# QZ1-boy/CDFO

Measured on AMD Instinct MI355X. Metric: x4 SR frames/sec, 7-frame 270x480->1080p, higher is better.
Workload: dtype fp16 MFMA, fp32 accumulate (1 pass inside Block_, 2 passes = fp16 hi+lo activations elsewhere, split-bf16 for the returned feature cache; 2-4e-4 max-abs vs the fp32 reference, bound 1e-3); 1 GPU; JCT-VC ClassB-shape synthetic clips: 8 clips/GPU x 7x1x270x480 luma (padded to 272x480) + MV/residual/partition/unfiltered priors -> 1080x1920, fresh path (pre_L1_fea=None), precision=fp16x2, Gumbel noise drawn per forward inside the mask kernel (the reference's default behaviour); clips_per_gpu=8, parallelism=batch-shard x1, weights=random init (seed 0), launch=eager

## Files before the change

### cdfo_amd/csrc/conv1x1_stream.hip

```cpp
#include "plane_chunk.h"

namespace {

struct st_item { const float* base; int ld; int ch0; };

struct st_args {
  st_item act[CDFO_MAXSRC * 4];
  int nkb;
  st_item res[2];
  const float* res_scale;
  const float* w; long long w_bstride; const float* bias;
  int Cin, Cout, CoutP, act_fn;
  float* out; int ldo;
  int B; long long P;
  int tiles_per_image; long long tiles;
  int ns;
  _Float16* ln_hl; const float* ln_g; const float* ln_b;
  const float* w_last;
  int W;
  float* csum; int csum_slots;
  pc_plane plane;
};

__host__ __device__ inline long long st_owner(long long t, long long tiles, int grid) { return ((t + 1) * grid + tiles - 1) / tiles - 1; }
// ... 42 lines not shown
    d_part[k] = (s & 15) ^ (p & 15);
  }
  auto part_off = [&](int q) { return r * 256 + ((q ^ (r & 15)) << 4); };

  f16x8_t twh[TAPS ? 4 : 1], twl[TAPS ? 4 : 1];
  if (TAPS) {
#pragma unroll
    for (int s4 = 0; s4 < 4; ++s4)
#pragma unroll
      for (int j = 0; j < 8; ++j) {
        const float wv = r < 9 ? a.w_last[(16 * s4 + 8 * h + j) * 9 + r] : 0.f;
        twh[s4][j] = (_Float16)wv;
        twl[s4][j] = (_Float16)(wv - (float)twh[s4][j]);
      }
  }

  for (long long img_t0 = t_lo; img_t0 < t_hi;) {
    const int b = (int)(img_t0 / a.tiles_per_image);
    const long long img_end = (long long)(b + 1) * a.tiles_per_image;
    const long long seg_hi = img_end < t_hi ? img_end : t_hi;
    __syncthreads();
    {
      const float* wb = a.w + (long long)b * a.w_bstride;
      const int ngrp = (a.Cin >> 2) * NCB * 64;
      for (int i = tid; i < ngrp; i += ST_THREADS) {
        const int rowpos = i % (NCB * 64), kg = i / (NCB * 64);
        const int n = mfma_row_channel(rowpos);
        f32x4 wv = {0.f, 0.f, 0.f, 0.f};
        if (n < a.CoutP) wv = *reinterpret_cast<const f32x4*>(wb + ((long long)kg * a.CoutP + n) * 4);
        const int c = kg >> 2, hh = (kg >> 1) & 1, j0 = (kg & 1) * 4;
        u32x2 hi, lo;
        split4_bf16(wv, hi, lo);
        const int off = ((c * 2 + hh) * (NCB * 64) + rowpos) * 16 + j0 * 2;
        *reinterpret_cast<u32x2*>(sWh + off) = hi;
        *reinterpret_cast<u32x2*>(sWl + off) = lo;
      }
      for (int i = tid; i < NCB * 64; i += ST_THREADS) sBias[i] = (a.bias && i < a.Cout) ? a.bias[i] : 0.f;
      if (PLANE) pc_load_weights<NCB>(a.plane.w + (long long)b * a.plane.w_bstride, a.CoutP, sPh, sPl, tid);
    }
    __syncthreads();

    const long long n_items = (seg_hi - img_t0) * items_per_tile;
    long long issued = 0;
    auto issue = [&](long long it) {
      const long long tile = img_t0 + it / items_per_tile;
      const int k = (int)(it % items_per_tile);
      const long long p0 = (tile - (long long)b * a.tiles_per_image) * 128 + wave * 32;
      if (a.res_scale && k == 0) {
        const long long rows = a.P - p0;
        const i32x4 rs = lds_dma_rsrc_uniform(a.res_scale + (long long)b * a.P + (rows > 0 ? p0 : 0),
                                              (unsigned)(rows > 0 ? (rows < 32 ? rows : 32) * 4 : 0));
        lds_dma0_dword((unsigned)r * 4, rs, __builtin_amdgcn_readfirstlane(scale_lds + (unsigned)(tile & 1) * 256));
      }
      if (PLANE && k == 0)
        pc_issue(pc_image(a.plane, b), (int)a.P, a.plane.W, (int)p0, lane, tap_lds + (unsigned)((it / items_per_tile) % NS) * PC_SLOT);
      st_item src;
      int chan0;
      if (k < nkb) { src = a.act[k]; chan0 = src.ch0; }
      else {
        const int j = k - nkb;
        src = a.res[j / NCB];
        chan0 = (j % NCB) * 64;
      }
      const long long rows_left = a.P - p0;
      const float* base = src.base + ((long long)b * a.P + (rows_left > 0 ? p0 : 0)) * src.ld + chan0;
      i32x4 rsrc = lds_dma_rsrc_uniform(base, 0u);
      const long long bytes = rows_left > 0 ? (rows_left < 32 ? rows_left : 32) * (long long)src.ld * 4 : 0;
      lds_dma_rsrc_resize_uniform(rsrc, (unsigned)bytes);
      unsigned voff[8];
#pragma unroll
      for (int q = 0; q < 8; ++q) voff[q] = (unsigned)(d_px[q] * src.ld * 4 + d_part[q] * 16);
      lds_dma0(voff, rsrc, __builtin_amdgcn_readfirstlane(ring_lds + (unsigned)(it % NS) * ST_STAGE));
    };
    for (; issued < NS - 1 && issued < n_items; ++issued) issue(issued);

    f32x16 acc[NCB][2];
    float cs[CSUM ? 32 : 1];
#pragma unroll
    for (int e = 0; e < (CSUM ? 32 : 1); ++e) cs[e] = 0.f;
    for (long long it = 0; it < n_items; ++it) {
      const int k = (int)(it % items_per_tile);
      st_wait_landed(TAPS ? 0 : issued - it - 1);
      const unsigned char* st = ring + (it % NS) * ST_STAGE;
      if (TAPS) {
        if (issued < n_items) { wait_lgkm<0>(); issue(issued); ++issued; }
      }
      if (k == 0) {
#pragma unroll
        for (int cb = 0; cb < NCB; ++cb)
#pragma unroll
          for (int ni = 0; ni < 2; ++ni)
#pragma unroll
            for (int e = 0; e < 16; ++e) acc[cb][ni][e] = 0.f;
        if (PLANE) {
          const int p = (int)((img_t0 + it / items_per_tile - (long long)b * a.tiles_per_image) * 128) + wave * 32 + r;
          unsigned thi[4], tlo[4];
          pc_operand(tap_slots + ((it / items_per_tile) % NS) * PC_SLOT, r, h, p, (int)a.P, a.plane.W, thi, tlo);
          pc_mfma<NCB>(sPh, sPl, r, h, thi, tlo, acc);
        }
      }
      if (k < nkb) {
#pragma unroll
        for (int c = 0; c < 4; ++c) {
          const f32x4 v0 = *reinterpret_cast<const f32x4*>(st + part_off(c * 4 + h * 2));
          const f32x4 v1 = *reinterpret_cast<const f32x4*>(st + part_off(c * 4 + h * 2 + 1));
          union { unsigned u[4]; bf16x8_t v; } ph, pl;
          split8_bf16(v0, v1, ph.u, pl.u);
          const int wrow = ((k * 4 + c) * 2 + h) * (NCB * 64) + r;
#pragma unroll
          for (int cb = 0; cb < NCB; ++cb)
#pragma unroll
            for (int ni = 0; ni < 2; ++ni) {
              const bf16x8_t wh = *reinterpret_cast<const bf16x8_t*>(sWh + (wrow + cb * 64 + ni * 32) * 16);
              const bf16x8_t wl = *reinterpret_cast<const bf16x8_t*>(sWl + (wrow + cb * 64 + ni * 32) * 16);
              acc[cb][ni] = __builtin_amdgcn_mfma_f32_32x32x16_bf16(wh, pl.v, acc[cb][ni], 0, 0, 0);
              acc[cb][ni] = __builtin_amdgcn_mfma_f32_32x32x16_bf16(wl, ph.v, acc[cb][ni], 0, 0, 0);
              acc[cb][ni] = __builtin_amdgcn_mfma_f32_32x32x16_bf16(wh, ph.v, acc[cb][ni], 0, 0, 0);
            }
        }
        if (k == nkb - 1) {
#pragma unroll
          for (int cb = 0; cb < NCB; ++cb)
#pragma unroll
            for (int ni = 0; ni < 2; ++ni)
#pragma unroll
              for (int e = 0; e < 16; ++e) {
                const float t = acc[cb][ni][e] + sBias[cb * 64 + ni * 32 + (e >> 3) * 16 + h * 8 + (e & 7)];
                acc[cb][ni][e] = fmaxf(t, 0.f) + slope * fminf(t, 0.f);
              }
        }
      } else {
        const int cb = (k - nkb) % NCB;
        float sc = 1.f;
        if (a.res_scale && (k - nkb) / NCB == nres - 1)
          sc = *reinterpret_cast<const float*>(scale_slots + ((img_t0 + it / items_per_tile) & 1) * 256 + lane * 4);
#pragma unroll
        for (int cc = 0; cc < NCB; ++cc) {
          if (cc != cb) continue;
#pragma unroll
          for (int ni = 0; ni < 2; ++ni)
#pragma unroll
            for (int jj = 0; jj < 2; ++jj) {
              const int q = (ni * 32 + jj * 16 + h * 8) >> 2;
              const f32x4 r0 = *reinterpret_cast<const f32x4*>(st + part_off(q));
              const f32x4 r1 = *reinterpret_cast<const f32x4*>(st + part_off(q + 1));
#pragma unroll
              for (int e = 0; e < 4; ++e) { acc[cc][ni][8 * jj + e] = fmaf(sc, r0[e], acc[cc][ni][8 * jj + e]); acc[cc][ni][8 * jj + 4 + e] = fmaf(sc, r1[e], acc[cc][ni][8 * jj + 4 + e]); }
            }
        }
      }
      if (!TAPS && issued < n_items) { wait_lgkm<0>(); issue(issued); ++issued; }
      if (k == items_per_tile - 1) {
        const long long tile = img_t0 + it / items_per_tile;
        const long long pin = (tile - (long long)b * a.tiles_per_image) * 128 + wave * 32 + r;
        if (NCB == 1 && a.ln_hl && !a.ln_g) {
          typedef _Float16 st_f16x8 __attribute__((ext_vector_type(8)));
          if (pin < a.P) {
#pragma unroll
            for (int ni = 0; ni < 2; ++ni)
#pragma unroll
              for (int jj = 0; jj < 2; ++jj) {
                const int n = ni * 32 + jj * 16 + h * 8;
                st_f16x8 hv;
#pragma unroll
                for (int e = 0; e < 8; ++e) hv[e] = (_Float16)acc[0][ni][8 * jj + e];
                *reinterpret_cast<st_f16x8*>(a.ln_hl + (((long long)b * 4 + (n >> 4)) * a.P + pin) * 16 + h * 8) = hv;
              }
          }
        } else if (NCB == 1 && a.ln_hl) {
          typedef _Float16 st_f16x8 __attribute__((ext_vector_type(8)));
          float sm = 0.f;
#pragma unroll
          for (int ni = 0; ni < 2; ++ni)
#pragma unroll
            for (int e = 0; e < 16; ++e) sm += acc[0][ni][e];
          sm += __shfl_xor(sm, 32, 64);
          const float mu = sm * (1.f / 64.f);
          float sq = 0.f;
#pragma unroll
          for (int ni = 0; ni < 2; ++ni)
#pragma unroll
            for (int e = 0; e < 16; ++e) { const float d = acc[0][ni][e] - mu; sq = fmaf(d, d, sq); }
          sq += __shfl_xor(sq, 32, 64);
          const float rstd = 1.f / sqrtf(sq * (1.f / 64.f) + 1e-5f);
          if (pin < a.P) {
#pragma unroll
            for (int ni = 0; ni < 2; ++ni)
#pragma unroll
              for (int jj = 0; jj < 2; ++jj) {
                const int n = ni * 32 + jj * 16 + h * 8;
                const f32x4 g0 = *reinterpret_cast<const f32x4*>(a.ln_g + n), g1 = *reinterpret_cast<const f32x4*>(a.ln_g + n + 4);
                const f32x4 b0 = *reinterpret_cast<const f32x4*>(a.ln_b + n), b1 = *reinterpret_cast<const f32x4*>(a.ln_b + n + 4);
                st_f16x8 hi, lo;
#pragma unroll
                for (int e = 0; e < 8; ++e) {
                  const float y = (acc[0][ni][8 * jj + e] - mu) * rstd * (e < 4 ? g0[e & 3] : g1[e & 3]) + (e < 4 ? b0[e & 3] : b1[e & 3]);
                  hi[e] = (_Float16)y;
                  lo[e] = (_Float16)(y - (float)hi[e]);
                }
                _Float16* o16 = a.ln_hl + (((long long)b * 8 + (n >> 4)) * a.P + pin) * 16 + h * 8;
                *reinterpret_cast<st_f16x8*>(o16) = hi;
                *reinterpret_cast<st_f16x8*>(o16 + 4 * a.P * 16) = lo;
              }
          }
        }
        if (TAPS) {
          const int oy = (int)(pin / a.W), ox = (int)(pin - (long long)oy * a.W);
#pragma unroll
          for (int cb = 0; cb < NCB; ++cb) {
            float amax = 0.f;
#pragma unroll
            for (int ni = 0; ni < 2; ++ni)
#pragma unroll
              for (int e = 0; e < 16; ++e) amax = fmaxf(amax, fabsf(acc[cb][ni][e]));
            amax = fmaxf(amax, __shfl_xor(amax, 32, 64));
            int ex = 0;
            if (amax > 0.f && amax < INFINITY) frexpf(amax, &ex);
            ex = ex < -100 ? -100 : (ex > 100 ? 100 : ex);
            const float sc = ldexpf(1.f, 14 - ex), inv = ldexpf(1.f, ex - 14);
            f32x16 tacc;
#pragma unroll
            for (int e = 0; e < 16; ++e) tacc[e] = 0.f;
#pragma unroll
            for (int s4 = 0; s4 < 4; ++s4) {
              unsigned hh[4], ll[4];
#pragma unroll
              for (int j = 0; j < 4; ++j)
                split_pair_f16(acc[cb][s4 >> 1][8 * (s4 & 1) + 2 * j] * sc, acc[cb][s4 >> 1][8 * (s4 & 1) + 2 * j + 1] * sc, hh[j], ll[j]);
              const u32x4 hu = {hh[0], hh[1], hh[2], hh[3]}, lu = {ll[0], ll[1], ll[2], ll[3]};
              const f16x8_t yh = __builtin_bit_cast(f16x8_t, hu), yl = __builtin_bit_cast(f16x8_t, lu);
              tacc = __builtin_amdgcn_mfma_f32_32x32x16_f16(twl[s4], yh, tacc, 0, 0, 0);
              tacc = __builtin_amdgcn_mfma_f32_32x32x16_f16(twh[s4], yl, tacc, 0, 0, 0);
              tacc = __builtin_amdgcn_mfma_f32_32x32x16_f16(twh[s4], yh, tacc, 0, 0, 0);
            }
            if (pin < a.P) {
              const long long opix = ((long long)b * 2 * (a.P / a.W) + 2 * oy + (cb >> 1)) * (2 * a.W) + 2 * ox + (cb & 1);
              float* op = a.out + opix * a.ldo;
              const f32x4 t4 = {tacc[0] * inv, tacc[1] * inv, tacc[2] * inv, tacc[3] * inv};
              *reinterpret_cast<f32x4*>(op + 4 * h) = t4;
              if (h == 0) op[8] = tacc[4] * inv;
            }
          }
        } else if (pin < a.P) {
          if (CSUM) {
#pragma unroll
            for (int ni = 0; ni < 2; ++ni)
#pragma unroll
              for (int e = 0; e < 16; ++e) cs[ni * 16 + e] += acc[0][ni][e];
          }
          float* op = a.out + ((long long)b * a.P + pin) * a.ldo;
#pragma unroll
          for (int cb = 0; cb < NCB; ++cb)
#pragma unroll
            for (int ni = 0; ni < 2; ++ni)
#pragma unroll
              for (int jj = 0; jj < 2; ++jj) {
                const int n = cb * 64 + ni * 32 + jj * 16 + h * 8;
                if (n < a.Cout) {
                  f32x4 v0, v1;
#pragma unroll
                  for (int e = 0; e < 4; ++e) { v0[e] = acc[cb][ni][8 * jj + e]; v1[e] = acc[cb][ni][8 * jj + 4 + e]; }
                  *reinterpret_cast<f32x4*>(op + n) = v0;
                  *reinterpret_cast<f32x4*>(op + n + 4) = v1;
                }
              }
        }
      }
    }
    if (CSUM) {
      float* red = reinterpret_cast<float*>(ring);
#pragma unroll
      for (int ni = 0; ni < 2; ++ni)
#pragma unroll
        for (int jj = 0; jj < 2; ++jj) {
          const int n = ni * 32 + jj * 16 + h * 8;
          const f32x4 v0 = {cs[ni * 16 + 8 * jj], cs[ni * 16 + 8 * jj + 1], cs[ni * 16 + 8 * jj + 2], cs[ni * 16 + 8 * jj + 3]};
          const f32x4 v1 = {cs[ni * 16 + 8 * jj + 4], cs[ni * 16 + 8 * jj + 5], cs[ni * 16 + 8 * jj + 6], cs[ni * 16 + 8 * jj + 7]};
          *reinterpret_cast<f32x4*>(red + r * 64 + n) = v0;
          *reinterpret_cast<f32x4*>(red + r * 64 + n + 4) = v1;
        }
      __syncthreads();
      const int slot = (int)(blockIdx.x - st_owner((long long)b * a.tiles_per_image, a.tiles, gridDim.x));
      if (tid < 64 && slot >= 0 && slot < a.csum_slots) {
        float sw[4];
#pragma unroll
        for (int wv = 0; wv < 4; ++wv) {
          const float* rw = reinterpret_cast<const float*>(smem + ring_off + wv * NS * ST_STAGE);
          float t = 0.f;
          for (int rr = 0; rr < 32; ++rr) t += rw[rr * 64 + tid];
          sw[wv] = t;
        }
        a.csum[((long long)b * a.csum_slots + slot) * 64 + tid] = (sw[0] + sw[1]) + (sw[2] + sw[3]);
      }
    }
    img_t0 = seg_hi;
  }
}

struct sg_args {
  st_item src[3];
  const float* w; const float* bias; int act_fn;
  long long P; int tiles_per_image; long long tiles;
  float* gram; float* sum0; float* sum1; int slots;
};

constexpr int SG_NS = 3;

template <int CH>
__global__ __launch_bounds__(ST_THREADS) void align_gram_partial_kernel(sg_args a) {
  extern __shared__ __attribute__((aligned(16))) unsigned char smem[];
  constexpr int NS = SG_NS, NKB = 2, IPT = 3, GS = CH + 2;
  const int tid = threadIdx.x, lane = tid & 63, h = lane >> 5, r = lane & 31;
  const int wave = __builtin_amdgcn_readfirstlane(tid >> 6);
  constexpr int w_half = NKB * 4 * 2 * 64 * 16;
  constexpr int ring_off = 2 * w_half + 64 * 4;
  unsigned char* sWh = smem;
  unsigned char* sWl = smem + w_half;
  float* sBias = reinterpret_cast<float*>(smem + 2 * w_half);
  unsigned char* ring = smem + ring_off + wave * NS * ST_STAGE;
  const unsigned ring_lds = (unsigned)(unsigned long long)(smem) + ring_off + wave * NS * ST_STAGE;

  const long long t_lo = a.tiles * blockIdx.x / gridDim.x, t_hi = a.tiles * (blockIdx.x + 1) / gridDim.x;
  if (t_lo >= t_hi) return;
  const float slope = a.act_fn == CDFO_ACT_NONE ? 1.f : (a.act_fn == CDFO_ACT_LRELU ? 0.1f : 0.f);

  int d_px[8], d_part[8];
#pragma unroll
  for (int k = 0; k < 8; ++k) {
    const int s = 64 * k + lane, p = s >> 4;
    d_px[k] = p;
    d_part[k] = (s & 15) ^ (p & 15);
  }
  auto part_off = [&](int q) { return r * 256 + ((q ^ (r & 15)) << 4); };

  for (int i = tid; i < (128 >> 2) * 64; i += ST_THREADS) {
    const int rowpos = i % 64, kg = i / 64;
    const int n = mfma_row_channel(rowpos);
    const f32x4 wv = *reinterpret_cast<const f32x4*>(a.w + ((long long)kg * 64 + n) * 4);
    const int c = kg >> 2, hh = (kg >> 1) & 1, j0 = (kg & 1) * 4;
    u32x2 hi, lo;
    split4_bf16(wv, hi, lo);
    const int off = ((c * 2 + hh) * 64 + rowpos) * 16 + j0 * 2;
    *reinterpret_cast<u32x2*>(sWh + off) = hi;
    *reinterpret_cast<u32x2*>(sWl + off) = lo;
  }
  for (int i = tid; i < 64; i += ST_THREADS) sBias[i] = a.bias ? a.bias[i] : 0.f;

  const int c_part = lane >> 2, c_sub = (lane & 3) * 4, h_part = (lane / CH) * CH / 4;

  for (long long img_t0 = t_lo; img_t0 < t_hi;) {
    const int b = (int)(img_t0 / a.tiles_per_image);
    const long long img_end = (long long)(b + 1) * a.tiles_per_image;
    const long long seg_hi = img_end < t_hi ? img_end : t_hi;
    __syncthreads();

    const long long n_items = (seg_hi - img_t0) * IPT;
    long long issued = 0;
    auto issue = [&](long long it) {
      const long long tile = img_t0 + it / IPT;
      const st_item src = a.src[(int)(it % IPT)];
      const long long p0 = (tile - (long long)b * a.tiles_per_image) * 128 + wave * 32;
      const long long rows_left = a.P - p0;
      const float* base = src.base + ((long long)b * a.P + (rows_left > 0 ? p0 : 0)) * src.ld + src.ch0;
      i32x4 rsrc = lds_dma_rsrc_uniform(base, 0u);
      const long long bytes = rows_left > 0 ? (rows_left < 32 ? rows_left : 32) * (long long)src.ld * 4 : 0;
      lds_dma_rsrc_resize_uniform(rsrc, (unsigned)bytes);
      unsigned voff[8];
#pragma unroll
      for (int q = 0; q < 8; ++q) voff[q] = (unsigned)(d_px[q] * src.ld * 4 + d_part[q] * 16);
      lds_dma0(voff, rsrc, __builtin_amdgcn_readfirstlane(ring_lds + (unsigned)(it % NS) * ST_STAGE));
    };
    for (; issued < NS - 1 && issued < n_items; ++issued) issue(issued);

    f32x16 acc[2];
    float g[CH], sq = 0.f, sk = 0.f, sx[2] = {0.f, 0.f};
#pragma unroll
    for (int j = 0; j < CH; ++j) g[j] = 0.f;
    for (long long it = 0; it < n_items; ++it) {
      const int k = (int)(it % IPT);
      st_wait_landed(issued - it - 1);
      const unsigned char* st = ring + (it % NS) * ST_STAGE;
      if (k == 0) {
#pragma unroll
        for (int ni = 0; ni < 2; ++ni)
#pragma unroll
          for (int e = 0; e < 16; ++e) acc[ni][e] = 0.f;
      }
      if (k < NKB) {
#pragma unroll
        for (int c = 0; c < 4; ++c) {
          const f32x4 v0 = *reinterpret_cast<const f32x4*>(st + part_off(c * 4 + h * 2));
          const f32x4 v1 = *reinterpret_cast<const f32x4*>(st + part_off(c * 4 + h * 2 + 1));
          union { unsigned u[4]; bf16x8_t v; } ph, pl;
          split8_bf16(v0, v1, ph.u, pl.u);
          const int wrow = ((k * 4 + c) * 2 + h) * 64 + r;
#pragma unroll
          for (int ni = 0; ni < 2; ++ni) {
            const bf16x8_t wh = *reinterpret_cast<const bf16x8_t*>(sWh + (wrow + ni * 32) * 16);
            const bf16x8_t wl = *reinterpret_cast<const bf16x8_t*>(sWl + (wrow + ni * 32) * 16);
            acc[ni] = __builtin_amdgcn_mfma_f32_32x32x16_bf16(wh, pl.v, acc[ni], 0, 0, 0);
            acc[ni] = __builtin_amdgcn_mfma_f32_32x32x16_bf16(wl, ph.v, acc[ni], 0, 0, 0);
            acc[ni] = __builtin_amdgcn_mfma_f32_32x32x16_bf16(wh, ph.v, acc[ni], 0, 0, 0);
          }
        }
        float t4[4] = {0.f, 0.f, 0.f, 0.f};
#pragma unroll
        for (int p = 0; p < 32; ++p)
          t4[p & 3] += *reinterpret_cast<const float*>(st + p * 256 + ((c_part ^ (p & 15)) << 4) + c_sub);
        sx[k] += (t4[0] + t4[1]) + (t4[2] + t4[3]);
        if (k == NKB - 1) {
          const long long pin = (img_t0 + it / IPT - (long long)b * a.tiles_per_image) * 128 + wave * 32 + r;
          const bool inside = pin < a.P;
#pragma unroll
          for (int ni = 0; ni < 2; ++ni)
#pragma unroll
            for (int e = 0; e < 16; ++e) {
              const float t = acc[ni][e] + sBias[ni * 32 + (e >> 3) * 16 + h * 8 + (e & 7)];
              acc[ni][e] = inside ? fmaxf(t, 0.f) + slope * fminf(t, 0.f) : 0.f;
            }
        }
      } else {
        unsigned char* kst = ring + ((it - 1) % NS) * ST_STAGE;
#pragma unroll
        for (int ni = 0; ni < 2; ++ni)
#pragma unroll
          for (int jj = 0; jj < 2; ++jj) {
            const int q0 = (ni * 32 + jj * 16 + h * 8) >> 2;
            const f32x4 v0 = {acc[ni][8 * jj], acc[ni][8 * jj + 1], acc[ni][8 * jj + 2], acc[ni][8 * jj + 3]};
            const f32x4 v1 = {acc[ni][8 * jj + 4], acc[ni][8 * jj + 5], acc[ni][8 * jj + 6], acc[ni][8 * jj + 7]};
            *reinterpret_cast<f32x4*>(kst + part_off(q0)) = v0;
            *reinterpret_cast<f32x4*>(kst + part_off(q0 + 1)) = v1;
          }
        float gt[CH], tq = 0.f, tk = 0.f;
#pragma unroll
        for (int j = 0; j < CH; ++j) gt[j] = 0.f;
#pragma unroll
        for (int p = 0; p < 32; ++p) {
          const int own = p * 256 + ((c_part ^ (p & 15)) << 4) + c_sub;
          const float qv = *reinterpret_cast<const float*>(st + own);
          const float kc = *reinterpret_cast<const float*>(kst + own);
          tq = fmaf(qv, qv, tq);
          tk = fmaf(kc, kc, tk);
#pragma unroll
          for (int j4 = 0; j4 < CH / 4; ++j4) {
            const f32x4 kv = *reinterpret_cast<const f32x4*>(kst + p * 256 + (((h_part + j4) ^ (p & 15)) << 4));
#pragma unroll
            for (int e = 0; e < 4; ++e) gt[j4 * 4 + e] = fmaf(qv, kv[e], gt[j4 * 4 + e]);
          }
        }
#pragma unroll
        for (int j = 0; j < CH; ++j) g[j] += gt[j];
        sq += tq;
        sk += tk;
      }
      if (issued < n_items) { wait_lgkm<0>(); issue(issued); ++issued; }
    }

    {
      float* red = reinterpret_cast<float*>(ring);
#pragma unroll
      for (int j = 0; j < CH; ++j) red[lane * GS + j] = g[j];
      red[lane * GS + CH] = sq;
      red[lane * GS + CH + 1] = sk;
      red[64 * GS + lane] = sx[0];
      red[64 * GS + 64 + lane] = sx[1];
      __syncthreads();
      const int slot = (int)(blockIdx.x - st_owner((long long)b * a.tiles_per_image, a.tiles, gridDim.x));
      if (slot >= 0 && slot < a.slots) {
        const float* r0 = reinterpret_cast<const float*>(smem + ring_off);
        const float* r1 = reinterpret_cast<const float*>(smem + ring_off + 1 * NS * ST_STAGE);
        const float* r2 = reinterpret_cast<const float*>(smem + ring_off + 2 * NS * ST_STAGE);
        const float* r3 = reinterpret_cast<const float*>(smem + ring_off + 3 * NS * ST_STAGE);
        const long long bs = (long long)b * a.slots + slot;
        for (int i = tid; i < 64 * GS + 128; i += ST_THREADS) {
          const float v = (r0[i] + r1[i]) + (r2[i] + r3[i]);
          if (i < 64 * GS) a.gram[bs * (64 * GS) + i] = v;
          else if (i < 64 * GS + 64) a.sum0[bs * 64 + (i - 64 * GS)] = v;
          else a.sum1[bs * 64 + (i - 64 * GS - 64)] = v;
        }
      }
    }
    img_t0 = seg_hi;
  }
}

}

extern "C" int cdfo_stream_slots_for_grid(int B, long long P, int grid) {
  if (B <= 0 || P <= 0 || grid <= 0 || (P + 127) / 128 > 0x7fffffff / 2) return CDFO_EINVAL;
  const int tpi = (int)((P + 127) / 128);
  const long long tiles = (long long)B * tpi;
  return st_slots(B, tpi, (int)(tiles < grid ? tiles : grid));
}
extern "C" int cdfo_stream_slot_of(int B, long long P, int grid, int wg, int b) {
  if (B <= 0 || P <= 0 || grid <= 0 || wg < 0 || b < 0 || b >= B) return CDFO_EINVAL;
  const int tpi = (int)((P + 127) / 128);
  const long long tiles = (long long)B * tpi;
  const int g = (int)(tiles < grid ? tiles : grid);
  if (wg >= g) return -1;
  const long long t_lo = tiles * wg / g, t_hi = tiles * (wg + 1) / g;
  const long long lo = t_lo > (long long)b * tpi ? t_lo : (long long)b * tpi, hi = t_hi < (long long)(b + 1) * tpi ? t_hi : (long long)(b + 1) * tpi;
  if (lo >= hi) return -1;
  return (int)(wg - st_owner((long long)b * tpi, tiles, g));
}
extern "C" int cdfo_align_stats_slots(int B, long long P) {
  const int cus = cdfo_num_cus();
  if (cus <= 0) return CDFO_EINVAL;
  return cdfo_stream_slots_for_grid(B, P, cus);
}

extern "C" int cdfo_align_stats(const float* x0, int ld0, const float* x1, int ld1, const float* q, int ldq, const float* w_packed,
                                const float* bias, int act, int ch_per_head, int B, long long P, int nslots, float* gram_partial,
                                float* sum0_partial, float* sum1_partial, void* stream) {
  if (B <= 0 || P <= 0 || nslots <= 0 || !x0 || !x1 || !q || !w_packed || !gram_partial || !sum0_partial || !sum1_partial) return CDFO_EINVAL;
  if (act != CDFO_ACT_NONE && act != CDFO_ACT_LRELU && act != CDFO_ACT_RELU) return CDFO_EINVAL;
  if (ch_per_head != 8 && ch_per_head != 16) return CDFO_EINVAL;
  const int lds_[3] = {ld0, ld1, ldq};
  for (int i = 0; i < 3; ++i)
    if (lds_[i] < 64 || lds_[i] % 4 || (long long)lds_[i] * 4 * 32 >= (1ll << 31)) return CDFO_EINVAL;
  if (!aligned16(x0) || !aligned16(x1) || !aligned16(q) || !aligned16(w_packed) || !aligned16(gram_partial) || !aligned16(sum0_partial) ||
      !aligned16(sum1_partial))
    return CDFO_EALIGN;
  if ((P + 127) / 128 > 0x7fffffff / 2) return CDFO_EINVAL;
  hipStream_t st = static_cast<hipStream_t>(stream);
  sg_args s{};
  s.src[0] = {x0, ld0, 0}; s.src[1] = {x1, ld1, 0}; s.src[2] = {q, ldq, 0};
  s.w = w_packed; s.bias = bias; s.act_fn = act;
  s.P = P;
  s.gram = gram_partial; s.sum0 = sum0_partial; s.sum1 = sum1_partial; s.slots = nslots;
  int grid;
  if (!st_tiling(B, P, s.tiles_per_image, s.tiles, grid)) return CDFO_EINVAL;
  if (nslots < st_slots(B, s.tiles_per_image, grid)) return CDFO_EINVAL;
  const int lds = st_lds_bytes(2, 1, SG_NS);
  const double px = (double)B * P;
  CdfoProfScope prof(st, KID_GRAM, px * (2.0 * 128 * 64 + 2.0 * 64 * 18), 4.0 * 192 * px);
  static CdfoAttrOnce once8, once16;
  return ch_per_head == 16 ? st_launch(align_gram_partial_kernel<16>, once16, grid, lds, st, s)
                           : st_launch(align_gram_partial_kernel<8>, once8, grid, lds, st, s);
}

int cdfo_conv1x1_stream_try(const cdfo_conv_args& a, hipStream_t st, const pc_plane* pl) {
  const bool ln_out = a.out2_cp16 != nullptr;
  const bool taps = a.store_mode == CDFO_STORE_TAPS9;
  if (taps && pl) return 0;
  if (taps) {
    if (a.Cin != 64 || a.nsrc != 1 || a.ldo % 4 || a.ldo < 12 || a.ln_gamma || ln_out || (long long)a.ld[0] * 4 * 32 >= (1ll << 31)) return 0;
    st_args s{};
    s.act[0].base = a.src[0]; s.act[0].ld = a.ld[0]; s.act[0].ch0 = 0;
    s.nkb = 1;
    s.w = a.w; s.w_bstride = a.w_bstride; s.bias = a.bias;
    s.Cin = 64; s.Cout = 256; s.CoutP = 256; s.act_fn = a.act;
    s.out = a.out; s.ldo = a.ldo; s.B = a.B; s.P = (long long)a.H * a.W;
    s.w_last = a.res2; s.W = a.W;
    s.ns = 2;
    int grid;
    if (!st_tiling(a.B, s.P, s.tiles_per_image, s.tiles, grid)) return CDFO_EINVAL;
    const double px = (double)a.B * s.P;
    CdfoProfScope prof(st, KID_CONV1, 2.0 * px * 256 * 64 + 2.0 * px * 4 * 9 * 64, 4.0 * (px * 64 + px * 4 * a.ldo + 64.0 * 256));
    static CdfoAttrOnce once;
    const int e = st_launch(conv1x1_stream_kernel<4, true>, once, grid, st_lds_bytes(1, 4, s.ns), st, s);
    return e == 0 ? 1 : e;
  }
  if (a.store_mode != CDFO_STORE_PLAIN || (a.ln_gamma && !ln_out) || a.CoutP % 64 || a.CoutP > 128 || a.Cout % 8) return 0;
  const bool plane = pl != nullptr;
  if (plane && (a.CoutP != 64 || ln_out || a.res2_pixscale || !pc_shape_ok((long long)a.H * a.W, a.W))) return 0;
  if (ln_out && (a.CoutP != 64 || a.Cout != 64)) return 0;
  if (a.chan_sum_out && (a.CoutP != 64 || a.Cout != 64 || ln_out || a.chan_sum_slots <= 0)) return 0;
  const int ncb = a.CoutP / 64, nkb = a.Cin / 64;
  if (nkb < 1 || nkb > CDFO_MAXSRC * 4) return 0;
  const int w_bytes = st_weight_bytes(nkb, ncb);
  const int scale_bytes = (a.res2 && a.res2_pixscale) ? 4 * 512 : 0;
  int ns = plane ? (ST_MAX_LDS - w_bytes - pc_weight_bytes(ncb)) / (4 * (ST_STAGE + PC_SLOT)) : (ST_MAX_LDS - scale_bytes - w_bytes) / (4 * ST_STAGE);
  if (ns > ST_MAXNS) ns = ST_MAXNS;
  if (scale_bytes) {
    const int items_per_tile = nkb + ((a.res1 ? 1 : 0) + 1) * ncb;
    if (ns > items_per_tile + 2) ns = items_per_tile + 2;
  }
  if (ns < 3) return 0;
  const long long P = (long long)a.H * a.W;
  st_args s{};
  int k = 0;
  for (int i = 0; i < a.nsrc; ++i) {
    if ((long long)a.ld[i] * 4 * 32 >= (1ll << 31)) return 0;
    for (int c = 0; c < a.cs[i]; c += 64) { s.act[k].base = a.src[i]; s.act[k].ld = a.ld[i]; s.act[k].ch0 = c; ++k; }
  }
  if (k != nkb) return 0;
  s.nkb = nkb;
  int nr = 0;
  if (a.res1) { if (a.ldr1 < a.CoutP) return 0; s.res[nr].base = a.res1; s.res[nr].ld = a.ldr1; ++nr; }
  if (a.res2) { if (a.ldr2 < a.CoutP) return 0; s.res[nr].base = a.res2; s.res[nr].ld = a.ldr2; ++nr; }
  s.res_scale = a.res2 ? a.res2_pixscale : nullptr;
  s.w = a.w; s.w_bstride = a.w_bstride; s.bias = a.bias;
  s.Cin = a.Cin; s.Cout = a.Cout; s.CoutP = a.CoutP; s.act_fn = a.act;
  s.out = a.out; s.ldo = a.ldo; s.B = a.B; s.P = P;
  s.ln_hl = ln_out ? static_cast<_Float16*>(a.out2_cp16) : nullptr; s.ln_g = a.ln_gamma; s.ln_b = a.ln_beta;
  s.ns = ns;
  int grid;
  if (!st_tiling(a.B, P, s.tiles_per_image, s.tiles, grid)) return CDFO_EINVAL;
  const int lds = st_lds_bytes(nkb, ncb, ns) + scale_bytes + (plane ? pc_lds_bytes(ncb, ns) : 0);
  const double px = (double)a.B * P;
  if (plane) { s.plane = *pl; s.plane.W = a.W; }
  CdfoProfScope prof(st, KID_CONV1, 2.0 * px * a.Cout * (a.Cin + (plane ? 16 : 0)),
                     4.0 * (px * a.Cout * (1 + nr) + px * a.Cin + (plane ? px : 0.0) + (double)a.Cin * a.Cout));
  if (a.chan_sum_out) {
    if (a.chan_sum_slots < st_slots(a.B, s.tiles_per_image, grid)) return 0;
    s.csum = a.chan_sum_out; s.csum_slots = a.chan_sum_slots;
  }
  static CdfoAttrOnce once_csum, once1, once2, once_pl, once_pl_csum;
  if (plane) {
    const int e = a.chan_sum_out ? st_launch(conv1x1_stream_kernel<1, false, true, true>, once_pl_csum, grid, lds, st, s)
                                 : st_launch(conv1x1_stream_kernel<1, false, false, true>, once_pl, grid, lds, st, s);
    return e == 0 ? 1 : e;
  }
  const int e = a.chan_sum_out ? st_launch(conv1x1_stream_kernel<1, false, true>, once_csum, grid, lds, st, s)
                : ncb == 1     ? st_launch(conv1x1_stream_kernel<1>, once1, grid, lds, st, s)
                               : st_launch(conv1x1_stream_kernel<2>, once2, grid, lds, st, s);
  return e == 0 ? 1 : e;
}
```

### cdfo_amd/csrc/plane_chunk.h

```cpp
#pragma once
#include "stream_ring.h"

struct pc_plane {
  const float* base; int Bi; long long s_b, s_g;
  int W;
  const float* w; long long w_bstride;
};

namespace {

constexpr int PC_SLOT = 3 * 256;
constexpr unsigned PC_OUTSIDE = 0x80000000u;

__host__ __device__ constexpr int pc_weight_bytes(int ncb) { return 2 * (2 * ncb * 64 * 16); }
__host__ __device__ constexpr int pc_lds_bytes(int ncb, int ns) { return pc_weight_bytes(ncb) + 4 * ns * PC_SLOT; }
inline bool pc_shape_ok(long long P, int W) { return W > 0 && P > 0 && P % W == 0 && P + 2ll * W + 64 < (1ll << 29); }

__device__ __forceinline__ const float* pc_image(const pc_plane& pl, int m) {
  return pl.base + (long long)(m % pl.Bi) * pl.s_b + (long long)(m / pl.Bi) * pl.s_g;
}

template <int NCB>
__device__ __forceinline__ void pc_load_weights(const float* w16, int CoutP, unsigned char* sPh, unsigned char* sPl, int tid) {
  for (int i = tid; i < 2 * NCB * 64; i += ST_THREADS) {
    const int rowpos = i % (NCB * 64), hh = i / (NCB * 64);
    const int n = mfma_row_channel(rowpos);
    f32x4 v0 = {0.f, 0.f, 0.f, 0.f}, v1 = {0.f, 0.f, 0.f, 0.f};
    if (n < CoutP) {
      v0 = *reinterpret_cast<const f32x4*>(w16 + n * 16 + hh * 8);
      v1 = *reinterpret_cast<const f32x4*>(w16 + n * 16 + hh * 8 + 4);
    }
    unsigned hi[4], lo[4];
    split8_bf16(v0, v1, hi, lo);
    const u32x4 h4 = {hi[0], hi[1], hi[2], hi[3]}, l4 = {lo[0], lo[1], lo[2], lo[3]};
    *reinterpret_cast<u32x4*>(sPh + (hh * (NCB * 64) + rowpos) * 16) = h4;
    *reinterpret_cast<u32x4*>(sPl + (hh * (NCB * 64) + rowpos) * 16) = l4;
  }
}

__device__ __forceinline__ void pc_issue(const float* img, int P, int W, int p0, int lane, unsigned slot_lds) {
  const i32x4 rs = lds_dma_rsrc_uniform(img, (unsigned)P * 4u);
#pragma unroll
  for (int dy = 0; dy < 3; ++dy) {
    const int idx = p0 + (dy - 1) * W - 1 + lane;
    const unsigned voff = (lane < 34 && idx >= 0 && idx < P) ? (unsigned)idx * 4u : PC_OUTSIDE;
    lds_dma0_dword(voff, rs, __builtin_amdgcn_readfirstlane(slot_lds + (unsigned)dy * 256u));
  }
}

__device__ __forceinline__ void pc_operand(const unsigned char* slot, int r, int h, int p, int P, int W, unsigned (&hi)[4],
                                           unsigned (&lo)[4]) {
  const int x = p % W;
  const bool inside = p < P, lok = inside && x > 0, rok = inside && x + 1 < W;
  float t[9];
#pragma unroll
  for (int dy = 0; dy < 3; ++dy) {
    const float* row = reinterpret_cast<const float*>(slot + dy * 256) + r;
    t[3 * dy] = lok ? row[0] : 0.f;
    t[3 * dy + 1] = inside ? row[1] : 0.f;
    t[3 * dy + 2] = rok ? row[2] : 0.f;
  }
  f32x4 v0, v1;
#pragma unroll
  for (int j = 0; j < 4; ++j) {
    v0[j] = h ? (j == 0 ? t[8] : (j == 1 && inside ? 1.f : 0.f)) : t[j];
    v1[j] = h ? 0.f : t[4 + j];
  }
  split8_bf16(v0, v1, hi, lo);
}

template <int NCB>
__device__ __forceinline__ void pc_mfma(const unsigned char* sPh, const unsigned char* sPl, int r, int h, const unsigned (&hi)[4],
                                        const unsigned (&lo)[4], f32x16 (&acc)[NCB][2]) {
  union { unsigned u[4]; bf16x8_t v; } ph, pl;
#pragma unroll
  for (int i = 0; i < 4; ++i) { ph.u[i] = hi[i]; pl.u[i] = lo[i]; }
  const int wrow = h * (NCB * 64) + r;
#pragma unroll
  for (int cb = 0; cb < NCB; ++cb)
#pragma unroll
    for (int ni = 0; ni < 2; ++ni) {
      const bf16x8_t wh = *reinterpret_cast<const bf16x8_t*>(sPh + (wrow + cb * 64 + ni * 32) * 16);
      const bf16x8_t wl = *reinterpret_cast<const bf16x8_t*>(sPl + (wrow + cb * 64 + ni * 32) * 16);
      acc[cb][ni] = __builtin_amdgcn_mfma_f32_32x32x16_bf16(wh, pl.v, acc[cb][ni], 0, 0, 0);
      acc[cb][ni] = __builtin_amdgcn_mfma_f32_32x32x16_bf16(wl, ph.v, acc[cb][ni], 0, 0, 0);
      acc[cb][ni] = __builtin_amdgcn_mfma_f32_32x32x16_bf16(wh, ph.v, acc[cb][ni], 0, 0, 0);
    }
}

}
```

### cdfo_amd/csrc/stats.hip

```cpp
#include "common.h"

namespace {

__global__ __launch_bounds__(256) void chan_sum_partial_kernel(const float* __restrict__ in, int ldi, long long P,
                                                               int nchunk, float* __restrict__ partial) {
  __shared__ f32x4 red[16][16];
  const int b = blockIdx.y, chunk = blockIdx.x;
  const int c4 = threadIdx.x & 15, sub = threadIdx.x >> 4;
  const long long per = (P + nchunk - 1) / nchunk;
  const long long p0 = chunk * per, p1 = (p0 + per < P) ? p0 + per : P;
  const float* base = in + (long long)b * P * ldi + c4 * 4;
  f32x4 s0 = {0.f, 0.f, 0.f, 0.f}, s1 = s0;
  long long p = p0 + sub;
  for (; p + 16 < p1; p += 32) {
    s0 += *reinterpret_cast<const f32x4*>(base + p * ldi);
    s1 += *reinterpret_cast<const f32x4*>(base + (p + 16) * ldi);
  }
  if (p < p1) s0 += *reinterpret_cast<const f32x4*>(base + p * ldi);
  red[sub][c4] = s0 + s1;
  __syncthreads();
  if (sub == 0) {
    f32x4 t = red[0][c4];
#pragma unroll
    for (int k = 1; k < 16; ++k) t += red[k][c4];
    *reinterpret_cast<f32x4*>(partial + ((long long)b * nchunk + chunk) * 64 + c4 * 4) = t;
  }
}

template <int CH>
__global__ __launch_bounds__(256) void gram_partial_kernel(const float* __restrict__ q, int ldq,
                                                           const float* __restrict__ k, int ldk, long long P,
                                                           int nchunk, float* __restrict__ partial) {
  __shared__ float red[4][64 * (CH + 2)];
  const int b = blockIdx.y, chunk = blockIdx.x;
  const int c = threadIdx.x & 63, sub = threadIdx.x >> 6;
  const int hbase = (c / CH) * CH;
  const long long per = (P + nchunk - 1) / nchunk;
  const long long p0 = chunk * per, p1 = (p0 + per < P) ? p0 + per : P;
  const float* qb = q + (long long)b * P * ldq;
  const float* kb = k + (long long)b * P * ldk;
  float g[CH], sq = 0.f, sk = 0.f;
#pragma unroll
  for (int j = 0; j < CH; ++j) g[j] = 0.f;
  for (long long p = p0 + sub; p < p1; p += 4) {
    const float qv = qb[p * ldq + c];
    const float kc = kb[p * ldk + c];
    sq += qv * qv;
    sk += kc * kc;
#pragma unroll
    for (int j4 = 0; j4 < CH / 4; ++j4) {
      const f32x4 kv = *reinterpret_cast<const f32x4*>(kb + p * ldk + hbase + j4 * 4);
#pragma unroll
      for (int e = 0; e < 4; ++e) g[j4 * 4 + e] += qv * kv[e];
    }
  }
#pragma unroll
  for (int j = 0; j < CH; ++j) red[sub][c * (CH + 2) + j] = g[j];
  red[sub][c * (CH + 2) + CH] = sq;
  red[sub][c * (CH + 2) + CH + 1] = sk;
  __syncthreads();
  float* out = partial + ((long long)b * nchunk + chunk) * 64 * (CH + 2);
  for (int i = threadIdx.x; i < 64 * (CH + 2); i += 256) out[i] = (red[0][i] + red[1][i]) + (red[2][i] + red[3][i]);
}

template <int CH>
__device__ void reduce_and_softmax(const float* __restrict__ partial, int nchunk, const float* __restrict__ temperature,
                                   float* stats, float* attn) {
  constexpr int N = 64 * (CH + 2);
  for (int i = threadIdx.x; i < N; i += blockDim.x) {
    float s = 0.f;
#pragma unroll 8
    for (int ch = 0; ch < nchunk; ++ch) s += partial[(long long)ch * N + i];
    stats[i] = s;
  }
  __syncthreads();
  if (threadIdx.x < 64) {
    const int c = threadIdx.x, head = c / CH;
    const float nq = fmaxf(sqrtf(stats[c * (CH + 2) + CH]), 1e-12f);
    const float t = temperature[head];
    float l[CH], mx = -INFINITY;
#pragma unroll
    for (int j = 0; j < CH; ++j) {
      const float nk = fmaxf(sqrtf(stats[(head * CH + j) * (CH + 2) + CH + 1]), 1e-12f);
      l[j] = stats[c * (CH + 2) + j] / (nq * nk) * t;
      mx = fmaxf(mx, l[j]);
    }
    float sum = 0.f;
#pragma unroll
    for (int j = 0; j < CH; ++j) { l[j] = expf(l[j] - mx); sum += l[j]; }
#pragma unroll
    for (int j = 0; j < CH; ++j) attn[c * CH + j] = l[j] / sum;
  }
  __syncthreads();
}

__global__ __launch_bounds__(256) void mdta_fold_kernel(const float* __restrict__ partial, int nchunk,
                                                        const float* __restrict__ temperature,
                                                        const float* __restrict__ proj, float* __restrict__ wout) {
  constexpr int CH = 8;
  __shared__ float stats[64 * (CH + 2)];
  __shared__ float attn[64 * CH];
  const int b = blockIdx.x;
  reduce_and_softmax<CH>(partial + (long long)b * nchunk * 64 * (CH + 2), nchunk, temperature, stats, attn);
  float* wo = wout + (long long)b * 4096;
  for (int idx = threadIdx.x; idx < 4096; idx += blockDim.x) {
    const int o = idx >> 6, i = idx & 63, hb = (i / CH) * CH, j = i - hb;
    float s = 0.f;
#pragma unroll
    for (int cc = 0; cc < CH; ++cc) s += proj[o * 64 + hb + cc] * attn[(hb + cc) * CH + j];
    wo[((i >> 2) * 64 + o) * 4 + (i & 3)] = s;
  }
}

__global__ __launch_bounds__(256) void align_fold_kernel(const float* __restrict__ gram_partial, int nchunk_g,
                                                         const float* __restrict__ sum_warp,
                                                         const float* __restrict__ sum_pred, int nchunk_s, float inv_P,
                                                         const float* __restrict__ temperature,
                                                         const float* __restrict__ du0_w, const float* __restrict__ du0_b,
                                                         const float* __restrict__ du2_w, const float* __restrict__ du2_b,
                                                         const float* __restrict__ proj, const float* __restrict__ wf,
                                                         float* __restrict__ wout) {
  constexpr int CH = 16;
  __shared__ float stats[64 * (CH + 2)];
  __shared__ float attn[64 * CH];
  __shared__ float Q[64 * 64];
  __shared__ float mean[2][64];
  __shared__ float hid[2][4];
  __shared__ float gate[2][64];
  const int b = blockIdx.x;
  reduce_and_softmax<CH>(gram_partial + (long long)b * nchunk_g * 64 * (CH + 2), nchunk_g, temperature, stats, attn);
  if (threadIdx.x < 128) {
    const int which = threadIdx.x >> 6, c = threadIdx.x & 63;
    const float* sp = (which ? sum_pred : sum_warp) + (long long)b * nchunk_s * 64;
    float s = 0.f;
#pragma unroll 8
    for (int ch = 0; ch < nchunk_s; ++ch) s += sp[ch * 64 + c];
    mean[which][c] = s * inv_P;
  }
  __syncthreads();
  if (threadIdx.x < 8) {
    const int which = threadIdx.x >> 2, m = threadIdx.x & 3;
    float s = du0_b[m];
    for (int c = 0; c < 64; ++c) s += du0_w[m * 64 + c] * mean[which][c];
    hid[which][m] = fmaxf(s, 0.f);
  }
  __syncthreads();
  if (threadIdx.x < 128) {
    const int which = threadIdx.x >> 6, c = threadIdx.x & 63;
    float s = du2_b[c];
    for (int m = 0; m < 4; ++m) s += du2_w[c * 4 + m] * hid[which][m];
    gate[which][c] = 1.f / (1.f + expf(-s));
  }
  for (int idx = threadIdx.x; idx < 4096; idx += blockDim.x) {
    const int o = idx >> 6, c = idx & 63;
    float s = 0.f;
    for (int m = 0; m < 64; ++m) s += wf[o * 128 + m] * proj[m * 64 + c];
    Q[idx] = s;
  }
  __syncthreads();
  float* wo = wout + (long long)b * (192 * 64);
  for (int idx = threadIdx.x; idx < 4096; idx += blockDim.x) {
    const int o = idx >> 6, i = idx & 63, hb = (i / CH) * CH, j = i - hb;
    float r = 0.f;
#pragma unroll
    for (int cc = 0; cc < CH; ++cc) r += Q[o * 64 + hb + cc] * attn[(hb + cc) * CH + j];
    wo[((i >> 2) * 64 + o) * 4 + (i & 3)] = r * gate[0][i];
    wo[(((64 + i) >> 2) * 64 + o) * 4 + (i & 3)] = r * gate[1][i];
    wo[(((128 + i) >> 2) * 64 + o) * 4 + (i & 3)] = wf[o * 128 + 64 + i];
  }
}

__global__ __launch_bounds__(64) void vec_mlp_kernel(const float* __restrict__ sum_partial, int nchunk, float inv_P,
                                                     const float* __restrict__ w1, const float* __restrict__ b1, int c1,
                                                     int act1, const float* __restrict__ w2,
                                                     const float* __restrict__ b2, int c2, int act2,
                                                     float* __restrict__ out) {
  __shared__ float mean[64], hid[64];
  const int b = blockIdx.x, t = threadIdx.x;
  float s = 0.f;
#pragma unroll 8
  for (int ch = 0; ch < nchunk; ++ch) s += sum_partial[((long long)b * nchunk + ch) * 64 + t];
  mean[t] = s * inv_P;
  __syncthreads();
  if (t < c1) {
    float a = b1 ? b1[t] : 0.f;
    for (int c = 0; c < 64; ++c) a += w1[t * 64 + c] * mean[c];
    hid[t] = act_apply(a, act1);
  }
  __syncthreads();
  if (!w2) {
    if (t < c1) out[(long long)b * c1 + t] = hid[t];
    return;
  }
  if (t < c2) {
    float a = b2 ? b2[t] : 0.f;
    for (int c = 0; c < c1; ++c) a += w2[t * c1 + c] * hid[c];
    out[(long long)b * c2 + t] = act_apply(a, act2);
  }
}

}

extern "C" int cdfo_chan_sum_partial(const float* in, int ldi, int B, long long P, int nchunk, float* partial,
                                     void* stream) {
  if (B <= 0 || P <= 0 || nchunk <= 0 || ldi % 4) return CDFO_EINVAL;
  if (!aligned16(in) || !aligned16(partial)) return CDFO_EALIGN;
  CdfoProfScope prof(static_cast<hipStream_t>(stream), KID_CHAN_SUM, 0, 4.0*64*(double)B*P);
  hipLaunchKernelGGL(chan_sum_partial_kernel, dim3(nchunk, B), dim3(256), 0, static_cast<hipStream_t>(stream), in, ldi,
                     P, nchunk, partial);
  CDFO_LAUNCH_CHECK();
  return 0;
}

extern "C" int cdfo_gram_partial(const float* q, int ldq, const float* k, int ldk, int B, long long P, int ch_per_head,
                                 int nchunk, float* partial, void* stream) {
  if (B <= 0 || P <= 0 || nchunk <= 0 || ldk % 4) return CDFO_EINVAL;
  if (!aligned16(k)) return CDFO_EALIGN;
  hipStream_t st = static_cast<hipStream_t>(stream);
  CdfoProfScope prof(static_cast<hipStream_t>(stream), KID_GRAM, 2.0*64*(ch_per_head+2)*(double)B*P, 4.0*128*(double)B*P);
  if (ch_per_head == 8)
    hipLaunchKernelGGL(gram_partial_kernel<8>, dim3(nchunk, B), dim3(256), 0, st, q, ldq, k, ldk, P, nchunk, partial);
  else if (ch_per_head == 16)
    hipLaunchKernelGGL(gram_partial_kernel<16>, dim3(nchunk, B), dim3(256), 0, st, q, ldq, k, ldk, P, nchunk, partial);
  else
    return CDFO_EINVAL;
  CDFO_LAUNCH_CHECK();
  return 0;
}

extern "C" int cdfo_mdta_fold(const float* partial, int nchunk, const float* temperature, const float* proj_w, int B,
                              float* wout, void* stream) {
  if (B <= 0 || nchunk <= 0) return CDFO_EINVAL;
  CdfoProfScope prof(static_cast<hipStream_t>(stream), KID_FOLD, 0, 0);
  hipLaunchKernelGGL(mdta_fold_kernel, dim3(B), dim3(256), 0, static_cast<hipStream_t>(stream), partial, nchunk,
                     temperature, proj_w, wout);
  CDFO_LAUNCH_CHECK();
  return 0;
}

extern "C" int cdfo_align_fold(const float* gram_partial, int nchunk_g, const float* sum_warp, const float* sum_pred,
                               int nchunk_s, long long P, const float* temperature, const float* du0_w,
                               const float* du0_b, const float* du2_w, const float* du2_b, const float* proj_w,
                               const float* fusion_w, int B, float* wout, void* stream) {
  if (B <= 0 || nchunk_g <= 0 || nchunk_s <= 0 || P <= 0) return CDFO_EINVAL;
  CdfoProfScope prof(static_cast<hipStream_t>(stream), KID_FOLD, 0, 0);
  hipLaunchKernelGGL(align_fold_kernel, dim3(B), dim3(256), 0, static_cast<hipStream_t>(stream), gram_partial, nchunk_g,
                     sum_warp, sum_pred, nchunk_s, 1.0f / (float)P, temperature, du0_w, du0_b, du2_w, du2_b, proj_w,
                     fusion_w, wout);
  CDFO_LAUNCH_CHECK();
  return 0;
}

extern "C" int cdfo_vec_mlp(const float* sum_partial, int nchunk, long long P, const float* w1, const float* b1, int c1,
                            int act1, const float* w2, const float* b2, int c2, int act2, int B, float* out,
                            void* stream) {
  if (B <= 0 || nchunk <= 0 || c1 <= 0 || c1 > 64 || (w2 && (c2 <= 0 || c2 > 64))) return CDFO_EINVAL;
  CdfoProfScope prof(static_cast<hipStream_t>(stream), KID_FOLD, 0, 0);
  hipLaunchKernelGGL(vec_mlp_kernel, dim3(B), dim3(64), 0, static_cast<hipStream_t>(stream), sum_partial, nchunk,
                     1.0f / (float)P, w1, b1, c1, act1, w2, b2, c2, act2, out);
  CDFO_LAUNCH_CHECK();
  return 0;
}
```

### cdfo_amd/csrc/stream_ring.h

```cpp
#pragma once
#include "lds_dma.h"
#include "numeric.h"

namespace {

constexpr int ST_THREADS = 256;
constexpr int ST_STAGE = 8192;
constexpr int ST_MAXNS = 4;
constexpr int ST_MAX_LDS = 160 * 1024 - 256;

__device__ __forceinline__ void st_wait_landed(long long younger) {
  if (younger >= 2) wait_vm<16>();
  else if (younger == 1) wait_vm<8>();
  else wait_vm<0>();
}

inline bool st_tiling(int B, long long P, int& tiles_per_image, long long& tiles, int& grid) {
  tiles_per_image = (int)((P + 127) / 128);
  tiles = (long long)B * tiles_per_image;
  const int cus = cdfo_num_cus();
  grid = (int)(tiles < cus ? tiles : cus);
  return cus > 0;
}
inline int st_weight_bytes(int nkb, int ncb) { return 2 * (nkb * 4 * 2 * ncb * 64 * 16) + ncb * 64 * 4; }
inline int st_lds_bytes(int nkb, int ncb, int ns) { return st_weight_bytes(nkb, ncb) + 4 * ns * ST_STAGE; }

template <class KernelPtr, class Args>
int st_launch(KernelPtr kernel, CdfoAttrOnce& once, int grid, int lds, hipStream_t st, const Args& s) {
  const hipError_t e = cdfo_set_max_lds(once, reinterpret_cast<const void*>(kernel), ST_MAX_LDS);
  if (e != hipSuccess) return (int)e;
  hipLaunchKernelGGL(kernel, dim3(grid), dim3(ST_THREADS), lds, st, s);
  return (int)hipGetLastError();
}

}
```

### cdfo_amd/cvsr_v8.py

```python
from __future__ import annotations

import threading

import contextlib
import math
from typing import Dict, List, Optional, Sequence

import torch
import torch.nn as nn

from . import kernels as K
from . import switches

NF, NFRAMES = 64, 7


def _param_spec():
    sp = []

    def conv(key, co, ci, kh, kw=None, bias=True, init="default"):
        kw = kw or kh
        sp.append((key + ".weight", (co, ci, kh, kw), ci * kh * kw, init))
        if bias:
            sp.append((key + ".bias", (co,), ci * kh * kw, "zero" if init == "kaiming0.1" else "bias"))

    conv("conv_first", 64, 1, 3)
    conv("conv_second", 64, 1, 3)
    p = "transformer_feature_extraction.path1."
    for n in ("norm1", "norm2"):
        sp.append((p + n + ".body.weight", (64,), None, "ones"))
        sp.append((p + n + ".body.bias", (64,), None, "zero"))
    sp.append((p + "attn.temperature", (8, 1, 1), None, "ones"))
    conv(p + "attn.qkv", 192, 64, 1, bias=False)
    conv(p + "attn.qkv_dwconv", 192, 1, 3, bias=False)
    conv(p + "attn.project_out", 64, 64, 1, bias=False)
    conv(p + "conv", 64, 64, 3)
    u = p + "side_to_feaoneUDSA.body."
    conv(u + "0", 16, 64, 3)
    conv(u + "2", 16, 16, 3)
    conv(u + "4", 16, 16, 3)
    conv(u + "6.spatial", 1, 2, 7)
    conv(u + "7", 16, 16, 3)
    conv(u + "9", 16, 16, 3)
    conv(u + "11", 64, 16, 3)
    conv("conv_expand_fea_r", 64, 128, 3)
    conv("conv_expand_ufs", 64, 1, 3)
    conv("conv_expand_rms", 64, 1, 3)
    conv("tsa_fusion", 64, 448, 1)
    for g in range(7):
        gp = f"recon_trunk.body.{g}."
        conv(gp + "conv", 64, 64, 3)
        for b in range(3):
            bp = gp + f"body.{b}."
            conv(bp + "body.0", 256, 64, 3, init="kaiming0.1")
            conv(bp + "body.2", 64, 256, 3, init="kaiming0.1")
            conv(bp + "down.0", 64, 64, 1, init="kaiming0.1")
            conv(bp + "up.0", 64, 64, 1, init="kaiming0.1")
    conv("upconv1", 256, 64, 1)
    conv("upconv2", 256, 64, 1)
    conv("conv_last", 1, 64, 3)
    a = "MV_deform_align."
    sp.append((a + "temperature", (4, 1, 1), None, "ones"))
    conv(a + "conv_du.0", 4, 64, 1)
    conv(a + "conv_du.2", 64, 4, 1)
    conv(a + "project_out", 64, 64, 1, bias=False)
    conv(a + "fusion_in.0", 64, 128, 1)
    conv(a + "fusion_in.2", 64, 64, 1)
    conv(a + "fusion_out.0", 64, 128, 1, bias=False)
    conv(a + "CALayer.conv_du.0", 64, 64, 1)
    conv(a + "CALayer.conv_du.2", 64, 64, 1)
    for rb in ("ResidualBlock.", "ResidualBlock1."):
        conv(a + rb + "conv1", 64, 64, 3, init="kaiming0.1")
        conv(a + rb + "conv2", 64, 64, 3, init="kaiming0.1")
    r = "RDAB."
    conv(r + "input_conv", 128, 64, 1)
    conv(r + "conv_du_re.0", 64, 64, 1)
    conv(r + "conv_du_re.2", 64, 64, 3)
    conv(r + "conv_du_re2.0", 64, 64, 1)
    conv(r + "fuse", 64, 128, 1)
    conv(r + "directW1_conv", 1, 1, 1, 9)
    conv(r + "directH1_conv", 1, 1, 9, 1)
    return sp


class _Holder(nn.Module):
    """Parameter container: reproduces the reference's module tree names without its Python forward code."""


def _register(root: nn.Module, key: str, param: nn.Parameter):
    parts = key.split(".")
    m = root
    for name in parts[:-1]:
        if name not in m._modules:
            m.add_module(name, _Holder())
        m = m._modules[name]
    m.register_parameter(parts[-1], param)


class CVSR_V8(nn.Module):
    def __init__(self, nf=64, nframes=7, fea_ext_RBs=7, SCGs=4, istraining=False):
        super().__init__()
        if nf != 64 or nframes != 7:
            raise ValueError("the HIP path is specialised for nf=64, nframes=7 (the only configuration the reference runs)")
        self.nf, self.center, self.istraining, self.stride = nf, nframes // 2, istraining, 4
        self.gumbel_uniform: Optional[Sequence[torch.Tensor]] = None
        self._precision = "fp16x2"
        self.neighbour_streams = 0
        self.udsa_n16 = switches.get("CDFO_UDSA_N16")
        self.udsa_side_stream = switches.get("CDFO_UDSA_STREAM")
        self.attn_pv_single = not switches.get("CDFO_ATTN_PV3")
        self.rdab_fused = switches.get("CDFO_RDAB_FUSED")
        self.prior_stems = switches.get("CDFO_PRIOR_STEMS")
        self.inline_rms = switches.get("CDFO_INLINE_RMS")
        self.neighbour_group = 0
        self.overlap_new_frame = switches.get("CDFO_OVERLAP_NEW")
        self.new_frame_alone = switches.get("CDFO_NEW_ALONE")
        self.trunk_side_stream = switches.get("CDFO_TRUNK_SIDE")
        self.wino_halfsplit = switches.get("CDFO_WINO_HS")
        self.align_stats = switches.get("CDFO_ALIGN_STATS")
        self.fe_weight_lo = True
        self.fea_r_single_pass = switches.get("CDFO_FEA_R_1PASS")
        for key, shape, fan_in, init in _param_spec():
            t = torch.empty(shape)
            if init == "default":
                nn.init.kaiming_uniform_(t, a=math.sqrt(5))
            elif init == "kaiming0.1":
                nn.init.kaiming_normal_(t, a=0, mode="fan_in")
                t.mul_(0.1)
            elif init == "bias":
                bound = 1.0 / math.sqrt(fan_in)
                nn.init.uniform_(t, -bound, bound)
            elif init == "ones":
                t.fill_(1.0)
            else:
                t.zero_()
            _register(self, key, nn.Parameter(t))
        self.debug_taps: Optional[dict] = None
        self.capture_noise: Optional[list] = None
        self._noise_seed = 0
        self._noise_key: Optional[torch.Tensor] = None
        self.range_guard = True
        self.last_range: Optional[dict] = None
        self._probe = None
        self._warned_range = False
        self.frames_extracted = 0
        self.frames_compensated = 0
        self._packed: Optional[dict] = None
        self._packed_sig = None

    def _signature(self):
        return tuple((p.data_ptr(), p._version) for p in self.parameters())

    def _weights(self) -> dict:
        sig = self._signature()
        if self._packed is not None and sig == self._packed_sig:
            return self._packed
        sd = {k: v.detach() for k, v in self.named_parameters()}
        for k, v in sd.items():
            if not v.is_cuda:
                raise NotImplementedError("CVSR_V8 (HIP): parameters must live on the GPU; call .cuda() / .to(device)")
            if v.dtype != torch.float32:
                raise NotImplementedError("CVSR_V8 (HIP): fp32 parameters expected")
        w: Dict[str, object] = {}

        def pc(key, **kw):
            w[key] = K.pack_conv(sd[key + ".weight"], sd.get(key + ".bias"), **kw)

        p = "transformer_feature_extraction.path1."
        for key in (p + "attn.qkv", p + "conv", p + "side_to_feaoneUDSA.body.0", p + "side_to_feaoneUDSA.body.11",
                    "conv_expand_fea_r", "tsa_fusion", "MV_deform_align.fusion_out.0",
                    "MV_deform_align.ResidualBlock.conv1", "MV_deform_align.ResidualBlock.conv2",
                    "MV_deform_align.ResidualBlock1.conv1", "MV_deform_align.ResidualBlock1.conv2",
                    "RDAB.input_conv", "RDAB.conv_du_re.0", "RDAB.conv_du_re.2", "RDAB.fuse"):
            pc(key)
        for g in range(7):
            pc(f"recon_trunk.body.{g}.conv")
            w[f"recon_trunk.body.{g}.conv_hl2"] = K.pack_conv_hilo(sd[f"recon_trunk.body.{g}.conv.weight"],
                                                                   sd[f"recon_trunk.body.{g}.conv.bias"], weight_lo=False)
            for b in range(3):
                for leaf in ("body.0", "body.2", "down.0", "up.0"):
                    pc(f"recon_trunk.body.{g}.body.{b}.{leaf}")
        masks = []
        for ph in range(4):
            pa, pb = ph >> 1, ph & 1
            m = 0
            for dy in range(3):
                for dx in range(3):
                    if 0 <= 2 * dy + pa - 1 <= 3 and 0 <= 2 * dx + pb - 1 <= 3:
                        m |= 1 << (dy * 3 + dx)
            masks += [m] * 16
        tap_mask = torch.tensor(masks, dtype=torch.int32, device=sd["conv_first.weight"].device)
        for g in range(7):
            for b in range(3):
                bp = f"recon_trunk.body.{g}.body.{b}."
                w3, b2 = sd[bp + "body.2.weight"], sd[bp + "body.2.bias"]
                wdn, bdn = sd[bp + "down.0.weight"][:, :, 0, 0], sd[bp + "down.0.bias"]
                w4 = w3.new_zeros(64, 256, 4, 4)
                for pa in range(2):
                    for pb in range(2):
                        w4[:, :, pa:pa + 3, pb:pb + 3] += 0.25 * w3
                wp = w3.new_zeros(64, 4, 256, 3, 3)
                for ph in range(4):
                    pa, pb = ph >> 1, ph & 1
                    for dy in range(3):
                        for dx in range(3):
                            u, v = 2 * dy + pa - 1, 2 * dx + pb - 1
                            if 0 <= u <= 3 and 0 <= v <= 3:
                                wp[:, ph, :, dy, dx] = w4[:, :, u, v]
                wf = torch.einsum("po,ocyx->pcyx", wdn, wp.view(64, 1024, 3, 3)).contiguous()
                fused = K.pack_conv(wf, wdn @ b2 + bdn)
                fused.tap_mask = tap_mask
                w[bp + "down_fused"] = fused
                wup, bup = sd[bp + "up.0.weight"][:, :, 0, 0], sd[bp + "up.0.bias"]
                w[bp + "body.2_up"] = K.pack_conv(torch.einsum("po,ocyx->pcyx", wup, w3).contiguous(), wup @ b2 + bup)
                w[bp + "pro"] = K.pack_block_prologue(sd[bp + "up.0.weight"], sd[bp + "up.0.bias"],
                                                      sd[bp + "down.0.weight"], sd[bp + "down.0.bias"])
        fe = "transformer_feature_extraction.path1."
        wlo = bool(getattr(self, "fe_weight_lo", True))
        w[fe + "conv_hl"] = K.pack_conv_hilo(sd[fe + "conv.weight"], sd[fe + "conv.bias"], wlo)
        w[fe + "side_to_feaoneUDSA.body.11_hl"] = K.pack_conv_hilo(sd[fe + "side_to_feaoneUDSA.body.11.weight"],
                                                                   sd[fe + "side_to_feaoneUDSA.body.11.bias"], wlo)
        w[fe + "qkv_dw"] = K.pack_qkv_dw(sd[fe + "attn.qkv.weight"], sd[fe + "norm1.body.weight"], sd[fe + "norm1.body.bias"])
        w["rms_du0"] = K.compose_stem_1x1(sd["conv_expand_rms.weight"], sd["conv_expand_rms.bias"], sd["RDAB.conv_du_re.0.weight"],
                                          sd["RDAB.conv_du_re.0.bias"])
        w["RDAB.conv_du_re.2_s2d"] = K.pack_conv_s2p2_s2d(sd["RDAB.conv_du_re.2.weight"], sd["RDAB.conv_du_re.2.bias"])
        w["RDAB.conv_du_re.2_stats"] = K.pack_rdab_stats(sd["RDAB.conv_du_re.2.weight"])
        w["rms_chunk"] = K.pack_plane_chunk(sd["conv_expand_rms.weight"], sd["conv_expand_rms.bias"])
        w["rms_chunk_input_conv"] = K.pack_plane_chunk(*K.compose_stem_1x1(
            sd["conv_expand_rms.weight"], sd["conv_expand_rms.bias"], sd["RDAB.input_conv.weight"],
            torch.zeros_like(sd["RDAB.input_conv.bias"])))
        w[fe + "side_to_feaoneUDSA.body.0_n16"] = K.pack_conv_n16(sd[fe + "side_to_feaoneUDSA.body.0.weight"])
        w["udsa_head"] = K.pack_udsa_head(sd[fe + "side_to_feaoneUDSA.body.0.weight"], sd[fe + "side_to_feaoneUDSA.body.0.bias"],
                                          sd["conv_second.weight"], sd["conv_second.bias"])
        pc("upconv1", shuffle2=True)
        pc("upconv2", shuffle2=True)
        w["raw"] = {k: v.contiguous() for k, v in sd.items()}
        self._packed, self._packed_sig = w, sig
        return w

    PRECISIONS = {"f32": K.PREC_F32, "bf16x3": K.PREC_BF16X3, "bf16": K.PREC_BF16, "fp16x2": K.PREC_FP16X2}

    def _conv(self, *args, exact=False, inner=False, **kw):
        prec = self.PRECISIONS[self.precision]
        if exact and prec == K.PREC_FP16X2:
            prec = K.PREC_BF16X3
        elif inner and prec == K.PREC_FP16X2:
            prec = K.PREC_FP16X1
        return K.conv(*args, prec=prec, **kw)

    def _udsa(self, w, x2, res, head=None):
        raw = w["raw"]
        u = "transformer_feature_extraction.path1.side_to_feaoneUDSA.body."
        if head is not None:
            t = head
        elif self.precision != "f32" and self.udsa_n16:
            t = K.conv3x3_n16(x2, w[u + "0_n16"], raw[u + "0.bias"], K.ACT_LRELU)
        else:
            t = self._conv(x2, w[u + "0"], pad=1, act=K.ACT_LRELU, exact=True)
        t = K.small_conv16(t, raw[u + "2.weight"], raw[u + "2.bias"], 2, 2, act=K.ACT_LRELU)
        t = K.small_conv16(t, raw[u + "4.weight"], raw[u + "4.bias"], 2, 2, act=K.ACT_LRELU)
        t = K.spatial_gate16(t, raw[u + "6.spatial.weight"], raw[u + "6.spatial.bias"])
        t = K.small_conv16(t, raw[u + "7.weight"], raw[u + "7.bias"], 2, 2, 0, True, K.ACT_LRELU)
        if self.precision == "fp16x2":
            t = K.small_conv16(t, raw[u + "9.weight"], raw[u + "9.bias"], 2, 2, 1, True, K.ACT_LRELU, out_hl=True)
            return K.conv_ring(t, w[u + "11_hl"], act=K.ACT_LRELU, res1=res, plane_wrap=2)
        t = K.small_conv16(t, raw[u + "9.weight"], raw[u + "9.bias"], 2, 2, 1, True, K.ACT_LRELU)
        return self._conv(t, w[u + "11"], pad=1, act=K.ACT_LRELU, res1=res, exact=True)

    def _feature_extraction(self, w, x1, prior, P, Bn):
        raw = w["raw"]
        p = "transformer_feature_extraction.path1."
        x2 = None
        main = torch.cuda.current_stream(x1.device)
        side = self._trunk_side(x1.device) if self.udsa_side_stream else None
        for rnd in range(3):
            with (torch.cuda.stream(side) if side is not None else contextlib.nullcontext()):
                if side is not None and rnd == 0:
                    side.wait_stream(main)
                if rnd == 0:
                    x2 = self._udsa(w, None, x1, head=K.udsa_head(prior, P, Bn, self.H, self.W, w["udsa_head"]))
                else:
                    x2 = self._udsa(w, x2, x2)
                if side is not None:
                    x2.record_stream(main)
            if self.precision == "f32":
                qkv = self._conv(x1, w[p + "attn.qkv"], ln=(raw[p + "norm1.body.weight"], raw[p + "norm1.body.bias"]))
                qkv = K.dwconv3x3(qkv, raw[p + "attn.qkv_dwconv.weight"])
            else:
                v, part, n = K.qkv_dw(x1, w[p + "qkv_dw"], raw[p + "attn.qkv_dwconv.weight"], gram=True)
                fold = K.mdta_fold(part, n, raw[p + "attn.temperature"], raw[p + "attn.project_out.weight"])
                if self.precision == "fp16x2":
                    x1, ln = self._conv(v, fold, res1=x1, ln_out=(raw[p + "norm2.body.weight"], raw[p + "norm2.body.bias"]))
                else:
                    x1 = self._conv(v, fold, res1=x1)
            if self.precision == "f32":
                part, n = K.gram_partial(qkv[..., 0:64], qkv[..., 64:128], 8)
                fold = K.mdta_fold(part, n, raw[p + "attn.temperature"], raw[p + "attn.project_out.weight"])
                x1 = self._conv(qkv[..., 128:192], fold, res1=x1)
            if side is not None:
                main.wait_stream(side)
            if self.precision == "fp16x2":
                x1 = K.conv_ring(ln, w[p + "conv_hl"], res1=x1, res2=x2, plane_wrap=8)
            else:
                ln = K.layernorm64(x1, raw[p + "norm2.body.weight"], raw[p + "norm2.body.bias"])
                x1 = self._conv(ln, w[p + "conv"], pad=1, res1=x1, res2=x2, exact=True)
        return x1

    def _rdab(self, w, du0, x, noises, stats=None, rms_planes=None):
        raw = w["raw"]
        GB, H, W, _ = x.shape
        G = len(noises)
        B = GB // G
        if stats is not None:
            part, n, count = stats
        else:
            t = self._conv(du0, w["RDAB.conv_du_re.2_s2d"], pad=1, act=K.ACT_RELU, exact=True)
            part, n = K.chan_sum_partial(t)
            count = t.shape[1] * t.shape[2]
        vmax = K.vec_mlp(part, n, count, raw["RDAB.conv_du_re2.0.weight"],
                         raw["RDAB.conv_du_re2.0.bias"], 64, K.ACT_RELU)
        am = 20 if self.precision == "fp16x2" and self.attn_pv_single else 0
        wW, bW = raw["RDAB.directW1_conv.weight"], raw["RDAB.directW1_conv.bias"]
        fused_prep = self.rdab_fused and self.precision != "f32" and K.rdab_prep_fused_ok(x, w["RDAB.input_conv"])
        if rms_planes is not None and not (fused_prep and rms_planes[1] % B == 0):
            raise ValueError("_rdab: rms_planes needs the fused mask kernel and each noise's images inside one block of planes")
        if fused_prep:
            vdt = torch.float16 if am == 20 else torch.float32
            sq, vrow, qwin = (K.empty_act(GB, H, W, 64, x.device) for _ in range(3))
            vwin = torch.empty((GB, H, W, 64), dtype=vdt, device=x.device)
            for g, noise in enumerate(noises):
                sl = slice(g * B, (g + 1) * B)
                plane = None
                if rms_planes is not None:
                    view, Bi, s_b, s_g = rms_planes
                    off = (g * B % Bi) * s_b + (g * B // Bi) * s_g
                    first = view.as_strided((1,), (1,), view.storage_offset() + off)
                    plane = (first, B, s_b, 0, w["rms_chunk_input_conv"])
                K.rdab_prep_fused(x[sl], w["RDAB.input_conv"], vmax[sl], noise, wW, bW, v_f16=(False, am == 20),
                                  outs=(sq[sl], vrow[sl], qwin[sl], vwin[sl]), plane=plane)
        else:
            vdt = torch.float32
            xq = self._conv(x, w["RDAB.input_conv"])
            vwin = xq[..., 64:128]
            sq, vrow, qwin = (K.empty_act(GB, H, W, 64, x.device) for _ in range(3))
            for g, noise in enumerate(noises):
                sl = slice(g * B, (g + 1) * B)
                outs = (sq[sl], vrow[sl], qwin[sl])
                if isinstance(noise, tuple):
                    _, seed, draw, capture = noise
                    K.rdab_prep_rng(xq[sl], vmax[sl], seed, draw, wW, bW, noise_out=capture, outs=outs)
                else:
                    K.rdab_prep(xq[sl], vmax[sl], noise, wW, bW, outs=outs)
        cat = K.empty_act(GB, H, W, 128, x.device)
        rowo = K.seq_attn(sq, vrow, am, out_dtype=vdt)
        qc = K.colconv9(sq, raw["RDAB.directH1_conv.weight"], raw["RDAB.directH1_conv.bias"])
        K.seq_attn(qc, rowo, am + 1, out=cat[..., 0:64])
        K.seq_attn(qwin, vwin, am + 2, out=cat[..., 64:128])
        if rms_planes is not None:
            return self._conv(cat, w["RDAB.fuse"], res1=x, plane=(*rms_planes, w["rms_chunk"]))
        return self._conv(cat, w["RDAB.fuse"], res1=x)

    def _align(self, w, xc, extra, pred, mvs, mv_bstride, out, frames=None):
        raw = w["raw"]
        a = "MV_deform_align."
        GB, H, W, _ = xc.shape
        B = GB // len(mvs)
        warped = K.empty_act(GB, H, W, NF, xc.device)
        if frames is not None:
            bank, idx, mvs1, slot0 = frames
            K.flow_warp_frames(bank, idx, mvs1, mv_bstride, slot0, len(mvs), B, out=warped)
        for g, mv in enumerate(mvs if frames is None else ()):
            K.flow_warp(extra[g * B:(g + 1) * B], mv, mv_bstride, out=warped[g * B:(g + 1) * B])
        fused = self.precision != "f32" and self.align_stats
        if fused:
            gp, sw, sp, ng = K.align_stats(warped, pred, xc, w[a + "fusion_out.0"], K.ACT_RELU, 16)
            ns = ng
        else:
            kf = self._conv([warped, pred], w[a + "fusion_out.0"], act=K.ACT_RELU)
            gp, ng = K.gram_partial(xc, kf, 16)
            sw, ns = K.chan_sum_partial(warped)
            sp, _ = K.chan_sum_partial(pred)
        fold = K.align_fold(gp, ng, sw, sp, ns, H * W, raw[a + "temperature"], raw[a + "conv_du.0.weight"],
                            raw[a + "conv_du.0.bias"], raw[a + "conv_du.2.weight"], raw[a + "conv_du.2.bias"],
                            raw[a + "project_out.weight"], raw[a + "fusion_out.0.weight"])
        if fused:
            o, part, n = self._conv([warped, pred, xc], fold, act=K.ACT_RELU, chan_sum_out=True)
        else:
            o = self._conv([warped, pred, xc], fold, act=K.ACT_RELU)
            part, n = K.chan_sum_partial(o)
        gate = K.vec_mlp(part, n, H * W, raw[a + "CALayer.conv_du.0.weight"], raw[a + "CALayer.conv_du.0.bias"], 64,
                         K.ACT_RELU, raw[a + "CALayer.conv_du.2.weight"], raw[a + "CALayer.conv_du.2.bias"], 64,
                         K.ACT_SIGMOID)
        rb = [w[a + n] for n in ("ResidualBlock.conv1", "ResidualBlock.conv2", "ResidualBlock1.conv1", "ResidualBlock1.conv2")]
        fast16 = self.precision == "fp16x2" and H % 2 == 0 and all(c.wh is not None for c in rb)
        if fast16:
            o, o16 = K.scale_channels(o, gate, want_cp16=True)
        else:
            o = K.scale_channels(o, gate)
        if fast16:
            n16 = torch.empty_like(o16)
            o = K.conv3x3_ws_res(K.conv3x3_ws(o16, rb[0], act=K.ACT_RELU), rb[1], res1=o, out2_cp16=n16)
            return K.conv3x3_ws_res(K.conv3x3_ws(n16, rb[2], act=K.ACT_RELU), rb[3], res1=o, res2=xc, out=out)
        r = self._conv(o, rb[0], pad=1, act=K.ACT_RELU)
        o = self._conv(r, rb[1], pad=1, res1=o)
        r = self._conv(o, rb[2], pad=1, act=K.ACT_RELU)
        return self._conv(r, rb[3], pad=1, res1=o, res2=xc, out=out)

    def _block(self, w, p, x, x16=None, want16=False, want_hl=False):
        b0, b2, dn, up = w[p + "body.0"], w[p + "body.2"], w[p + "down.0"], w[p + "up.0"]
        t16 = self.precision == "fp16x2"
        if t16 and x.shape[1] % 4 == 0 and b0.wh is not None:
            c1 = lambda src, **kw: K.conv3x3_body0(src, b0, act=K.ACT_LRELU, **kw)
            up2 = (b0.ww is not None and K.wino_up2_enabled() and x.shape[1] % 2 == 0 and x.shape[2] % 2 == 0
                   and x.shape[1] * x.shape[2] * 8 * b0.Cout < (1 << 31))
            if x16 is None:
                u16, d16, x16 = K.block_prologue(x, w[p + "pro"], want_x16=True, lowres_up=up2)
            else:
                u16, d16 = K.block_prologue(x, w[p + "pro"], lowres_up=up2)
            hs = up2 and self.wino_halfsplit
            c2 = (lambda src: K.conv3x3_wino_up2(src, b0, act=K.ACT_LRELU, halfsplit=hs)) if up2 else (lambda src: c1(src, s2d=True))
            side = self._trunk_side(x.device) if self.trunk_side_stream else None
            if side is not None:
                main = torch.cuda.current_stream(x.device)
                side.wait_stream(main)
                with torch.cuda.stream(side):
                    d = K.conv_ring(c1(d16), w[p + "body.2_up"])
                out = K.conv_ring(c1(x16), b2, res1=x)
                t = c2(u16)
                main.wait_stream(side)
                d.record_stream(main)
            else:
                out = K.conv_ring(c1(x16), b2, res1=x)
                d = K.conv_ring(c1(d16), w[p + "body.2_up"])
                t = c2(u16)
            y16 = torch.empty_like(x16) if want16 else None
            if want_hl:
                y16 = torch.empty((x16.shape[0], 8) + tuple(x16.shape[2:]), dtype=torch.float16, device=x16.device)
            y = K.conv_ring(t, w[p + "down_fused"], res1=out, res_up2=d, out2_cp16=y16, out2_hl=want_hl, src_halfsplit=hs)
            return (y, y16) if (want16 or want_hl) else y
        out = self._conv(self._conv(x, b0, pad=1, act=K.ACT_LRELU, out_f16=t16, inner=True), b2, pad=1, res1=x)
        d = self._conv(K.resample2(x, up=False), dn)
        d = self._conv(self._conv(d, b0, pad=1, act=K.ACT_LRELU, out_f16=t16, inner=True), b2, pad=1)
        K.resample2(self._conv(d, up), up=True, out=out, accumulate=True)
        u = K.resample2(self._conv(x, up), up=True, out_f16=t16)
        t = self._conv(u, b0, pad=1, act=K.ACT_LRELU, s2d=True, out_f16=t16, inner=True)
        y = self._conv(t, w[p + "down_fused"], pad=1, res1=out)
        return (y, None) if want16 else y

    def _side(self, device, count):
        cache = self.__dict__.setdefault("_side_streams", {})
        if (device, count) not in cache:
            cache[(device, count)] = [torch.cuda.Stream(device) for _ in range(count)]
        return cache[(device, count)]

    def _trunk_side(self, device):
        return self._side(device, 1)[0]

    def _trunk(self, w, fused):
        y = fused
        for g in range(7):
            r, r16 = y, None
            fast = self.precision == "fp16x2" and y.shape[1] % 4 == 0 and w[f"recon_trunk.body.{g}.body.0.body.0"].wh is not None
            for b in range(3):
                if b < 2:
                    r, r16 = self._block(w, f"recon_trunk.body.{g}.body.{b}.", r, r16, want16=True)
                elif fast:
                    r, r16 = self._block(w, f"recon_trunk.body.{g}.body.{b}.", r, r16, want_hl=True)
                else:
                    r, r16 = self._block(w, f"recon_trunk.body.{g}.body.{b}.", r, r16), None
            if fast:
                y = K.conv_ring(r16, w[f"recon_trunk.body.{g}.conv_hl2"], res1=y, res2=fused if g == 6 else None)
            else:
                y = self._conv(r, w[f"recon_trunk.body.{g}.conv"], pad=1, res1=y, res2=fused if g == 6 else None)
        return y

    _tls = threading.local()

    @property
    def precision(self) -> str:
        ov = getattr(CVSR_V8._tls, "override", None)
        if ov is not None and ov[0] is self:
            return ov[1]
        return self._precision

    @precision.setter
    def precision(self, value: str):
        if value not in self.PRECISIONS:
            raise ValueError(f"precision must be one of {sorted(self.PRECISIONS)}, got {value!r}")
        self._precision = value

    def _resolve_noise(self, x, gumbel_uniform):
        noise = gumbel_uniform if gumbel_uniform is not None else self.gumbel_uniform
        if noise is None:
            if torch.cuda.is_current_stream_capturing():
                if self._noise_key is None or self._noise_key.device != x.device:
                    raise RuntimeError("CVSR_V8 (HIP): call model.refresh_noise_key(device) before capturing a forward "
                                       "that draws its own Gumbel noise")
                self._noise_seed = self._noise_key
            else:
                self._noise_seed = K.next_noise_seed(x.device)
        return noise

    def forward(self, x, mvs0, mvs1, pms, rms, ufs, pre_L1_fea=None, gumbel_uniform=None):
        self._check("forward", x, grad_ok=True, capture_ok=True)
        with K.on_device(x):
            training = torch.is_grad_enabled() and any(p.requires_grad for p in self.parameters())
            if training and torch.cuda.is_current_stream_capturing():
                raise RuntimeError("CVSR_V8 (HIP): the autograd path cannot be captured into a HIP graph (its mask kernel takes the "
                                   "Philox key as a launch argument); capture inference forwards under torch.no_grad()")
            noise = self._resolve_noise(x, gumbel_uniform)
            if training:
                if pre_L1_fea is not None:
                    raise NotImplementedError("CVSR_V8 (HIP): the cached-feature path is an inference path; training uses fresh clips")
                for prm in self.parameters():
                    if not prm.is_cuda or prm.dtype != torch.float32:
                        raise NotImplementedError("CVSR_V8 (HIP): fp32 parameters on the GPU expected")
                from .cvsr_v8_train import forward_train
                return forward_train(self, x, mvs0, mvs1, pms, rms, ufs, noise)
            return self._guarded(x.device, lambda: self._forward(x, mvs0, mvs1, pms, rms, ufs, pre_L1_fea, noise))

    def _guarded(self, device, run, rerun=None):
        if not (self.precision == "fp16x2" and self.range_guard):
            return run()
        capturing = torch.cuda.is_current_stream_capturing()
        if capturing:
            probe = self.__dict__.get("_graph_probe")
            if probe is None:
                raise RuntimeError("CVSR_V8 (HIP): the fp16 range guard reads probes back and cannot be captured by hand; use "
                                   "model.capture(), whose graph carries the two probes and whose replay() reads them back")
            probe.zero_()
        else:
            probe = torch.zeros(4, dtype=torch.int32, device=device)
        self._probe = probe
        try:
            res = run()
        finally:
            self._probe = None
        if capturing or not self._settle_range(probe):
            return res
        return self._recompute_bf16x3(rerun or run, self._noise_seed)

    def _settle_range(self, probe) -> bool:
        pinned = self.__dict__.setdefault("_guard_pinned", {})
        if probe.device not in pinned:
            pinned[probe.device] = torch.zeros(4, dtype=torch.int32).pin_memory()
        host = pinned[probe.device]
        host.copy_(probe, non_blocking=True)
        ev = torch.cuda.Event()
        ev.record()
        ev.synchronize()
        self.last_range = self._range_verdict(host)
        return self.last_range["fallback"]

    FP16_WINDOW = (2.0 ** -6, 2.0 ** 11)

    def _range_verdict(self, host4) -> dict:
        amax = host4[0:1].view(torch.float32).item()
        nonfinite = bool(host4[1].item()) or bool(host4[3].item())
        lo, hi = self.FP16_WINDOW
        return {"trunk_input_amax": amax, "nonfinite": nonfinite, "fallback": nonfinite or not (amax == 0.0 or lo <= amax <= hi)}

    def _range_fallback(self, args, out_ref, l1_ref):
        x, mvs0, mvs1, pms, rms, ufs, pre, noise, seed = args
        res = self._recompute_bf16x3(lambda: self._forward(x, mvs0, mvs1, pms, rms, ufs, pre, noise), seed)
        if out_ref is not None:
            out_ref.copy_(res[0])
        if l1_ref is not None:
            l1_ref.copy_(res[1])
        return res

    def _recompute_bf16x3(self, run, seed):
        lr = self.last_range
        if not self._warned_range:
            import warnings
            warnings.warn(f"CVSR_V8 (HIP): activations leave the fp16 range (max |trunk input| = {lr['trunk_input_amax']:.3g}, non-finite "
                          f"result: {lr['nonfinite']}); this forward and others like it are recomputed with "
                          "precision='bf16x3'.  Set model.precision = 'bf16x3' to avoid the repeated work.")
            self._warned_range = True
        CVSR_V8._tls.override = (self, "bf16x3")
        keep_seed, self._noise_seed = self._noise_seed, seed
        try:
            with torch.no_grad():
                return run()
        finally:
            CVSR_V8._tls.override = None
            self._noise_seed = keep_seed

    def forward_front(self, x, mvs0, mvs1, pms, rms, ufs, pre_L1_fea=None, gumbel_uniform=None):
        self._check("forward_front", x, capture_ok=True)
        with K.on_device(x):
            noise = self._resolve_noise(x, gumbel_uniform)
            fused, L1, xf = self._front(x, mvs0, mvs1, pms, rms, ufs, pre_L1_fea, noise)
        return (fused, xf), L1.permute(0, 3, 1, 2)

    def forward_back(self, state):
        fused, xf = state
        with K.on_device(fused):
            return self._back(fused, xf)

    def _check(self, what: str, t: torch.Tensor, size=None, clip=False, grad_ok=False, capture_ok=False):
        if not t.is_cuda:
            raise NotImplementedError("CVSR_V8 (HIP): CPU tensors are not supported; there is no CPU fallback")
        if not grad_ok and torch.is_grad_enabled() and any(p.requires_grad for p in self.parameters()):
            raise NotImplementedError(f"CVSR_V8 (HIP): {what} is an inference call -- wrap it in torch.no_grad()")
        if not capture_ok and torch.cuda.is_current_stream_capturing():
            raise NotImplementedError(f"CVSR_V8 (HIP): {what} is not captured into HIP graphs")
        if clip:
            if t.dim() != 5 or t.shape[1] != NFRAMES or t.shape[2] != 1:
                raise ValueError(f"expected x of shape [B,7,1,H,W], got {tuple(t.shape)}")
            size = t.shape[3:]
        if size is not None:
            H, W = size
            if H % 8 or W % 8:
                raise ValueError(f"H and W must be multiples of 8 (window attention, arch.py:2147,2235); got {H}x{W}")

    def extract_features(self, frames, pms):
        self._check("extract_features", frames, size=frames.shape[2:])
        F, C, H, W = frames.shape
        if C != 1 or tuple(pms.shape) != (F, 1, H, W):
            raise ValueError(f"expected frames and pms of shape [F,1,H,W], got {tuple(frames.shape)} and {tuple(pms.shape)}")
        with K.on_device(frames):
            w = self._weights()
            raw = w["raw"]
            self.H, self.W = H, W
            self.frames_extracted += F
            f = K.stem_conv(frames.contiguous().float(), H * W, F, H, W, raw["conv_first.weight"], raw["conv_first.bias"], K.ACT_LRELU)
            return self._feature_extraction(w, f, pms.contiguous().float(), H * W, F)

    def forward_windows(self, Lf, x, mvs0, mvs1, rms, ufs, gumbel_uniform=None):
        self._check("forward_windows", x, clip=True)
        Kw, N, C, H, W = x.shape
        if tuple(Lf.shape) != (N, Kw, H, W, NF):
            raise ValueError(f"expected x [K,7,1,H,W] and Lf [7,K,H,W,64], got {tuple(x.shape)} and {tuple(Lf.shape)}")
        if Lf.dtype != torch.float32 or not Lf.is_contiguous():
            raise ValueError("Lf must be a dense fp32 tensor")
        with K.on_device(x):
            noise = self._resolve_noise(x, gumbel_uniform)
            x = x.contiguous().float()
            mvs1 = mvs1.contiguous().float()
            self.H, self.W = H, W

            def run():
                fused = self._fuse_windows(self._weights(), Lf, x, mvs1, rms, ufs, noise)
                return self._back(fused, x)

            return self._guarded(x.device, run)

    def resolve_noise_key(self, device, key: Optional[int] = None) -> int:
        self._noise_seed = K.next_noise_seed(torch.device(device)) if key is None else int(key)
        return self._noise_seed

    def compensate_features(self, fea, rms, gumbel_uniform=None, draws=None):
        self._check("compensate_features", fea, size=fea.shape[1:3])
        if fea.dim() != 4 or fea.shape[3] != NF or fea.dtype != torch.float32 or not fea.is_contiguous():
            raise ValueError(f"compensate_features: fea must be a dense fp32 [F,H,W,64] tensor, got {fea.dtype} {tuple(fea.shape)}")
        F, H, W, _ = fea.shape
        if tuple(rms.shape) != (F, 1, H, W):
            raise ValueError(f"compensate_features: rms must be [F,1,H,W] = {(F, 1, H, W)}, got {tuple(rms.shape)}")
        noise = gumbel_uniform if gumbel_uniform is not None else self.gumbel_uniform
        draws = list(range(F)) if draws is None else [int(d) for d in draws]
        if len(draws) != F or (noise is not None and len(noise) != F):
            raise ValueError(f"compensate_features: one noise tensor / one draw index per frame expected (F = {F})")
        for f, u in enumerate(noise or ()):
            if tuple(u.shape) != (1, NF, H, W):
                raise ValueError(f"compensate_features: noise of frame {f} must be [1,64,{H},{W}], got {tuple(u.shape)}")
        with K.on_device(fea):
            w = self._weights()
            self.H, self.W = H, W
            self.frames_compensated += F
            return self._compensate(w, fea, [(rms.contiguous().float(), H * W, slice(0, F))], draws, noise)[0]

    def forward_windows_shared(self, Lc, comp_bank, comp_idx, x, mvs1, ufs, recompensate=None):
        self._check("forward_windows_shared", x, clip=True)
        Kw, N, C, H, W = x.shape
        if tuple(Lc.shape) != (Kw, H, W, NF) or comp_bank.dim() != 4 or tuple(comp_bank.shape[1:]) != (H, W, NF):
            raise ValueError(f"expected x [K,7,1,H,W], Lc [K,H,W,64] and comp_bank [cap,H,W,64], got {tuple(x.shape)}, {tuple(Lc.shape)} "
                             f"and {tuple(comp_bank.shape)}")
        for name, t in (("Lc", Lc), ("comp_bank", comp_bank)):
            if t.dtype != torch.float32 or not t.is_contiguous():
                raise ValueError(f"{name} must be a dense fp32 tensor")
        if comp_idx.dtype != torch.int32 or comp_idx.device != x.device or comp_idx.numel() != (N - 1) * Kw or not comp_idx.is_contiguous():
            raise ValueError("comp_idx must be a dense int32 [6,K] tensor on the operands' device")
        if tuple(mvs1.shape) != (Kw, N, 2, H, W) or ufs.numel() != Kw * N * H * W:
            raise ValueError(f"expected mvs1 [K,7,2,H,W] and ufs [K,7,1,H,W], got {tuple(mvs1.shape)} and {tuple(ufs.shape)}")
        with K.on_device(x):
            x = x.contiguous().float()
            mvs1 = mvs1.contiguous().float()
            ufs = ufs.contiguous().float().view(Kw, 1, N, H, W)
            self.H, self.W = H, W
            state = [comp_bank, comp_idx.view(-1)]

            def run():
                fused = self._fuse_windows_shared(self._weights(), Lc, state[0], state[1], x, mvs1, ufs)
                return self._back(fused, x)

            def rerun():
                if recompensate is not None:
                    bank2, idx2 = recompensate()
                    state[0], state[1] = bank2, idx2.view(-1)
                return run()

            return self._guarded(x.device, run, rerun)

    def capture(self, x, mvs0, mvs1, pms, rms, ufs, pre_L1_fea=None, gumbel_uniform=None, check_range: bool = True):
        from .graph import CapturedForward
        return CapturedForward(self, x, mvs0, mvs1, pms, rms, ufs, pre_L1_fea, gumbel_uniform, check_range)

    def capture_pipelined(self, x, mvs0, mvs1, pms, rms, ufs, pre_L1_fea=None, gumbel_uniform=None, check_range: bool = True):
        from .graph import PipelinedForward
        return PipelinedForward(self, x, mvs0, mvs1, pms, rms, ufs, pre_L1_fea, gumbel_uniform, check_range)

    def refresh_noise_key(self, device=None) -> int:
        dev = torch.device(device) if device is not None else next(self.parameters()).device
        if dev.type == "cuda" and dev.index is None:
            dev = torch.device("cuda", torch.cuda.current_device())
        seed = K.next_noise_seed(dev)
        if self._noise_key is None or self._noise_key.device != dev:
            self._noise_key = torch.empty(1, dtype=torch.int64, device=dev)
        self._noise_key.fill_(seed)
        return seed

    def _forward(self, x, mvs0, mvs1, pms, rms, ufs, pre_L1_fea=None, gumbel_uniform=None):
        fused, L1, xf = self._front(x, mvs0, mvs1, pms, rms, ufs, pre_L1_fea, gumbel_uniform)
        return self._back(fused, xf, L1), L1.permute(0, 3, 1, 2)

    def _front(self, x, mvs0, mvs1, pms, rms, ufs, pre_L1_fea=None, gumbel_uniform=None):
        self._check("forward", x, clip=True, grad_ok=True, capture_ok=True)
        B, N, C, H, W = x.shape
        w = self._weights()
        raw = w["raw"]
        self.H, self.W = H, W
        ctr = self.center
        x = x.contiguous().float()
        pms = pms.contiguous().float()
        mvs1 = mvs1.contiguous().float()
        P = H * W

        nstr = int(getattr(self, "neighbour_streams", 0)) or 2
        gsz = int(getattr(self, "neighbour_group", 0)) or ctr
        deferred_new = None

        self.frames_extracted += B * N if pre_L1_fea is None else B
        if pre_L1_fea is None:
            f = K.stem_conv(x, P, B * N, H, W, raw["conv_first.weight"], raw["conv_first.bias"], K.ACT_LRELU)
            L1 = self._feature_extraction(w, f, pms, P, B * N)
        else:
            last_x, last_p = x[:, -1].contiguous(), pms[:, -1].contiguous()
            pre = self._as_pixel_major(pre_L1_fea, B * N, H, W)
            L1 = torch.empty_like(pre)
            L1v, prev = L1.view(B, N, H, W, NF), pre.view(B, N, H, W, NF)
            L1v[:, :-1].copy_(prev[:, 1:])

            def new_frame_features():
                f = K.stem_conv(last_x, P, B, H, W, raw["conv_first.weight"], raw["conv_first.bias"], K.ACT_LRELU)
                L1v[:, -1].copy_(self._feature_extraction(w, f, last_p, P, B))

            if B == 1 and nstr > 1 and gsz == ctr and self.overlap_new_frame:
                deferred_new = new_frame_features
            else:
                new_frame_features()
        Lf = (K.swap_outer(L1, B, N) if B > 1 else L1).view(N, B, H, W, NF)
        return self._fuse_windows(w, Lf, x, mvs1, rms, ufs, gumbel_uniform, deferred_new), L1, x

    def _fuse_windows(self, w, Lf, x, mvs1, rms, ufs, gumbel_uniform, deferred_new=None):
        N, ctr = NFRAMES, self.center
        nstr = int(getattr(self, "neighbour_streams", 0)) or 2
        gsz = int(getattr(self, "neighbour_group", 0)) or ctr
        if ufs.shape[1] != 1:
            ufs, rms = ufs.transpose(1, 2), rms.transpose(1, 2)
        ufs = ufs.contiguous().float()
        rms = rms.contiguous().float()
        groups = [list(range(s, min(s + gsz, e))) for (s0, e) in ((0, ctr), (ctr + 1, N)) for s in range(s0, e, gsz)]
        if deferred_new is not None and self.new_frame_alone:
            groups = [list(range(0, ctr)), list(range(ctr + 1, N - 1)), [N - 1]]
        xcG = Lf[ctr].repeat(gsz, 1, 1, 1) if gsz > 1 else Lf[ctr]
        keep = []
        aligned = self._fork_join(x.device, nstr, groups, deferred_new, lambda gi, idxs: self._neighbour_group(
            w, Lf, idxs, xcG, ufs, rms, mvs1, gumbel_uniform, keep))
        return self._fuse(w, Lf[ctr], aligned)

    def _fuse_windows_shared(self, w, Lc, comp_bank, comp_idx, x, mvs1, ufs):
        B, N, ctr = x.shape[0], NFRAMES, self.center
        xcG = Lc.repeat(ctr, 1, 1, 1)
        keep = []
        aligned = self._fork_join(x.device, 2, [list(range(0, ctr)), list(range(ctr + 1, N))], None, lambda gi, idxs: self._align_group(
            w, idxs, xcG, ufs, mvs1, keep, frames=(comp_bank, comp_idx[gi * ctr * B:(gi + 1) * ctr * B])))
        return self._fuse(w, Lc, aligned)

    def _fork_join(self, device, nstr, groups, deferred_new, body):
        main = torch.cuda.current_stream(device)
        side = self._side(device, nstr) if nstr > 1 else []
        for st in side:
            st.wait_stream(main)
        if deferred_new is not None:
            deferred_new()
        by_frame = {}
        for gi, idxs in enumerate(groups):
            on_side = bool(side) and not (deferred_new is not None and NFRAMES - 1 in idxs)
            with torch.cuda.stream(side[gi % len(side)]) if on_side else contextlib.nullcontext():
                al = body(gi, idxs)
            if on_side:
                al.record_stream(main)
            B = al.shape[0] // len(idxs)
            for n, i in enumerate(idxs):
                by_frame[i] = al[n * B:(n + 1) * B]
        for st in side:
            main.wait_stream(st)
        return by_frame

    def _fuse(self, w, centre, aligned):
        fused = self._conv([centre if i == self.center else aligned[i] for i in range(NFRAMES)], w["tsa_fusion"], act=K.ACT_LRELU)
        if self._probe is not None:
            K.range_probe(fused, self._probe[0:2])
        return fused

    def _back(self, fused, x, L1=None):
        B, N, C, H, W = x.shape
        w = self._weights()
        raw = w["raw"]
        ctr, P = self.center, H * W
        t = self._trunk(w, fused)
        if self._probe is not None:
            K.range_probe(t, self._probe[2:4])
        if self.debug_taps is not None:
            self.debug_taps.update(L1_fea=L1, fused=fused, trunk=t)
        t = self._conv(t, w["upconv1"], act=K.ACT_LRELU)
        if self.precision == "f32":
            t = self._conv(t, w["upconv2"], act=K.ACT_LRELU)
            out = K.conv_last(t, raw["conv_last.weight"], raw["conv_last.bias"], x[:, ctr], N * P)
        else:
            out = K.upconv_last(t, w["upconv2"], raw["conv_last.weight"], raw["conv_last.bias"], x[:, ctr], N * P)
        return out

    def _neighbour_group(self, w, Lf, idxs, xcG, ufs, rms, mvs1, noise, keep):
        N, B, H, W, _ = Lf.shape
        G = len(idxs)
        stems = [(rms[:, 0, i], N * H * W, slice(n * B, (n + 1) * B)) for n, i in enumerate(idxs)]
        draws = [i - (i > self.center) for i in idxs]
        fea_i, x_n = self._compensate(w, Lf[idxs[0]:idxs[0] + G].view(G * B, H, W, NF), stems, draws,
                                      None if noise is None else [noise[d] for d in draws], keep)
        if self.debug_taps is not None:
            for n, i in enumerate(idxs):
                self.debug_taps[f"rdab_{i}"] = x_n[n * B:(n + 1) * B]
        return self._align_group(w, idxs, xcG, ufs, mvs1, keep, extra=fea_i)

    def _compensate(self, w, fea, stems, draws, noise, keep=None):
        raw = w["raw"]
        M, H, W, _ = fea.shape
        dev = fea.device
        du0 = stats = planes = None
        if self.prior_stems and self.precision != "f32" and not self.istraining and K.rdab_stats_ok(H, W):
            stats = self._mask_stats(w, stems, M, H, W)
            planes = self._inline_rms_planes(w, fea, stems, len(draws))
        if planes is not None:
            fea_com = None
        elif stats is not None:
            fea_com = K.empty_act(M, H, W, NF, dev)
            for rms, bstride, sl in stems:
                K.stem_conv(rms, bstride, sl.stop - sl.start, H, W, raw["conv_expand_rms.weight"], raw["conv_expand_rms.bias"],
                            add=fea[sl], out2=fea_com[sl], write_out=False)
        else:
            fea_com = K.empty_act(M, H, W, NF, dev)
            du0 = K.empty_act(M, H // 2 + 1, W // 2 + 1, 4 * NF, dev)
            du0[:, H // 2].zero_()
            du0[:, :, W // 2].zero_()
            for rms, bstride, sl in stems:
                K.stem_conv2(rms, bstride, sl.stop - sl.start, H, W, raw["conv_expand_rms.weight"], raw["conv_expand_rms.bias"],
                             fea[sl], fea_com[sl], w["rms_du0"][0], w["rms_du0"][1], K.ACT_RELU, du0[sl], s2dB=True)
        noises = []
        for k, draw in enumerate(draws):
            if noise is None:
                cap = None
                if self.capture_noise is not None:
                    cap = torch.empty((M // len(draws), NF, H, W), device=dev, dtype=torch.float32)
                    self.capture_noise.append(cap)
                noises.append(("rng", self._noise_seed, draw, cap))
            else:
                noises.append(noise[k].to(device=dev, dtype=torch.float32).contiguous())
        if planes is not None:
            x_n = self._rdab(w, du0, fea, noises, stats, rms_planes=planes)
        else:
            x_n = self._rdab(w, du0, fea_com, noises, stats)
        fea_i = self._conv([fea, x_n], w["conv_expand_fea_r"], pad=1, inner=self.fea_r_single_pass)
        if keep is not None:
            keep.extend([du0, stats, fea_com, noises, x_n, fea_i])
        return fea_i, x_n

    @staticmethod
    def _affine_stems(stems):
        v0, s_b, sl0 = stems[0]
        Bi = sl0.stop - sl0.start
        step = (stems[1][0].data_ptr() - v0.data_ptr()) // 4 if len(stems) > 1 else 0
        if step >= 0 and all(v.untyped_storage().data_ptr() == v0.untyped_storage().data_ptr() and bs == s_b
                             and (sl.start, sl.stop) == (k * Bi, (k + 1) * Bi) and v.data_ptr() == v0.data_ptr() + 4 * k * step
                             for k, (v, bs, sl) in enumerate(stems)):
            return v0, Bi, s_b, step
        return None

    def _inline_rms_planes(self, w, fea, stems, nnoise):
        M, H, W, _ = fea.shape
        if not (self.inline_rms and "rms_chunk" in w and self.rdab_fused and K.plane_ok(H, W) and M % nnoise == 0
                and K.rdab_prep_fused_ok(fea, w["RDAB.input_conv"])):
            return None
        aff = self._affine_stems(stems)
        if aff is None or aff[1] % (M // nnoise) or any(v.dtype != torch.float32 for v, _, _ in stems):
            return None
        return aff

    @staticmethod
    def _mask_stats(w, stems, M, H, W):
        args = (*w["rms_du0"], w["RDAB.conv_du_re.2_stats"], w["raw"]["RDAB.conv_du_re.2.bias"])
        aff = CVSR_V8._affine_stems(stems)
        if aff is not None:
            v0, Bi, s_b, step = aff
            return K.rdab_stats(v0, Bi, s_b, step, M, H, W, *args)
        count = (H // 2 + 1) * (W // 2 + 1)
        n = K.nchunks_for(count)
        part = torch.empty((M, n, 64), dtype=torch.float32, device=stems[0][0].device)
        for v, bs, sl in stems:
            K.rdab_stats(v, sl.stop - sl.start, bs, 0, sl.stop - sl.start, H, W, *args, out=part[sl])
        return part, n, count

    def _align_group(self, w, idxs, xcG, ufs, mvs1, keep, extra=None, frames=None):
        raw = w["raw"]
        B, N, _, H, W = mvs1.shape
        GB, P = len(idxs) * B, H * W
        ufs_prior = K.empty_act(GB, H, W, NF, xcG.device)
        for n, i in enumerate(idxs):
            K.stem_conv(ufs[:, 0, i], N * P, B, H, W, raw["conv_expand_ufs.weight"], raw["conv_expand_ufs.bias"],
                        out=ufs_prior[n * B:(n + 1) * B])
        al = K.empty_act(GB, H, W, NF, xcG.device)
        xc = xcG if xcG.shape[0] == GB else xcG[:GB]
        self._align(w, xc, extra, ufs_prior, [mvs1[:, i] for i in idxs], N * 2 * P, al,
                    frames=None if frames is None else (*frames, mvs1, idxs[0]))
        if self.debug_taps is not None:
            for n, i in enumerate(idxs):
                self.debug_taps[f"align_{i}"] = al[n * B:(n + 1) * B]
        keep.extend([ufs_prior, xc])
        return al

    @staticmethod
    def _as_pixel_major(t: torch.Tensor, F: int, H: int, W: int) -> torch.Tensor:
        if tuple(t.shape) != (F, NF, H, W):
            raise ValueError(f"pre_L1_fea must be [{F},{NF},{H},{W}], got {tuple(t.shape)}")
        t = t.float()
        v = t.permute(0, 2, 3, 1)
        if v.is_contiguous():
            return v
        return K.nchw_to_nhwc(t.contiguous())
```

### cdfo_amd/kernels.py

```python
from __future__ import annotations

import contextlib
import ctypes as C
from dataclasses import dataclass
from typing import Optional, Sequence

import numpy as np
import torch

from . import _lib, switches
from ._lib import CdfoError, ConvArgs, _vp, check

ACT_NONE, ACT_LRELU, ACT_RELU, ACT_SIGMOID = 0, 1, 2, 3
PREC_F32, PREC_BF16X3, PREC_BF16, PREC_FP16X2, PREC_FP16, PREC_FP16X1 = 0, 1, 2, 3, 4, 5


def _stream() -> C.c_void_p:
    return C.c_void_p(torch.cuda.current_stream().cuda_stream)


def on_device(t: torch.Tensor):
    if not t.is_cuda:
        raise NotImplementedError("the HIP path needs device tensors (there is no CPU fallback)")
    return torch.cuda.device(t.device)
# ... 1057 lines not shown
    lo = (w - hi.float()).bfloat16()
    pack = lambda t: t.view(128, 4, 2, 8).permute(1, 2, 0, 3).contiguous().view(-1)
    return torch.cat([pack(hi), pack(lo)]).contiguous(), torch.cat([b_up.detach().float(), b_dn.detach().float()]).contiguous()


def block_prologue(x: torch.Tensor, packed, want_x16: bool = False, lowres_up: bool = False):
    B, H, W, Cc, ld = _chk_act(x)
    assert Cc == 64 and H % 2 == 0 and W % 2 == 0
    u16 = torch.empty((B, 4, H, W, 16) if lowres_up else (B, 4, 2 * H, 2 * W, 16), dtype=torch.float16, device=x.device)
    d16 = torch.empty((B, 4, H // 2, W // 2, 16), dtype=torch.float16, device=x.device)
    x16 = torch.empty((B, 4, H, W, 16), dtype=torch.float16, device=x.device) if want_x16 else None
    check(_lib.lib().cdfo_block_prologue2(_vp(x), ld, B, H, W, _vp(packed[0]), _vp(packed[1]), _vp(None if lowres_up else u16),
                                          _vp(u16 if lowres_up else None), _vp(d16), _vp(x16), _stream()), "cdfo_block_prologue2")
    return (u16, d16, x16) if want_x16 else (u16, d16)


def pack_qkv_dw(w_qkv: torch.Tensor, gamma: torch.Tensor, beta: torch.Tensor):
    w = w_qkv.detach().float().reshape(192, 64)
    wg = w * gamma.detach().float()[None, :]
    hi = wg.bfloat16()
    lo = (wg - hi.float()).bfloat16()
    pack = lambda t: t.view(192, 4, 2, 8).permute(1, 2, 0, 3).contiguous().view(-1)
    return torch.cat([pack(hi), pack(lo)]).contiguous(), (w @ beta.detach().float()).contiguous()


def qkv_dw(x: torch.Tensor, packed, dw_w: torch.Tensor, eps: float = 1e-5, gram: bool = False):
    B, H, W, Cc, ld = _chk_act(x)
    assert Cc == 64
    if gram:
        out = empty_act(B, H, W, 64, x.device)
        n = int(_lib.lib().cdfo_qkv_dw_gram_slots(B, H, W))
        if n < 1:
            raise CdfoError("cdfo_qkv_dw_gram_slots failed")
        part = torch.zeros((B, n, 640), dtype=torch.float32, device=x.device)
        check(_lib.lib().cdfo_qkv_dw(_vp(x), ld, B, H, W, _vp(packed[0]), _vp(packed[1]), _vp(dw_w), C.c_float(eps), _vp(out),
                                     64, _vp(part), n, _stream()), "cdfo_qkv_dw")
        return out, part, n
    out = empty_act(B, H, W, 192, x.device)
    check(_lib.lib().cdfo_qkv_dw(_vp(x), ld, B, H, W, _vp(packed[0]), _vp(packed[1]), _vp(dw_w), C.c_float(eps), _vp(out),
                                 192, None, 0, _stream()), "cdfo_qkv_dw")
    return out


def layernorm64_hl(x: torch.Tensor, gamma: torch.Tensor, beta: torch.Tensor) -> torch.Tensor:
    B, H, W, Cc, ld = _chk_act(x)
    assert Cc == 64
    out = torch.empty((B, 8, H, W, 16), dtype=torch.float16, device=x.device)
    check(_lib.lib().cdfo_layernorm64_cp16hl(_vp(x), ld, _vp(gamma), _vp(beta), B, C.c_longlong(H * W), _vp(out), _stream()),
          "cdfo_layernorm64_cp16hl")
    return out


def pack_conv_hilo(weight: torch.Tensor, bias: Optional[torch.Tensor], weight_lo: bool = True) -> PackedConv:
    w = weight.detach().float()
    wh = w.half().float()
    return pack_conv(torch.cat([wh, wh, w - wh] if weight_lo else [wh, wh], 1).contiguous(), bias)


def dwconv3x3(x: torch.Tensor, w: torch.Tensor) -> torch.Tensor:
    B, H, W, Cc, ld = _chk_act(x)
    out = empty_act(B, H, W, Cc, x.device)
    check(_lib.lib().cdfo_dwconv3x3(_vp(x), ld, _vp(w), B, H, W, Cc, _vp(out), Cc, _stream()), "cdfo_dwconv3x3")
    return out


def flow_warp(x: torch.Tensor, mv: torch.Tensor, mv_bstride: int, out: Optional[torch.Tensor] = None) -> torch.Tensor:
    B, H, W, Cc, ld = _chk_act(x)
    if out is None:
        out = empty_act(B, H, W, Cc, x.device)
    elif tuple(out.shape) != (B, H, W, Cc) or not out.is_contiguous():
        raise ValueError("flow_warp: out must be a dense tensor of the input's shape")
    check(_lib.lib().cdfo_flow_warp(_vp(x), ld, _vp(mv), C.c_longlong(mv_bstride), B, H, W, Cc, _vp(out), Cc,
                                    _stream()), "cdfo_flow_warp")
    return out


def flow_warp_frames(bank: torch.Tensor, idx: torch.Tensor, mv: torch.Tensor, mv_kstride: int, slot0: int, G: int, K: int,
                     out: Optional[torch.Tensor] = None) -> torch.Tensor:
    n_bank, H, W, Cc, ld = _chk_act(bank, "bank")
    if idx.dtype != torch.int32 or idx.device != bank.device or idx.dim() != 1 or not idx.is_contiguous() or idx.numel() != G * K:
        raise ValueError("flow_warp_frames: idx must be a dense int32 vector of G*K entries on the bank's device")
    if mv.dtype != torch.float32 or mv.device != bank.device:
        raise ValueError("flow_warp_frames: mv must be an fp32 tensor on the bank's device")
    if out is None:
        out = empty_act(G * K, H, W, Cc, bank.device)
    _, _, _, _, ldo = _chk_act(out, "out")
    if tuple(out.shape) != (G * K, H, W, Cc):
        raise ValueError("flow_warp_frames: out must hold G*K frames of the bank's shape")
    check(_lib.lib().cdfo_flow_warp_frames(_vp(bank), ld, n_bank, _vp(idx), _vp(mv), C.c_longlong(mv_kstride), slot0, G, K, H, W, Cc,
                                           _vp(out), ldo, _stream()), "cdfo_flow_warp_frames")
    return out


def resample2(x: torch.Tensor, up: bool, out: Optional[torch.Tensor] = None, accumulate: bool = False,
              out_f16: bool = False, cp16: bool = False) -> torch.Tensor:
    B, H, W, Cc, ld = _chk_act(x)
    Ho, Wo = (2 * H, 2 * W) if up else (H // 2, W // 2)
    if cp16:
        assert up and out is None and not accumulate
        out = torch.empty((B, Cc // 16, Ho, Wo, 16), dtype=torch.float16, device=x.device)
        check(_lib.lib().cdfo_resample2(_vp(x), ld, B, H, W, Cc, _vp(out), 16, 1, 0, 2, _stream()), "cdfo_resample2")
        return out
    odt = torch.float16 if out_f16 else torch.float32
    if out is None:
        assert not accumulate
        out = torch.empty((B, Ho, Wo, Cc), dtype=odt, device=x.device)
    ob, oh, ow, oc, ldo = _chk_act(out, "out", odt)
    assert (ob, oh, ow, oc) == (B, Ho, Wo, Cc)
    check(_lib.lib().cdfo_resample2(_vp(x), ld, B, H, W, Cc, _vp(out), ldo, int(up), int(accumulate), int(out_f16),
                                    _stream()), "cdfo_resample2")
    return out


def scale_channels(x: torch.Tensor, gate: torch.Tensor, want_cp16: bool = False):
    B, H, W, Cc, ld = _chk_act(x)
    out = empty_act(B, H, W, Cc, x.device)
    o16 = torch.empty((B, Cc // 16, H, W, 16), dtype=torch.float16, device=x.device) if want_cp16 else None
    check(_lib.lib().cdfo_scale_channels(_vp(x), ld, _vp(gate), B, C.c_longlong(H * W), Cc, _vp(out), Cc, _vp(o16),
                                         _stream()), "cdfo_scale_channels")
    return (out, o16) if want_cp16 else out


def upconv_last(x: torch.Tensor, pc: PackedConv, w_last: torch.Tensor, b_last: torch.Tensor, xc: torch.Tensor,
                xc_bstride: int) -> torch.Tensor:
    if not pc.shuffle2 or pc.Cout != 256 or pc.ks != 1:
        raise ValueError("upconv_last: needs the pixel-shuffle packing of a 1x1 conv with 256 outputs")
    a, taps = _conv_args([x], pc, act=ACT_LRELU, store_mode=3)
    B, H2, W2 = a.B, a.H, a.W
    a.res2 = w_last.detach().contiguous().float().data_ptr()
    check(_lib.lib().cdfo_conv1x1_bf16x3(C.byref(a), _stream()), "cdfo_conv1x1_bf16x3 (tap sums)")
    out = torch.empty((B, 1, 2 * H2, 2 * W2), dtype=torch.float32, device=x.device)
    check(_lib.lib().cdfo_conv_last_taps(_vp(taps), 12, _vp(b_last), _vp(xc), C.c_longlong(xc_bstride), B, 2 * H2, 2 * W2,
                                         _vp(out), _stream()), "cdfo_conv_last_taps")
    return out


def conv_last(x: torch.Tensor, w: torch.Tensor, bias: torch.Tensor, xc: torch.Tensor, xc_bstride: int) -> torch.Tensor:
    B, Hh, Wh, Cc, ld = _chk_act(x)
    assert Cc == 64
    out = torch.empty((B, 1, Hh, Wh), dtype=torch.float32, device=x.device)
    check(_lib.lib().cdfo_conv_last(_vp(x), ld, _vp(w), _vp(bias), _vp(xc), C.c_longlong(xc_bstride), B, Hh, Wh,
                                    _vp(out), _stream()), "cdfo_conv_last")
    return out


def small_conv16(x: torch.Tensor, w: torch.Tensor, bias: torch.Tensor, stride: int, pad: int, out_pad: int = 0,
                 transposed: bool = False, act: int = ACT_NONE, out_hl: bool = False) -> torch.Tensor:
    B, H, W, Cc, ld = _chk_act(x)
    assert Cc == 16
    if transposed:
        Ho, Wo = (H - 1) * stride - 2 * pad + 3 + out_pad, (W - 1) * stride - 2 * pad + 3 + out_pad
    else:
        Ho, Wo = (H + 2 * pad - 3) // stride + 1, (W + 2 * pad - 3) // stride + 1
    if out_hl:
        hl = torch.empty((B, 2, Ho, Wo, 16), dtype=torch.float16, device=x.device)
        check(_lib.lib().cdfo_small_conv16_hl(_vp(x), ld, _vp(w), _vp(bias), B, H, W, stride, pad, out_pad, int(transposed), act,
                                              _vp(hl), _stream()), "cdfo_small_conv16_hl")
        return hl
    out = empty_act(B, Ho, Wo, 16, x.device)
    check(_lib.lib().cdfo_small_conv16(_vp(x), ld, _vp(w), _vp(bias), B, H, W, stride, pad, out_pad, int(transposed),
                                       act, _vp(out), 16, _stream()), "cdfo_small_conv16")
    return out


def spatial_gate16(x: torch.Tensor, w: torch.Tensor, bias: torch.Tensor) -> torch.Tensor:
    B, H, W, Cc, ld = _chk_act(x)
    assert Cc == 16
    out = empty_act(B, H, W, 16, x.device)
    check(_lib.lib().cdfo_spatial_gate16(_vp(x), ld, _vp(w), _vp(bias), B, H, W, _vp(out), 16, _stream()),
          "cdfo_spatial_gate16")
    return out


def chan_pool(x: torch.Tensor) -> torch.Tensor:
    B, H, W, Cc, ld = _chk_act(x)
    out = torch.empty((B, H, W, 2), dtype=torch.float32, device=x.device)
    check(_lib.lib().cdfo_chan_pool(_vp(x), ld, C.c_longlong(B * H * W), Cc, _vp(out), _stream()), "cdfo_chan_pool")
    return out


def gate_map_cumulative(pooled: torch.Tensor, cum: Optional[torch.Tensor], w: torch.Tensor, bias: torch.Tensor) -> torch.Tensor:
    B, H, W, two = pooled.shape
    if two != 2 or not pooled.is_contiguous() or (cum is not None and (tuple(cum.shape) != (B, H, W) or not cum.is_contiguous())):
        raise ValueError("gate_map_cumulative: pooled [B,H,W,2] and cum [B,H,W] expected")
    out = torch.empty((B, H, W), dtype=torch.float32, device=pooled.device)
    check(_lib.lib().cdfo_gate_map_cumulative(_vp(pooled), _vp(cum), _vp(w), _vp(bias), B, H, W, int(w.shape[-1]), _vp(out), _stream()),
          "cdfo_gate_map_cumulative")
    return out


def spatial_gate(x: torch.Tensor, w: torch.Tensor, bias: torch.Tensor) -> torch.Tensor:
    B, H, W, Cc, ld = _chk_act(x)
    out = empty_act(B, H, W, Cc, x.device)
    gate = torch.empty((B, H, W), dtype=torch.float32, device=x.device)
    check(_lib.lib().cdfo_spatial_gate(_vp(x), ld, _vp(chan_pool(x)), _vp(w), _vp(bias), B, H, W, Cc, int(w.shape[-1]),
                                       _vp(gate), _vp(out), Cc, _stream()), "cdfo_spatial_gate")
    return out


def rdab_mix(xf: torch.Tensor, xc: torch.Tensor, w3: torch.Tensor, b3: torch.Tensor, vmax: torch.Tensor,
             noise: torch.Tensor) -> torch.Tensor:
    B, H, W, Cc, ld = _chk_act(xf)
    if tuple(noise.shape) != (B, 64, H, W) or not noise.is_contiguous() or noise.dtype != torch.float32:
        raise ValueError(f"rdab_mix: noise must be a contiguous fp32 [B,64,H,W] tensor, got {tuple(noise.shape)}")
    if tuple(vmax.shape) != (B, 64) or tuple(w3.shape) != (1, 2, 3, 3):
        raise ValueError("rdab_mix: vmax must be [B,64] and the spatial weight [1,2,3,3]")
    out = empty_act(B, H, W, 64, xf.device)
    check(_lib.lib().cdfo_rdab_mix(_vp(xf), ld, _vp(chan_pool(xc)), _vp(w3), _vp(b3), _vp(vmax), _vp(noise), B, H, W,
                                   _vp(out), 64, _stream()), "cdfo_rdab_mix")
    return out


def shrink_planes(t: torch.Tensor, level: int) -> torch.Tensor:
    B, Cc, H, W = t.shape
    if t.stride(3) != 1 or t.stride(2) != W or t.stride(1) != H * W:
        t = t.contiguous()
    out = torch.empty((B, Cc, H >> level, W >> level), dtype=torch.float32, device=t.device)
    check(_lib.lib().cdfo_shrink_planes(_vp(t), C.c_longlong(t.stride(0)), Cc, B, H, W, level, _vp(out), _stream()),
          "cdfo_shrink_planes")
    return out


def lincomb(a: torch.Tensor, ca: float, b: Optional[torch.Tensor] = None, cb: float = 0.0,
            c: Optional[torch.Tensor] = None, cc: float = 0.0, out: Optional[torch.Tensor] = None) -> torch.Tensor:
    for t in (a, b, c, out):
        if t is not None and (not t.is_contiguous() or t.dtype != torch.float32 or t.shape != a.shape):
            raise ValueError("lincomb: contiguous fp32 tensors of one shape expected")
    if out is None:
        out = torch.empty_like(a)
    check(_lib.lib().cdfo_lincomb(_vp(out), _vp(a), float(ca), _vp(b), float(cb), _vp(c), float(cc),
                                  C.c_longlong(a.numel()), _stream()), "cdfo_lincomb")
    return out


def nchunks_for(P: int) -> int:
    return max(1, min(128, P // 1024))


def chan_sum_partial(x: torch.Tensor):
    B, H, W, Cc, ld = _chk_act(x)
    assert Cc == 64
    n = nchunks_for(H * W)
    part = torch.empty((B, n, 64), dtype=torch.float32, device=x.device)
    check(_lib.lib().cdfo_chan_sum_partial(_vp(x), ld, B, C.c_longlong(H * W), n, _vp(part), _stream()),
          "cdfo_chan_sum_partial")
    return part, n


def pack_rdab_stats(w2: torch.Tensor) -> torch.Tensor:
    if tuple(w2.shape) != (64, 64, 3, 3):
        raise ValueError(f"pack_rdab_stats: a [64,64,3,3] weight expected, got {tuple(w2.shape)}")
    w = w2.detach().float().permute(2, 3, 1, 0).reshape(9, 4, 2, 2, 4, 64).permute(0, 1, 3, 5, 2, 4).reshape(9, 4, 2, 64, 8)
    hi = w.to(torch.bfloat16)
    return torch.stack([hi, (w - hi.float()).to(torch.bfloat16)]).contiguous()


def rdab_stats_ok(H: int, W: int) -> bool:
    return H > 0 and W > 0 and H % 2 == 0 and W % 2 == 0 and H * W < (1 << 30)


def rdab_stats(img: torch.Tensor, Bi: int, s_b: int, s_g: int, B: int, H: int, W: int, w0: torch.Tensor, b0: torch.Tensor,
               w2_packed: torch.Tensor, b2: torch.Tensor, out: Optional[torch.Tensor] = None):
    if not rdab_stats_ok(H, W):
        raise ValueError(f"rdab_stats: an even-sized map expected, got {H} x {W} (use stem_conv2 + conv + chan_sum_partial)")
    if img.dtype != torch.float32 or not img.is_cuda or B <= 0 or Bi <= 0 or s_b < 0 or s_g < 0:
        raise ValueError("rdab_stats: an fp32 device tensor, B, Bi > 0 and non-negative strides expected")
    last = (min(B, Bi) - 1) * s_b + ((B - 1) // Bi) * s_g + H * W
    if last > img.untyped_storage().nbytes() // 4 - img.storage_offset():
        raise ValueError("rdab_stats: the planes reach beyond the tensor's storage")
    if (w2_packed.dtype != torch.bfloat16 or tuple(w2_packed.shape) != (2, 9, 4, 2, 64, 8) or not w2_packed.is_contiguous()
            or tuple(w0.shape) != (64, 1, 3, 3) or not w0.is_contiguous() or w0.dtype != torch.float32
            or any(t.numel() != 64 or t.dtype != torch.float32 or not t.is_contiguous() for t in (b0, b2))
            or any(t.device != img.device for t in (w0, b0, w2_packed, b2))):
        raise ValueError("rdab_stats: w0 [64,1,3,3], b0 [64], b2 [64] fp32 and pack_rdab_stats' image expected on the maps' device")
    count = (H // 2 + 1) * (W // 2 + 1)
    n = nchunks_for(count)
    if out is None:
        out = torch.empty((B, n, 64), dtype=torch.float32, device=img.device)
    elif tuple(out.shape) != (B, n, 64) or out.dtype != torch.float32 or not out.is_contiguous() or out.device != img.device:
        raise ValueError(f"rdab_stats: out must be a dense fp32 [{B},{n},64] tensor on the maps' device")
    with on_device(img):
        check(_lib.lib().cdfo_rdab_stats(_vp(img), Bi, C.c_longlong(s_b), C.c_longlong(s_g), _vp(w0), _vp(b0), _vp(w2_packed),
                                         _vp(b2), B, H, W, n, _vp(out), _stream()), "cdfo_rdab_stats")
    return out, n, count


def gram_partial(q: torch.Tensor, k: torch.Tensor, ch_per_head: int):
    B, H, W, Cc, ldq = _chk_act(q, "q")
    _, _, _, _, ldk = _chk_act(k, "k")
    n = nchunks_for(H * W)
    part = torch.empty((B, n, 64 * (ch_per_head + 2)), dtype=torch.float32, device=q.device)
    check(_lib.lib().cdfo_gram_partial(_vp(q), ldq, _vp(k), ldk, B, C.c_longlong(H * W), ch_per_head, n, _vp(part),
                                       _stream()), "cdfo_gram_partial")
    return part, n


def align_stats_slots(B: int, P: int) -> int:
    n = _lib.lib().cdfo_align_stats_slots(B, C.c_longlong(P))
    if n <= 0:
        raise CdfoError(f"cdfo_align_stats_slots({B}, {P}) failed: {n}")
    return n


def align_stats(x0: torch.Tensor, x1: torch.Tensor, q: torch.Tensor, pc: PackedConv, act: int, ch_per_head: int):
    B, H, W, c0, ld0 = _chk_act(x0, "x0")
    b1, h1, w1, c1, ld1 = _chk_act(x1, "x1")
    bq, hq, wq, cq, ldq = _chk_act(q, "q")
    if (b1, h1, w1) != (B, H, W) or (bq, hq, wq) != (B, H, W) or (c0, c1, cq) != (64, 64, 64):
        raise ValueError("align_stats: three [B,H,W,64] operands expected")
    if pc.ks != 1 or pc.Cin != 128 or pc.Cout != 64 or pc.CoutP != 64 or pc.w_bstride != 0:
        raise ValueError("align_stats: a packed 128 -> 64 1x1 convolution expected")
    n = align_stats_slots(B, H * W)
    gs = 64 * (ch_per_head + 2)
    buf = torch.zeros((B * n * (gs + 128),), dtype=torch.float32, device=q.device)
    gram = buf[:B * n * gs].view(B, n, gs)
    s0 = buf[B * n * gs:B * n * (gs + 64)].view(B, n, 64)
    s1 = buf[B * n * (gs + 64):].view(B, n, 64)
    check(_lib.lib().cdfo_align_stats(_vp(x0), ld0, _vp(x1), ld1, _vp(q), ldq, _vp(pc.w), _vp(pc.bias), act, ch_per_head, B,
                                      C.c_longlong(H * W), n, _vp(gram), _vp(s0), _vp(s1), _stream()), "cdfo_align_stats")
    return gram, s0, s1, n


def mdta_fold(part: torch.Tensor, n: int, temperature: torch.Tensor, proj_w: torch.Tensor) -> PackedConv:
    B = part.shape[0]
    wout = torch.empty((B, 4096), dtype=torch.float32, device=part.device)
    check(_lib.lib().cdfo_mdta_fold(_vp(part), n, _vp(temperature), _vp(proj_w), B, _vp(wout), _stream()),
          "cdfo_mdta_fold")
    return PackedConv(wout, None, 64, 64, 1, 64, False, 4096)


_FOLD_CIN = {}


def fold_scale_inputs(fold: PackedConv, gate: torch.Tensor) -> PackedConv:
    if fold.Cin != 64 or fold.Cout != 64 or fold.ks != 1 or fold.w_bstride != 4096 or tuple(gate.shape) != (fold.w.shape[0], 64):
        raise ValueError("fold_scale_inputs: a mdta_fold result and a [B, 64] gate expected")
    cin = _FOLD_CIN.get(gate.device)
    if cin is None:
        i = torch.arange(4096, device=gate.device)
        cin = (i // 1024) * 16 + ((i // 256) % 4) * 4 + i % 4
        if not (gate.is_cuda and torch.cuda.is_current_stream_capturing()):
            _FOLD_CIN[gate.device] = cin
    return PackedConv(fold.w * gate[:, cin], None, 64, 64, 1, 64, False, 4096)


def align_fold(gpart, ng, sw, sp, ns, P, temperature, du0_w, du0_b, du2_w, du2_b, proj_w, fusion_w) -> PackedConv:
    B = gpart.shape[0]
    wout = torch.empty((B, 192 * 64), dtype=torch.float32, device=gpart.device)
    check(_lib.lib().cdfo_align_fold(_vp(gpart), ng, _vp(sw), _vp(sp), ns, C.c_longlong(P), _vp(temperature),
                                     _vp(du0_w), _vp(du0_b), _vp(du2_w), _vp(du2_b), _vp(proj_w), _vp(fusion_w), B,
                                     _vp(wout), _stream()), "cdfo_align_fold")
    return PackedConv(wout, None, 64, 192, 1, 64, False, 192 * 64)


def vec_mlp(part: torch.Tensor, n: int, P: int, w1, b1, c1: int, act1: int, w2=None, b2=None, c2: int = 0,
            act2: int = ACT_NONE) -> torch.Tensor:
    B = part.shape[0]
    out = torch.empty((B, c2 if w2 is not None else c1), dtype=torch.float32, device=part.device)
    check(_lib.lib().cdfo_vec_mlp(_vp(part), n, C.c_longlong(P), _vp(w1), _vp(b1), c1, act1, _vp(w2), _vp(b2), c2, act2,
                                  B, _vp(out), _stream()), "cdfo_vec_mlp")
    return out


def _prep_outs(outs, B, H, W, device):
    if outs is None:
        return empty_act(B, H, W, 64, device), empty_act(B, H, W, 64, device), empty_act(B, H, W, 64, device)
    for t in outs:
        if tuple(t.shape) != (B, H, W, 64) or not t.is_contiguous() or t.dtype != torch.float32:
            raise ValueError("rdab_prep: outs must be three dense fp32 [B,H,W,64] tensors")
    return outs


def rdab_prep(xq: torch.Tensor, vmax: torch.Tensor, noise: torch.Tensor, wW: torch.Tensor, bW: torch.Tensor, outs=None):
    B, H, W, Cc, ld = _chk_act(xq)
    assert Cc == 128 and noise.is_contiguous() and tuple(noise.shape) == (B, 64, H, W)
    sq, vrow, qwin = _prep_outs(outs, B, H, W, xq.device)
    check(_lib.lib().cdfo_rdab_prep(_vp(xq), ld, _vp(vmax), _vp(noise), _vp(wW), _vp(bW), B, C.c_longlong(H * W),
                                    _vp(sq), 64, _vp(vrow), 64, _vp(qwin), 64, _stream()), "cdfo_rdab_prep")
    return sq, vrow, qwin


def rdab_prep_rng(xq: torch.Tensor, vmax: torch.Tensor, seed: int, draw: int, wW: torch.Tensor, bW: torch.Tensor,
                  noise_out: Optional[torch.Tensor] = None, outs=None):
    B, H, W, Cc, ld = _chk_act(xq)
    assert Cc == 128
    if noise_out is not None and (tuple(noise_out.shape) != (B, 64, H, W) or not noise_out.is_contiguous()
                                  or noise_out.dtype != torch.float32):
        raise ValueError("rdab_prep_rng: noise_out must be a contiguous fp32 [B,64,H,W] tensor")
    sq, vrow, qwin = _prep_outs(outs, B, H, W, xq.device)
    if isinstance(seed, torch.Tensor):
        if seed.dtype != torch.int64 or seed.numel() != 1 or seed.device != xq.device:
            raise ValueError("rdab_prep_rng: a device-side key must be an int64[1] tensor on the operands' device")
        check(_lib.lib().cdfo_rdab_prep_rng_dev(_vp(xq), ld, _vp(vmax), _vp(seed), draw, _vp(noise_out), _vp(wW), _vp(bW), B,
                                                C.c_longlong(H * W), _vp(sq), 64, _vp(vrow), 64, _vp(qwin), 64, _stream()),
              "cdfo_rdab_prep_rng_dev")
        return sq, vrow, qwin
    check(_lib.lib().cdfo_rdab_prep_rng(_vp(xq), ld, _vp(vmax), C.c_longlong(seed & 0x7FFFFFFFFFFFFFFF), draw, _vp(noise_out),
                                        _vp(wW), _vp(bW), B, C.c_longlong(H * W), _vp(sq), 64, _vp(vrow), 64, _vp(qwin), 64,
                                        _stream()), "cdfo_rdab_prep_rng")
    return sq, vrow, qwin


def rdab_prep_fused_ok(x: torch.Tensor, pc: PackedConv) -> bool:
    return (x.dim() == 4 and x.shape[3] == 64 and (x.shape[1] * x.shape[2]) % 64 == 0 and pc.ks == 1 and pc.Cin == 64
            and pc.Cout == 128 and pc.CoutP == 128 and pc.w_bstride == 0 and not pc.shuffle2)


def rdab_prep_fused(x: torch.Tensor, pc: PackedConv, vmax: torch.Tensor, noise, wW: torch.Tensor, bW: torch.Tensor,
                    v_f16: bool = False, outs=None, plane=None):
    B, H, W, Cc, ld = _chk_act(x, "x")
    if not rdab_prep_fused_ok(x, pc):
        raise ValueError("rdab_prep_fused: a 64 -> 128 1x1 convolution over H*W % 64 == 0 pixels expected (use conv + rdab_prep)")
    row16, win16 = (v_f16, v_f16) if isinstance(v_f16, bool) else v_f16
    dts = (torch.float32, torch.float16 if row16 else torch.float32, torch.float32, torch.float16 if win16 else torch.float32)
    if outs is None:
        outs = tuple(torch.empty((B, H, W, 64), dtype=dt, device=x.device) for dt in dts)
    sq, vrow, qwin, vwin = outs
    for t, dt in zip(outs, dts):
        if tuple(t.shape) != (B, H, W, 64) or not t.is_contiguous() or t.dtype != dt:
            raise ValueError("rdab_prep_fused: outs must be dense [B,H,W,64] tensors: sq, qwin fp32; vrow, vwin fp32 or, as v_f16 says, fp16")
    seed, seed_dev, draw, noise_in, noise_out = 0, None, 0, None, None
    if isinstance(noise, tuple):
        _, seed, draw, noise_out = noise
        if noise_out is not None and (tuple(noise_out.shape) != (B, 64, H, W) or not noise_out.is_contiguous()
                                      or noise_out.dtype != torch.float32):
            raise ValueError("rdab_prep_fused: noise_out must be a contiguous fp32 [B,64,H,W] tensor")
        if isinstance(seed, torch.Tensor):
            if seed.dtype != torch.int64 or seed.numel() != 1 or seed.device != x.device:
                raise ValueError("rdab_prep_fused: a device-side key must be an int64[1] tensor on the operands' device")
            seed, seed_dev = 0, seed
        else:
            seed &= 0x7FFFFFFFFFFFFFFF
    else:
        noise_in = noise
        if tuple(noise.shape) != (B, 64, H, W) or not noise.is_contiguous() or noise.dtype != torch.float32:
            raise ValueError("rdab_prep_fused: noise must be a contiguous fp32 [B,64,H,W] tensor")
    args = (_vp(x), ld, _vp(pc.w), _vp(pc.bias), _vp(vmax), _vp(noise_in), C.c_longlong(seed), _vp(seed_dev), draw, _vp(noise_out),
            _vp(wW), _vp(bW), B, C.c_longlong(H * W), _vp(sq), 64, _vp(vrow), 64, _vp(qwin), 64, _vp(vwin), 64,
            int(row16) + 2 * int(win16))
    if plane is not None:
        view, Bi, s_b, s_g, table, _ = _plane_args(plane[:5], B, H, W, 128, "rdab_prep_fused")
        check(_lib.lib().cdfo_rdab_prep_fused_plane(*args, _vp(view), Bi, C.c_longlong(s_b), C.c_longlong(s_g), W, _vp(table), _stream()),
              "cdfo_rdab_prep_fused_plane")
    else:
        check(_lib.lib().cdfo_rdab_prep_fused(*args, _stream()), "cdfo_rdab_prep_fused")
    return sq, vrow, qwin, vwin


_seed_counter = 0


def next_noise_seed(device) -> int:
    global _seed_counter
    if torch.cuda.is_current_stream_capturing():
        base, off = int(torch.initial_seed()), 4 * _seed_counter
        _seed_counter += 1
    else:
        g = torch.cuda.default_generators[device.index if device.index is not None else torch.cuda.current_device()]
        base, off = int(g.initial_seed()), int(g.get_offset())
        g.set_offset(off + 4)
    return (base * 0x9E3779B97F4A7C15 + off * 0xD1B54A32D192ED03 + 0x632BE59BD9B4E019) & 0x7FFFFFFFFFFFFFFF


def colconv9(x: torch.Tensor, wH: torch.Tensor, bH: torch.Tensor) -> torch.Tensor:
    B, H, W, Cc, ld = _chk_act(x)
    out = empty_act(B, H, W, 64, x.device)
    check(_lib.lib().cdfo_colconv9(_vp(x), ld, _vp(wH), _vp(bH), B, H, W, _vp(out), 64, _stream()), "cdfo_colconv9")
    return out


def seq_attn(q: torch.Tensor, v: torch.Tensor, mode: int, out: Optional[torch.Tensor] = None,
             out_dtype: torch.dtype = torch.float32) -> torch.Tensor:
    if out is not None:
        out_dtype = out.dtype
    v_f16, out_f16 = v.dtype == torch.float16, out_dtype == torch.float16
    if (v_f16 and mode not in (20, 21, 22)) or (out_f16 and mode != 20):
        raise ValueError(f"seq_attn: an fp16 v needs mode 20, 21 or 22 and an fp16 out mode 20, got mode {mode}")
    B, H, W, Cc, ldq = _chk_act(q, "q")
    _, _, _, _, ldv = _chk_act(v, "v", v.dtype if v_f16 else torch.float32)
    if out is None:
        out = torch.empty((B, H, W, 64), dtype=out_dtype, device=q.device)
    _, _, _, _, ldo = _chk_act(out, "out", out_dtype if out_f16 else torch.float32)
    if v_f16 or out_f16:
        check(_lib.lib().cdfo_seq_attn_f16(_vp(q), ldq, _vp(v), ldv, _vp(out), ldo, B, H, W, mode, int(v_f16), int(out_f16),
                                           _stream()), "cdfo_seq_attn_f16")
        return out
    check(_lib.lib().cdfo_seq_attn(_vp(q), ldq, _vp(v), ldv, _vp(out), ldo, B, H, W, mode, _stream()), "cdfo_seq_attn")
    return out


def _train_batch(who, lr, pms, rms, ufs, mvl0, mvl1, hr, plan, crop):
    S, T, H, W = lr.shape
    want = [(lr, torch.uint8, (S, T, H, W)), (pms, torch.uint8, (S, T, H, W)), (rms, torch.int8, (S, T, H, W)),
            (ufs, torch.uint8, (S, T, ufs.shape[2] if ufs.dim() == 4 else -1, W)), (mvl0, torch.int8, (S, T, H, W, 3)),
            (hr, torch.uint8, (S, T, 4 * H, 4 * W))]
    if mvl1 is not None:
        want.append((mvl1, torch.int8, (S, T, H, W, 3)))
    for t, dtype, shape in want:
        if not t.is_cuda or t.device != lr.device or t.dtype != dtype or tuple(t.shape) != shape or not t.is_contiguous():
            raise ValueError(f"{who}: a dense {dtype} device tensor {shape} expected, got {t.dtype} {tuple(t.shape)} on {t.device}")
    if plan.dtype != torch.int32 or plan.dim() != 2 or plan.shape[1] != 8 or not plan.is_contiguous() or plan.device != lr.device \
            or plan.shape[0] == 0:
        raise ValueError(f"{who}: the plan is a dense int32 [B,8] tensor on the clip set's device, B >= 1")
    B, c, dev = int(plan.shape[0]), int(crop), lr.device
    if c <= 0 or c % 4 or c > min(H, W):
        raise ValueError(f"{who}: crop must be a positive multiple of 4 that fits the {H}x{W} frames, got {crop}")
    f32 = dict(dtype=torch.float32, device=dev)
    x, pm = torch.empty((B, 7, 1, c, c), **f32), torch.empty((B, 7, 1, c, c), **f32)
    rm, uf = torch.empty((B, 1, 7, c, c), **f32), torch.empty((B, 1, 7, c, c), **f32)
    mvs0, hro = torch.empty((B, 7, 2, c, c), **f32), torch.empty((B, 1, 4 * c, 4 * c), **f32)
    tail = (S, T, H, W, int(ufs.shape[2]), _vp(plan), B, c, _vp(x), _vp(pm), _vp(rm), _vp(uf), _vp(mvs0), _vp(hro), _stream())
    if mvl1 is None:
        check(_lib.lib().cdfo_train_batch(_vp(lr), _vp(pms), _vp(rms), _vp(ufs), _vp(mvl0), _vp(hr), *tail), "cdfo_train_batch")
    else:
        check(_lib.lib().cdfo_train_batch_ra(_vp(lr), _vp(pms), _vp(rms), _vp(ufs), _vp(mvl0), _vp(mvl1), _vp(hr), *tail),
              "cdfo_train_batch_ra")
    return x, mvs0, pm, rm, uf, hro


def train_batch(lr: torch.Tensor, pms: torch.Tensor, rms: torch.Tensor, ufs: torch.Tensor, mvl0: torch.Tensor, hr: torch.Tensor,
                plan: torch.Tensor, crop: int):
    return _train_batch("train_batch", lr, pms, rms, ufs, mvl0, None, hr, plan, crop)


def train_batch_ra(lr: torch.Tensor, pms: torch.Tensor, rms: torch.Tensor, ufs: torch.Tensor, mvl0: torch.Tensor, mvl1: torch.Tensor,
                   hr: torch.Tensor, plan: torch.Tensor, crop: int):
    if mvl1 is None:
        raise ValueError("train_batch_ra: mvl1 is required")
    return _train_batch("train_batch_ra", lr, pms, rms, ufs, mvl0, mvl1, hr, plan, crop)


CHARBONNIER_MAX_BLOCKS = 1024


def charbonnier(sr: torch.Tensor, hr: torch.Tensor, eps: float):
    for name, t in (("sr", sr), ("hr", hr)):
        if not t.is_cuda or t.dtype != torch.float32 or not t.is_contiguous():
            raise ValueError(f"charbonnier: {name} must be a dense fp32 device tensor, got {t.dtype} {tuple(t.shape)} strides {t.stride()}")
    if sr.shape != hr.shape or sr.device != hr.device or sr.numel() == 0:
        raise ValueError(f"charbonnier: sr and hr must have one non-empty shape on one device, got {tuple(sr.shape)} and {tuple(hr.shape)}")
    n = sr.numel()
    g = torch.empty_like(sr)
    partial = torch.empty(CHARBONNIER_MAX_BLOCKS, dtype=torch.float64, device=sr.device)
    loss = torch.empty((), dtype=torch.float32, device=sr.device)
    check(_lib.lib().cdfo_charbonnier(_vp(sr), _vp(hr), C.c_longlong(n), C.c_float(eps), _vp(g), _vp(partial), CHARBONNIER_MAX_BLOCKS,
                                      _vp(loss), _stream()), "cdfo_charbonnier")
    return loss, g
```

### cdfo_amd/switches.py

```python
from __future__ import annotations

import functools
import os
from typing import NamedTuple, Optional, Tuple, Union

ONOFF, INT, PATH = "on/off", "int", "path"


class Switch(NamedTuple):
    name: str
    default: Union[int, None]
    kind: str
    layer: str
    meaning: str
    values: Optional[Tuple[int, ...]] = None


TABLE = (
    Switch("CDFO_LIB_PATH", None, PATH, "python", "another build of libcdfo_hip.so (A/B builds, the developer library cdfo_amd/lib/dev/)"),
    Switch("CDFO_DCN_EXACT", 0, ONOFF, "python", "1: the DCN forward always on its exact-fp32 kernel (cdfo_amd.dcn.EXACT_FP32)"),
    Switch("CDFO_TRAIN_EXACT", 0, ONOFF, "python", "1: the training path's convolutions on exact-fp32 MFMA (cdfo_amd.autograd.CONV_PREC = PREC_F32)"),
    Switch("CDFO_WINO", 1, ONOFF, "python", "0: Block_.body[0] stays on the direct weights-stationary kernel instead of the Winograd F(2,3) one"),
    Switch("CDFO_WINO_UP2", 1, ONOFF, "python", "0: Block_'s x2 branch on a materialised double-resolution source instead of the interpolating Winograd form"),
    Switch("CDFO_WINO_HS", 0, ONOFF, "python", "1: the x2 branch's 256-channel intermediate in half-split rows (model.wino_halfsplit; measured: no gain in the forward, 105.2 vs 105.3 ms)"),
    Switch("CDFO_UDSA_N16", 1, ONOFF, "python", "0: the prior U-net's first layer off the 16-channel kernel (model.udsa_n16)"),
    Switch("CDFO_UDSA_STREAM", 1, ONOFF, "python", "0: the prior U-net on the caller's stream instead of a side stream (model.udsa_side_stream)"),
    Switch("CDFO_ATTN_PV3", 0, ONOFF, "python", "1: all three fp16 passes in the attentions' second product instead of one (model.attn_pv_single = False)"),
    Switch("CDFO_OVERLAP_NEW", 1, ONOFF, "python", "0: streaming, frames 0-2 start behind the new frame's feature extraction, not beside it (model.overlap_new_frame)"),
    Switch("CDFO_NEW_ALONE", 1, ONOFF, "python", "0: streaming, the new frame's neighbour pipeline is not a group of its own (model.new_frame_alone)"),
    Switch("CDFO_TRUNK_SIDE", 1, ONOFF, "python", "0: Block_'s half-resolution branch on the caller's stream instead of a side stream (model.trunk_side_stream)"),
    Switch("CDFO_FEA_R_1PASS", 0, ONOFF, "python", "1: conv_expand_fea_r with activations rounded once to fp16 (model.fea_r_single_pass)"),
    Switch("CDFO_V7_FEAR_1PASS", 1, ONOFF, "python", "0: CVSR_V7's conv_expand_fea_r on fp16 hi + lo activations, two passes (model.fea_r_single_pass)"),
    Switch("CDFO_V7_FUSE_ASSEMBLY", 1, ONOFF, "python", "0: MVDualAttAlignment assembles offsets / masks in a kernel of its own (fuse_assembly)"),
    Switch("CDFO_V7_HEAD_1PASS", 1, ONOFF, "python", "0: MVDualAttAlignment's offset head on two-pass activations (head_one_pass)"),
    Switch("CDFO_V7_OFF0_1PASS", 1, ONOFF, "python", "0: MVDualAttAlignment's conv_offset[0] on two-pass activations (off0_one_pass)"),
    Switch("CDFO_V7_WS_HEAD", 1, ONOFF, "python", "0: MVDualAttAlignment's offset head off the weights-stationary kernel (ws_head)"),
    Switch("CDFO_ALIGN_STATS", 1, ONOFF, "python", "0: DualAttAlignment's statistics on the five launches of round 5: kf written, Gram and channel sums in passes of their own (model.align_stats)"),
    Switch("CDFO_RDAB_FUSED", 1, ONOFF, "python", "0: LLongRangAttention's input_conv and mask kernel as two launches with the 128-channel product written, every V operand of its attentions fp32 (model.rdab_fused)"),
    Switch("CDFO_PRIOR_STEMS", 1, ONOFF, "python", "0: LLongRangAttention's mask statistics through memory: du0 written by the stem kernel, read back by conv_du_re.2, its result summed by a third launch (model.prior_stems)"),
    Switch("CDFO_INLINE_RMS", 1, ONOFF, "python", "0: fea_com = fea + conv_expand_rms(rms) written by the stem kernel and read by the mask kernel and RDAB.fuse, instead of built inside their products from the residual map; needs CDFO_PRIOR_STEMS (model.inline_rms)"),
    Switch("CDFO_WS_RING", 1, ONOFF, "hip", "0: Block_.body[0] on the private-halo kernel of rounds 1-2 instead of the ring-fed wave-specialised one"),
    Switch("CDFO_WS_WAVES", 12, INT, "hip", "8: two instead of three waves per SIMD in the private-halo weights-stationary kernel", (8, 12)),
    Switch("CDFO_RING_SPLIT", 1, ONOFF, "hip", "0: the four-tap ring convolution on the eight-identical-waves kernel"),
    Switch("CDFO_RING_TOUCH", 0, ONOFF, "hip", "1: producer-side touches of the tile's residual lines ahead of the epilogue (measured useless, off)"),
    Switch("CDFO_CONV1X1_STREAM", 1, ONOFF, "hip", "0: 1x1 convolutions on the one-tile-per-workgroup kernel instead of the persistent streaming one"),
    Switch("CDFO_TAPS_STREAM", 1, ONOFF, "hip", "0: the CDFO_STORE_TAPS9 1x1 convolution off the persistent streaming kernel"),
    Switch("CDFO_ATTN_NW", 0, INT, "hip", "4 | 8: force the attention workgroup width (0: chosen per shape)", (0, 4, 8)),
    Switch("CDFO_ATTN_XCD", 1, INT, "hip", "0: attention workgroups of one sequence spread over the XCDs as in round 2"),
    Switch("CDFO_DCN_WIN", 1, INT, "hip", "0: the DCN forward on the round-2 gather kernel instead of the window-sampled one"),
    Switch("CDFO_DCN_DBG", 0, INT, "hip", "developer library only (-DCDFO_DEV_ABLATIONS): ablation code of the window-sampled DCN kernel, wrong results"),
)
_ROWS = {s.name: s for s in TABLE}


def _parse(sw: Switch, raw: Optional[str]):
    if sw.kind == PATH:
        return raw or None
    if raw is None:
        return bool(sw.default) if sw.kind == ONOFF else sw.default
    if sw.kind == ONOFF and raw in ("0", "1"):
        return raw == "1"
    if sw.kind == INT and raw.lstrip("-").isdigit() and (sw.values is None or int(raw) in sw.values):
        return int(raw)
    allowed = "0 or 1" if sw.kind == ONOFF else ("one of %s" % (sw.values,) if sw.values else "an integer")
    raise ValueError(f"{sw.name}={raw!r}: expected {allowed} (cdfo_amd/switches.py)")


@functools.lru_cache(maxsize=None)
def get(name: str):
    sw = _ROWS[name]
    if sw.layer != "python":
        raise KeyError(f"{name} is read by the HIP library, not by Python")
    return _parse(sw, os.environ.get(name))


def check_hip_environment() -> None:
    for sw in TABLE:
        if sw.layer == "hip":
            _parse(sw, os.environ.get(sw.name))
```

### include/cdfo_hip.h

```cpp
#ifndef CDFO_HIP_H
#define CDFO_HIP_H

#ifdef __cplusplus
extern "C" {
#endif

#define CDFO_EINVAL (-1)
#define CDFO_EALIGN (-2)
#define CDFO_MAXSRC 8

enum { CDFO_ACT_NONE = 0, CDFO_ACT_LRELU = 1, CDFO_ACT_RELU = 2, CDFO_ACT_SIGMOID = 3 };
enum { CDFO_STORE_PLAIN = 0, CDFO_STORE_SHUFFLE2 = 1, CDFO_STORE_S2D = 2, CDFO_STORE_TAPS9 = 3, CDFO_STORE_OFFMASK = 4,
       CDFO_STORE_S2D_HS = 5  };
enum { CDFO_DTYPE_F32 = 0, CDFO_DTYPE_F16 = 1, CDFO_DTYPE_F64 = 2 };
enum { CDFO_PREC_F32 = 0, CDFO_PREC_BF16X3 = 1, CDFO_PREC_BF16 = 2, CDFO_PREC_FP16X2 = 3, CDFO_PREC_FP16 = 4, CDFO_PREC_FP16X1 = 5 };

int cdfo_abi_version(void);
const char* cdfo_build_info(void);
int cdfo_set_cu_limit(int n);

typedef struct {
  const float* src[CDFO_MAXSRC]; int ld[CDFO_MAXSRC]; int cs[CDFO_MAXSRC]; int nsrc;
  int B, H, W, Ho, Wo;
  int ks, stride, pad;
  int Cin, Cout, CoutP;
  const float* w; long long w_bstride; const float* bias;
  int act;
  const float* res1; int ldr1;
  const float* res2; int ldr2;
  float* out; int ldo; int store_mode;
  int prec;
  const float* ln_gamma; const float* ln_beta;
  const unsigned* tap_mask;
  int src_f16;
  int out_f16;
  void* out2_cp16;
  int src_plane_wrap;
  const float* res_up2; int ldru;
  int out2_lo;
  float* mask_out; const float* flow; long long flow_bstride; float off_mag; int off_accumulate;
  const float* res2_pixscale;
  int src_halfsplit;
  float* chan_sum_out;
  int chan_sum_slots;
} cdfo_conv_args;
int cdfo_sizeof_conv_args(void);
int cdfo_conv_igemm(const cdfo_conv_args* a, void* stream);

int cdfo_pack_conv_weight(const float* w_oihw, float* packed, int Cout, int Cin, int ks, int shuffle2,
                          int transposed, void* stream);

int cdfo_conv3x3_bf16(const cdfo_conv_args* a, void* stream);
int cdfo_pack_conv3x3_bf16(const float* w_oihw, void* packed, int Cout, int Cin, void* stream);
int cdfo_pack_conv3x3_f16(const float* w_oihw, void* packed, int Cout, int Cin, void* stream);

int cdfo_conv3x3_c64_ws(const void* src_cp16, int B, int H, int W, const void* w_f16, int CoutP, const float* bias,
                        int Cout, int act, void* out_cp16, int store_mode, int dbg, void* clk_probe, void* stream);
int cdfo_conv3x3_c64_wino(const void* src_cp16, int B, int H, int W, const void* w_wino, const float* bias, int Cout, int act,
                          void* out_cp16, int store_mode, void* stream);
int cdfo_pack_conv3x3_wino(const float* w_oihw, void* packed, int Cout, void* stream);
int cdfo_conv3x3_c64_wino_up2(const void* src_lr_cp16, int B, int H, int W, const void* w_wino, const float* bias, int Cout, int act,
                              void* out_cp16, int store_mode, void* stream);
int cdfo_conv3x3_c64_wino_dbg(const void* src_cp16, int B, int H, int W, const void* w_wino, const float* bias, int Cout, int act,
                              void* out_cp16, int store_mode, int dbg, void* clk_probe, void* stream);
int cdfo_conv3x3_c64_ws_offmask(const void* src_cp16, int B, int H, int W, const void* w_f16, int CoutP, const float* bias, int Cout,
                                float* offset, float* mask, const float* flow, long long flow_bstride, float mag, int accumulate,
                                void* stream);

int cdfo_conv3x3_c64_ws_res(const void* src_cp16, int B, int H, int W, const void* w_f16, int CoutP, const float* bias,
                            int Cout, int act, float* out, int ldo, const float* res1, int ldr1, const float* res2,
                            int ldr2, void* out2_cp16, void* stream);
int cdfo_conv3x3_ring(const cdfo_conv_args* a, void* stream);
int cdfo_to_cp16(const float* in, int ldi, int B, long long P, int C, void* out_cp16, void* stream);

int cdfo_conv1x1_bf16x3(const cdfo_conv_args* a, void* stream);
int cdfo_conv1x1_bf16x3_plane(const cdfo_conv_args* a, const float* plane, int plane_Bi, long long plane_sb, long long plane_sg,
                              const float* plane_w, long long plane_w_bstride, void* stream);

int cdfo_conv_last_taps(const float* taps, int ldt, const float* bias, const float* xc, long long xc_bstride, int B, int Hh,
                        int Wh, float* out, void* stream);
int cdfo_nchw_to_nhwc(const float* in, float* out, int B, int C, int H, int W, int ldo, void* stream);
int cdfo_nhwc_to_nchw(const float* in, int ldi, float* out, int B, int C, int H, int W, void* stream);
int cdfo_swap_outer(const float* in, float* out, int B, int N, long long block, void* stream);
int cdfo_range_probe(const float* x, long long n, void* slots2, void* stream);

int cdfo_stem_conv(const float* img, long long img_bstride, const float* w, const float* bias, int B, int H, int W,
                   int act, float* out, int ldo, const float* add, int lda, float* out2, int ldo2, void* stream);
int cdfo_stem_conv2(const float* img, long long img_bstride, const float* wA, const float* bA, const float* add, int lda,
                    float* outA, int ldoA, const float* wB, const float* bB, int actB, float* outB, int ldoB, int s2dB, int B,
                    int H, int W, void* stream);
int cdfo_layernorm64(const float* in, int ldi, const float* gamma, const float* beta, long long npix, float* out,
                     int ldo, void* stream);
int cdfo_layernorm64_cp16hl(const float* in, int ldi, const float* gamma, const float* beta, int B, long long P, void* out,
                            void* stream);
int cdfo_dwconv3x3(const float* in, int ldi, const float* w, int B, int H, int W, int C, float* out, int ldo,
                   void* stream);
int cdfo_flow_warp(const float* in, int ldi, const float* mv, long long mv_bstride, int B, int H, int W, int C,
                   float* out, int ldo, void* stream);
int cdfo_resample2(const float* in, int ldi, int B, int H, int W, int C, float* out, int ldo, int up, int accumulate,
                   int out_f16, void* stream);
int cdfo_scale_channels(const float* in, int ldi, const float* gate, int B, long long P, int C, float* out, int ldo,
                        void* out_cp16, void* stream);
int cdfo_conv_last(const float* in, int ldi, const float* w, const float* bias, const float* xc, long long xc_bstride,
                   int B, int Hh, int Wh, float* out, void* stream);

int cdfo_small_conv16(const float* in, int ldi, const float* w, const float* bias, int B, int H, int W, int stride,
                      int pad, int out_pad, int transposed, int act, float* out, int ldo, void* stream);
int cdfo_small_conv16_hl(const float* in, int ldi, const float* w, const float* bias, int B, int H, int W, int stride,
                         int pad, int out_pad, int transposed, int act, void* out_hl, void* stream);
int cdfo_udsa_head(const float* img, long long img_bstride, const float* wc, const float* bt, const float* b0, int B, int H,
                   int W, float* out, int ldo, void* stream);
int cdfo_spatial_gate16(const float* in, int ldi, const float* w, const float* bias, int B, int H, int W, float* out,
                        int ldo, void* stream);

int cdfo_chan_sum_partial(const float* in, int ldi, int B, long long P, int nchunk, float* partial, void* stream);
int cdfo_rdab_stats(const float* img, int Bi, long long s_b, long long s_g, const float* w0, const float* b0,
                    const void* w2_packed, const float* b2, int B, int H, int W, int nchunk, float* partial, void* stream);
int cdfo_gram_partial(const float* q, int ldq, const float* k, int ldk, int B, long long P, int ch_per_head, int nchunk,
                      float* partial, void* stream);
int cdfo_align_stats_slots(int B, long long P);
int cdfo_stream_slots_for_grid(int B, long long P, int grid);
int cdfo_stream_slot_of(int B, long long P, int grid, int wg, int b);
int cdfo_align_stats(const float* x0, int ld0, const float* x1, int ld1, const float* q, int ldq, const float* w_packed,
                     const float* bias, int act, int ch_per_head, int B, long long P, int nslots, float* gram_partial,
                     float* sum0_partial, float* sum1_partial, void* stream);
int cdfo_mdta_fold(const float* partial, int nchunk, const float* temperature, const float* proj_w, int B, float* wout,
                   void* stream);
int cdfo_align_fold(const float* gram_partial, int nchunk_g, const float* sum_warp, const float* sum_pred, int nchunk_s,
                    long long P, const float* temperature, const float* du0_w, const float* du0_b, const float* du2_w,
                    const float* du2_b, const float* proj_w, const float* fusion_w, int B, float* wout, void* stream);
int cdfo_vec_mlp(const float* sum_partial, int nchunk, long long P, const float* w1, const float* b1, int c1, int act1,
                 const float* w2, const float* b2, int c2, int act2, int B, float* out, void* stream);

int cdfo_rdab_prep(const float* xq, int ldx, const float* vmax, const float* noise, const float* wW, const float* bW,
                   int B, long long P, float* sq, int lds_, float* vrow, int ldv, float* qwin, int ldw, void* stream);
int cdfo_rdab_prep_rng(const float* xq, int ldx, const float* vmax, long long seed, int draw, float* noise_out,
                       const float* wW, const float* bW, int B, long long P, float* sq, int lds_, float* vrow, int ldv,
                       float* qwin, int ldw, void* stream);
int cdfo_rdab_prep_rng_dev(const float* xq, int ldx, const float* vmax, const void* seed_dev, int draw, float* noise_out,
                           const float* wW, const float* bW, int B, long long P, float* sq, int lds_, float* vrow, int ldv,
                           float* qwin, int ldw, void* stream);
int cdfo_rdab_prep_fused(const float* x, int ldx, const float* w_packed, const float* bias, const float* vmax,
                         const float* noise, long long seed, const void* seed_dev, int draw, float* noise_out,
                         const float* wW, const float* bW, int B, long long P, float* sq, int lds_, void* vrow, int ldv,
                         float* qwin, int ldw, void* vwin, int ldvw, int v_f16, void* stream);
int cdfo_rdab_prep_fused_plane(const float* x, int ldx, const float* w_packed, const float* bias, const float* vmax,
                               const float* noise, long long seed, const void* seed_dev, int draw, float* noise_out,
                               const float* wW, const float* bW, int B, long long P, float* sq, int lds_, void* vrow, int ldv,
                               float* qwin, int ldw, void* vwin, int ldvw, int v_f16, const float* plane, int plane_Bi,
                               long long plane_sb, long long plane_sg, int W, const float* plane_w, void* stream);
int cdfo_colconv9(const float* in, int ldi, const float* wH, const float* bH, int B, int H, int W, float* out, int ldo,
                  void* stream);
int cdfo_metric_partials(const float* a, const float* b, int N, int H, int W, int crop, float scale, int clamp, int round8,
                         int metric, double* partial, int partial_cap, int* nblocks_out, void* stream);
int cdfo_block_prologue(const float* x, int ldx, int B, int H, int W, const void* w_bf16, const float* bias128, void* u16,
                        void* d16, void* x16, void* stream);
int cdfo_block_prologue2(const float* x, int ldx, int B, int H, int W, const void* w_bf16, const float* bias128, void* u16, void* t16,
                         void* d16, void* x16, void* stream);
int cdfo_qkv_dw_gram_slots(int B, int H, int W);
int cdfo_qkv_dw(const float* x, int ldx, int B, int H, int W, const void* w_bf16, const float* bias, const float* dw_w,
                float eps, float* out, int ldo, float* gram, int gram_slots, void* stream);
int cdfo_seq_attn(const float* q, int ldq, const float* v, int ldv, float* out, int ldo, int B, int H, int W, int mode,
                  void* stream);
int cdfo_seq_attn_f16(const float* q, int ldq, const void* v, int ldv, void* out, int ldo, int B, int H, int W, int mode,
                      int v_f16, int out_f16, void* stream);

long long cdfo_dcn_workspace_bytes(int B, int C, int H, int W, int Co, int kh, int kw, int groups, int deformable_groups);
int cdfo_dcn_forward(const float* in, const float* offset, const float* mask, const float* weight, const float* bias,
                     float* out, int B, int C, int H, int W, int Co, int kh, int kw, int sh, int sw, int ph, int pw,
                     int dh, int dw, int groups, int deformable_groups, void* workspace, long long workspace_bytes,
                     void* stream);

int cdfo_dcn_backward(const float* in, const float* offset, const float* mask, const float* weight,
                      const float* grad_out, float* grad_in, float* grad_offset, float* grad_mask, float* grad_weight,
                      float* grad_bias, int B, int C, int H, int W, int Co, int kh, int kw, int sh, int sw, int ph,
                      int pw, int dh, int dw, int groups, int deformable_groups, float scale, void* stream);
long long cdfo_dcn_backward_workspace_bytes(int B, int C, int H, int W, int Co, int kh, int kw, int sh, int sw, int ph,
                                            int pw, int dh, int dw, int groups, int deformable_groups);
int cdfo_dcn_backward_ws(const float* in, const float* offset, const float* mask, const float* weight,
                         const float* grad_out, float* grad_in, float* grad_offset, float* grad_mask, float* grad_weight,
                         float* grad_bias, int B, int C, int H, int W, int Co, int kh, int kw, int sh, int sw, int ph,
                         int pw, int dh, int dw, int groups, int deformable_groups, float scale, void* workspace,
                         long long workspace_bytes, void* stream);

long long cdfo_dcn_workspace_bytes_dt(int dtype, int backward, int B, int C, int H, int W, int Co, int kh, int kw, int sh,
                                      int sw, int ph, int pw, int dh, int dw, int groups, int deformable_groups);
int cdfo_dcn_forward_dt(int dtype, const void* in, const void* offset, const void* mask, const void* weight,
                        const void* bias, void* out, int B, int C, int H, int W, int Co, int kh, int kw, int sh, int sw,
                        int ph, int pw, int dh, int dw, int groups, int deformable_groups, void* workspace,
                        long long workspace_bytes, void* stream);
int cdfo_dcn_backward_dt(int dtype, const void* in, const void* offset, const void* mask, const void* weight,
                         const void* grad_out, void* grad_in, void* grad_offset, void* grad_mask, void* grad_weight,
                         void* grad_bias, int B, int C, int H, int W, int Co, int kh, int kw, int sh, int sw, int ph, int pw,
                         int dh, int dw, int groups, int deformable_groups, float scale, void* workspace,
                         long long workspace_bytes, void* stream);

long long cdfo_conv_wgrad_slab_floats(int A, int Bc, int ks, int nsplit);
int cdfo_conv_wgrad(const float* S, int lds_, int A, const float* L, int ldl, int Bc, int N, int Hs, int Ws, int Hl, int Wl,
                    int ks, int stride, int pad, int nsplit, float* slab, float* dw, int Btot, int b_off, void* stream);
int cdfo_conv_wgrad_prec(const float* S, int lds_, int A, const float* L, int ldl, int Bc, int N, int Hs, int Ws, int Hl, int Wl,
                         int ks, int stride, int pad, int nsplit, float* slab, float* dw, int Btot, int b_off, int prec,
                         void* stream);
int cdfo_coldot(const float* a, int lda, const float* b, int ldb, int nimg, long long P, int C, int nchunk, float scale,
                float* part, float* out, void* stream);
int cdfo_ew(const float* a, int lda, const float* b, int ldb, long long rows, int C, int mode, int aux, float scale, long long P,
            float* out, int ldo, void* stream);
int cdfo_layernorm64_bwd(const float* x, int ldx, const float* g, int ldg, const float* gamma, long long npix, float* dx,
                         int ldo, float* part, int nblk, void* stream);
int cdfo_dwconv3x3_wgrad(const float* x, int ldx, const float* g, int ldg, int B, int H, int W, int C, float* part, int nblk,
                         void* stream);
int cdfo_spatial_gate16_bwd(const float* t, int ldt, const float* g, int ldg, const float* w, const float* bias, int B, int H,
                            int W, float* scratch, float* dt, int ldo, float* dw99, void* stream);
int cdfo_gumbel_mask(const float* vmax, const float* noise, long long seed, int draw, float* noise_out, int B, long long P,
                     float* mask, int ldm, void* stream);
int cdfo_chanconv9(const float* in, int ldi, const float* w9, const float* bias, int flip, long long npix, float* out, int ldo,
                   void* stream);
int cdfo_corr9(const float* in, int ldi, const float* g, int ldg, int axis, int B, int H, int W, float* part, int nblk,
               void* stream);
int cdfo_seq_attn_bwd(const float* q, int ldq, const float* v, int ldv, const float* o, int ldo, const float* g, int ldg,
                      float* dq, int lddq, float* dv, int lddv, int B, int H, int W, int mode, void* stream);
int cdfo_flow_warp_bwd(const float* g, int ldg, const float* mv, long long mv_bstride, int B, int H, int W, int C, float* dx,
                       int ldo, void* stream);
int cdfo_resample2_bwd(const float* g, int ldg, int B, int H, int W, int C, int up, float* din, int ldo, void* stream);

int cdfo_chan_pool(const float* x, int ld, long long npix, int C, float* out, void* stream);
int cdfo_gate_map_cumulative(const float* pooled, const float* cum_in, const float* w, const float* bias, int B, int H, int W, int ks,
                             float* cum_out, void* stream);
int cdfo_spatial_gate(const float* x, int ld, const float* pooled, const float* w, const float* bias, int B, int H, int W,
                      int C, int ks, float* gate_scratch, float* out, int ldo, void* stream);
int cdfo_rdab_mix(const float* xf, int ld, const float* pooled, const float* w3, const float* b3, const float* vmax,
                  const float* noise, int B, int H, int W, float* out, int ldo, void* stream);
int cdfo_shrink_planes(const float* src, long long src_bstride, int planes, int B, int H, int W, int level, float* dst,
                       void* stream);
int cdfo_lincomb(float* out, const float* a, float ca, const float* b, float cb, const float* c, float cc, long long n,
                 void* stream);

int cdfo_conv2d_nchw(const float* in, const float* w, const float* bias, int B, int C, int H, int W, int Co, int kh,
                     int kw, int stride, int pad, int act, float* out, void* stream);
int cdfo_maxpool_nchw(const float* in, int BC, int H, int W, int k, int stride, float* out, void* stream);
int cdfo_resize_bilinear_nchw(const float* in, int BC, int H, int W, int Ho, int Wo, int accumulate, float* out,
                              void* stream);
int cdfo_avgpool_nchw(const float* in, int BC, long long P, float* out, void* stream);
int cdfo_ew_nchw(const float* a, const float* b, const float* x, const float* y, long long n, long long P, int mode,
                 float* out, void* stream);
int cdfo_mv_offset_mask(const float* o1, const float* o2, int ld, const float* flow, long long flow_bstride, int B,
                        long long P, int third, float mag, float* offset, float* mask, void* stream);

int cdfo_conv3x3_c64_n16(const float* x, int ldx, int B, int H, int W, const void* w_packed, const float* bias, int act, float* out,
                         int ldo, void* stream);

int cdfo_conv2d_nchw_bwd(const float* in, const float* w, const float* gout, int B, int C, int H, int W, int Co, int kh, int kw,
                         int stride, int pad, float* gin, float* gw, float* gbias, void* stream);
int cdfo_maxpool_nchw_bwd(const float* in, const float* gout, int BC, int H, int W, int k, int stride, int* idx_scratch, float* gin,
                          void* stream);
int cdfo_resize_bilinear_nchw_bwd(const float* gout, int BC, int H, int W, int Ho, int Wo, float* gin, void* stream);
int cdfo_ew_nchw_bwd(const float* g, const float* y, const float* a, const float* x, const float* yv, long long n, long long P,
                     int mode, float* out, void* stream);
int cdfo_gate_nchw_bwd_y(const float* g, const float* a, const float* x, int BC, long long P, float* gy, void* stream);
int cdfo_mv_offset_mask_bwd(const float* o1, const float* o2, int ld, const float* goff, const float* gmask, int B, long long P,
                            int third, float mag, float* g1, float* g2, void* stream);

int cdfo_chan_pool_bwd(const float* x, int ld, const float* dpooled, long long npix, float* dx, int ldo, void* stream);
int cdfo_mul_plane(const float* x, int ld, const float* plane, long long npix, float* out, int ldo, void* stream);
int cdfo_dot_plane(const float* a, int lda, const float* b, int ldb, long long npix, float* out, void* stream);
int cdfo_gumbel_softmax(const float* v, const float* u, int B, long long P, float* out, int ldo, void* stream);
int cdfo_softmax64_bwd(const float* r, int ldr, const float* dm, int ldm, long long npix, float* dz, int ldo, void* stream);

#define CDFO_MV_F32 0
#define CDFO_MV_F64 1
#define CDFO_MV_F16 2
#define CDFO_MV_BF16 3
#define CDFO_MV_I8 4
#define CDFO_MV_U8 5
#define CDFO_MV_I16 6
#define CDFO_MV_I32 7
#define CDFO_MV_I64 8
int cdfo_seq_flows(const void* mv, int dtype, int T, int H, int W, int i0, int K, int Hp, int Wp, float* out, void* stream);
int cdfo_gather_frames(const void* src, int n_src, const int* idx, int n_dst, long long frame_bytes, void* dst, void* stream);
int cdfo_flow_warp_frames(const float* bank, int ldi, int n_bank, const int* idx, const float* mv, long long mv_kstride, int slot0,
                          int G, int K, int H, int W, int C, float* out, int ldo, void* stream);

int cdfo_live_planes(const void* lr, const void* ufs, const unsigned char* pms, const float* rms, int sample_bytes, int cap, int H, int W,
                     const int* table, int K, int E, int Hp, int Wp, int peak, float* x, float* r, float* u, float* lr_new, float* p_new,
                     float* r_new, void* stream);
int cdfo_seq_flows_ring(const float* ring, int cap, int H, int W, int i0, int K, int T_known, int Hp, int Wp, float* out, void* stream);

#define CDFO_QUANT_TRUNC 0
#define CDFO_QUANT_NEAREST 1
int cdfo_finish_frames(const float* src, int src_pitch, long long src_fstride, int K, int Ho, int Wo, unsigned char* dst, int mode,
                       const unsigned char* gt, int gt_pitch, long long gt_fstride, int Hgt, int Wgt, int crop, long long* partial,
                       int partial_cap, int* nblocks_out, void* stream);
int cdfo_metric_partials_u8(const unsigned char* a, int a_pitch, long long a_fstride, int Ha, int Wa, const unsigned char* b,
                            int b_pitch, long long b_fstride, int Hb, int Wb, int N, int crop, int metric, double* partial,
                            int partial_cap, int* nblocks_out, void* stream);

int cdfo_chroma_up4(const unsigned char* src, int src_pitch, long long src_pstride, int N, int h, int w, unsigned char* dst,
                    const unsigned char* gt, int gt_pitch, long long gt_pstride, int Hgt, int Wgt, int crop, long long* partial,
                    int partial_cap, int* nblocks_out, void* stream);

int cdfo_finish_frames_u16(const float* src, int src_pitch, long long src_fstride, int K, int Ho, int Wo, unsigned short* dst, int peak,
                           int mode, const unsigned short* gt, int gt_pitch, long long gt_fstride, int Hgt, int Wgt, int crop,
                           long long* partial, int partial_cap, int* nblocks_out, void* stream);
int cdfo_ssim_partials_u16(const unsigned short* a, int a_pitch, long long a_fstride, int Ha, int Wa, const unsigned short* b,
                           int b_pitch, long long b_fstride, int Hb, int Wb, int N, int crop, int peak, double* partial,
                           int partial_cap, int* nblocks_out, void* stream);
int cdfo_chroma_up4_u16(const unsigned short* src, int src_pitch, long long src_pstride, int N, int h, int w, unsigned short* dst,
                        int peak, const unsigned short* gt, int gt_pitch, long long gt_pstride, int Hgt, int Wgt, int crop,
                        long long* partial, int partial_cap, int* nblocks_out, void* stream);

#define CDFO_MSSSIM_MIN_SIZE 176
long long cdfo_msssim_pyramid_bytes(int Hc, int Wc, int N);
int cdfo_msssim_partials_u8(const unsigned char* a, int a_pitch, long long a_fstride, int Ha, int Wa, const unsigned char* b,
                            int b_pitch, long long b_fstride, int Hb, int Wb, int N, int crop, float* pyramid, long long pyramid_bytes,
                            double* partial, int partial_cap, int* nblocks_out, void* stream);
int cdfo_msssim_partials_u16(const unsigned short* a, int a_pitch, long long a_fstride, int Ha, int Wa, const unsigned short* b,
                             int b_pitch, long long b_fstride, int Hb, int Wb, int N, int crop, int peak, float* pyramid,
                             long long pyramid_bytes, double* partial, int partial_cap, int* nblocks_out, void* stream);

#define CDFO_NIQE_TABLE 9801
int cdfo_niqe_mscn_u8(const unsigned char* src, int pitch, long long fstride, int K, int R, int C, const double* window, double* dst,
                      void* stream);
int cdfo_niqe_mscn_f64(const double* src, int pitch, long long fstride, int K, int R, int C, const double* window, double* dst,
                       void* stream);
int cdfo_niqe_half(const unsigned char* src, int pitch, long long fstride, int K, int R, int C, double* dst, void* stream);
int cdfo_niqe_block_sums(const double* mscn, int K, int R, int C, int B, double* sums, void* stream);
int cdfo_niqe_features(const double* sums, int K, int nb, int count, const double* table, int scale, double* features, void* stream);

#define CDFO_BRISQUE_TABLE 9801
#define CDFO_BRISQUE_STRIP 16
int cdfo_brisque_mscn_u8(const unsigned char* src, int pitch, long long fstride, int K, int H, int W, const double* window, double* dst,
                         void* stream);
int cdfo_brisque_mscn_f64(const double* src, int pitch, long long fstride, int K, int H, int W, const double* window, double* dst,
                          void* stream);
int cdfo_brisque_half(const unsigned char* src, int pitch, long long fstride, int K, int H, int W, double* dst, void* stream);
int cdfo_brisque_sums(const double* mscn, int K, int H, int W, double* partials, void* stream);
int cdfo_brisque_features(const double* partials, int K, int G, int count, const double* table, int scale, double* features,
                          void* stream);

#define CDFO_TOF_MIN 32
#define CDFO_TOF_MAX_TAPS 19
#define CDFO_TOF_STRIP 16
int cdfo_tof_level_u8(const unsigned char* prev, int ppitch, long long pstride, const unsigned char* cur, int cpitch, long long cstride,
                      const unsigned char* first, int fpitch, int K, int H, int W, int h, int w, const double* taps, int ntaps,
                      double* dst, void* stream);
int cdfo_tof_polyexp(const double* img, int N, int h, int w, const double* kernels, double* R, void* stream);
int cdfo_tof_matrices(const double* R, const double* flow, int N, int h, int w, double* M, void* stream);
int cdfo_tof_blur_solve(const double* M, int N, int h, int w, double* flow, void* stream);
int cdfo_tof_flow_up(const double* src, int N, int hp, int wp, int h, int w, double* dst, void* stream);
int cdfo_tof_epe(const double* a, const double* b, int K, int h, int w, double* partials, double* out, void* stream);

#define CDFO_LPIPS_MIN 16
#define CDFO_LPIPS_STRIP 2
#define CDFO_LPIPS_STEM_MAXC 256
#define CDFO_LPIPS_MAX_LAYERS 8
int cdfo_lpips_stem_u8(const unsigned char* src, int pitch, long long fstride, int N, int h, int w, const float* weight,
                       const float* bias, int C0, int normalize, float* dst, void* stream);
int cdfo_lpips_pool2(const float* src, int N, int H, int W, int C, float* dst, void* stream);
int cdfo_lpips_dist(const float* fa, const float* fb, const double* lin, int N, int h, int w, int C, double* partials, void* stream);
int cdfo_lpips_fold(const double* partials, int N, int layers, const int* strips, const long long* counts, double* out, void* stream);

#define CDFO_CHARBONNIER_MAX_BLOCKS 1024
int cdfo_train_batch(const unsigned char* lr, const unsigned char* pms, const signed char* rms, const unsigned char* ufs,
                     const signed char* mvl0, const unsigned char* hr, int S, int T, int H, int W, int Hu, const int* plan, int B,
                     int crop, float* x, float* pms_out, float* rms_out, float* ufs_out, float* mvs0, float* hr_out, void* stream);
int cdfo_train_batch_ra(const unsigned char* lr, const unsigned char* pms, const signed char* rms, const unsigned char* ufs,
                        const signed char* mvl0, const signed char* mvl1, const unsigned char* hr, int S, int T, int H, int W, int Hu,
                        const int* plan, int B, int crop, float* x, float* pms_out, float* rms_out, float* ufs_out, float* mvs,
                        float* hr_out, void* stream);
int cdfo_charbonnier(const float* sr, const float* hr, long long n, float eps, float* grad, double* partial, int partial_cap,
                     float* loss, void* stream);

int cdfo_prof_begin(int max_records);
int cdfo_prof_end(int* launches, double* ms, double* flops, double* bytes, int nkid);
int cdfo_prof_kid_count(void);

#ifdef __cplusplus
}
#endif
#endif
```

Measured before the change: 78.71 frames/s.

## Build ufs_prior inline from partition plane in align stats and folded conv

Adds a plane variant of the alignment statistics kernel that recomputes the conv_expand_ufs 3x3 stem from the raw partition plane inside its MFMA product instead of reading a materialised 64-channel ufs_prior. The per-channel sum of ufs_prior is recovered from summed stencil taps through a stencil table. The fold kernel composes the gated attention weights with the stencil into per-batch tables, so the later 192->64 conv shrinks to 128 inputs plus the plane taps. This removes one stem launch per neighbour and the write and reads of a 64-channel activation, at the cost of more LDS and extra tap loads per tile.

```diff
diff --git a/cdfo_amd/csrc/conv1x1_stream.hip b/cdfo_amd/csrc/conv1x1_stream.hip
--- a/cdfo_amd/csrc/conv1x1_stream.hip
+++ b/cdfo_amd/csrc/conv1x1_stream.hip
@@ -368,14 +368,15 @@
   const float* w; const float* bias; int act_fn;
   long long P; int tiles_per_image; long long tiles;
   float* gram; float* sum0; float* sum1; int slots;
+  pc_plane plane; const float* stencil;
 };
 
 constexpr int SG_NS = 3;
 
-template <int CH>
+template <int CH, bool PLANE = false>
 __global__ __launch_bounds__(ST_THREADS) void align_gram_partial_kernel(sg_args a) {
   extern __shared__ __attribute__((aligned(16))) unsigned char smem[];
-  constexpr int NS = SG_NS, NKB = 2, IPT = 3, GS = CH + 2;
+  constexpr int NS = SG_NS, NKB = PLANE ? 1 : 2, IPT = NKB + 1, GS = CH + 2;
   const int tid = threadIdx.x, lane = tid & 63, h = lane >> 5, r = lane & 31;
   const int wave = __builtin_amdgcn_readfirstlane(tid >> 6);
   constexpr int w_half = NKB * 4 * 2 * 64 * 16;
@@ -385,6 +386,10 @@
   float* sBias = reinterpret_cast<float*>(smem + 2 * w_half);
   unsigned char* ring = smem + ring_off + wave * NS * ST_STAGE;
   const unsigned ring_lds = (unsigned)(unsigned long long)(smem) + ring_off + wave * NS * ST_STAGE;
+  unsigned char* sPh = smem + ring_off + 4 * NS * ST_STAGE;
+  unsigned char* sPl = sPh + pc_weight_bytes(1) / 2;
+  const unsigned char* tap_slots = sPh + pc_weight_bytes(1) + wave * NS * PC_SLOT;
+  const unsigned tap_lds = (unsigned)(unsigned long long)(smem) + ring_off + 4 * NS * ST_STAGE + pc_weight_bytes(1) + wave * NS * PC_SLOT;
 
   const long long t_lo = a.tiles * blockIdx.x / gridDim.x, t_hi = a.tiles * (blockIdx.x + 1) / gridDim.x;
   if (t_lo >= t_hi) return;
@@ -399,7 +404,7 @@
   }
   auto part_off = [&](int q) { return r * 256 + ((q ^ (r & 15)) << 4); };
 
-  for (int i = tid; i < (128 >> 2) * 64; i += ST_THREADS) {
+  for (int i = tid; i < (NKB * 64 >> 2) * 64; i += ST_THREADS) {
     const int rowpos = i % 64, kg = i / 64;
     const int n = mfma_row_channel(rowpos);
     const f32x4 wv = *reinterpret_cast<const f32x4*>(a.w + ((long long)kg * 64 + n) * 4);
@@ -411,6 +416,7 @@
     *reinterpret_cast<u32x2*>(sWl + off) = lo;
   }
   for (int i = tid; i < 64; i += ST_THREADS) sBias[i] = a.bias ? a.bias[i] : 0.f;
+  if (PLANE) pc_load_weights<1>(a.plane.w, 64, sPh, sPl, tid);
 
   const int c_part = lane >> 2, c_sub = (lane & 3) * 4, h_part = (lane / CH) * CH / 4;
 
@@ -426,6 +432,8 @@
       const long long tile = img_t0 + it / IPT;
       const st_item src = a.src[(int)(it % IPT)];
       const long long p0 = (tile - (long long)b * a.tiles_per_image) * 128 + wave * 32;
+      if (PLANE && it % IPT == 0)
+        pc_issue(pc_image(a.plane, b), (int)a.P, a.plane.W, (int)p0, lane, tap_lds + (unsigned)((it / IPT) % NS) * PC_SLOT);
       const long long rows_left = a.P - p0;
       const float* base = src.base + ((long long)b * a.P + (rows_left > 0 ? p0 : 0)) * src.ld + src.ch0;
       i32x4 rsrc = lds_dma_rsrc_uniform(base, 0u);
@@ -440,11 +448,19 @@
 
     f32x16 acc[2];
     float g[CH], sq = 0.f, sk = 0.f, sx[2] = {0.f, 0.f};
+    float ts[PLANE ? 10 : 1];
+#pragma unroll
+    for (int j = 0; j < (PLANE ? 10 : 1); ++j) ts[j] = 0.f;
 #pragma unroll
     for (int j = 0; j < CH; ++j) g[j] = 0.f;
     for (long long it = 0; it < n_items; ++it) {
       const int k = (int)(it % IPT);
-      st_wait_landed(issued - it - 1);
+      if (!PLANE) st_wait_landed(issued - it - 1);
+      else {
+        if (issued - it - 1 == 0) wait_vm<0>();
+        else if (k == 0) wait_vm<8>();
+        else wait_vm<11>();
+      }
       const unsigned char* st = ring + (it % NS) * ST_STAGE;
       if (k == 0) {
 #pragma unroll
@@ -474,6 +490,19 @@
         for (int p = 0; p < 32; ++p)
           t4[p & 3] += *reinterpret_cast<const float*>(st + p * 256 + ((c_part ^ (p & 15)) << 4) + c_sub);
         sx[k] += (t4[0] + t4[1]) + (t4[2] + t4[3]);
+        if (PLANE) {
+          const int p = (int)((img_t0 + it / IPT - (long long)b * a.tiles_per_image) * 128) + wave * 32 + r;
+          unsigned thi[4], tlo[4];
+          float t9[9];
+          pc_operand<true>(tap_slots + ((it / IPT) % NS) * PC_SLOT, r, h, p, (int)a.P, a.plane.W, thi, tlo, t9);
+          f32x16 pacc[1][2] = {{acc[0], acc[1]}};
+          pc_mfma<1>(sPh, sPl, r, h, thi, tlo, pacc);
+          acc[0] = pacc[0][0];
+          acc[1] = pacc[0][1];
+#pragma unroll
+          for (int j = 0; j < 9; ++j) ts[j] += t9[j];
+          ts[PLANE ? 9 : 0] += p < (int)a.P ? 1.f : 0.f;
+        }
         if (k == NKB - 1) {
           const long long pin = (img_t0 + it / IPT - (long long)b * a.tiles_per_image) * 128 + wave * 32 + r;
           const bool inside = pin < a.P;
@@ -529,7 +558,16 @@
       red[lane * GS + CH] = sq;
       red[lane * GS + CH + 1] = sk;
       red[64 * GS + lane] = sx[0];
-      red[64 * GS + 64 + lane] = sx[1];
+      if (!PLANE) red[64 * GS + 64 + lane] = sx[1];
+      else {
+#pragma unroll
+        for (int j = 0; j < 10; ++j) {
+          float v = ts[j];
+#pragma unroll
+          for (int m = 1; m < 32; m <<= 1) v += __shfl_xor(v, m, 64);
+          if (lane == 0) red[64 * GS + 64 + j] = v;
+        }
+      }
       __syncthreads();
       const int slot = (int)(blockIdx.x - st_owner((long long)b * a.tiles_per_image, a.tiles, gridDim.x));
       if (slot >= 0 && slot < a.slots) {
@@ -542,7 +580,17 @@
           const float v = (r0[i] + r1[i]) + (r2[i] + r3[i]);
           if (i < 64 * GS) a.gram[bs * (64 * GS) + i] = v;
           else if (i < 64 * GS + 64) a.sum0[bs * 64 + (i - 64 * GS)] = v;
-          else a.sum1[bs * 64 + (i - 64 * GS - 64)] = v;
+          else if (!PLANE) a.sum1[bs * 64 + (i - 64 * GS - 64)] = v;
+          else {
+            const int c = i - 64 * GS - 64;
+            float s1 = 0.f;
+#pragma unroll
+            for (int j = 0; j < 10; ++j) {
+              const int o = 64 * GS + 64 + j;
+              s1 = fmaf(a.stencil[c * 16 + j], (r0[o] + r1[o]) + (r2[o] + r3[o]), s1);
+            }
+            a.sum1[bs * 64 + c] = s1;
+          }
         }
       }
     }
@@ -575,34 +623,65 @@
   return cdfo_stream_slots_for_grid(B, P, cus);
 }
 
-extern "C" int cdfo_align_stats(const float* x0, int ld0, const float* x1, int ld1, const float* q, int ldq, const float* w_packed,
-                                const float* bias, int act, int ch_per_head, int B, long long P, int nslots, float* gram_partial,
-                                float* sum0_partial, float* sum1_partial, void* stream) {
-  if (B <= 0 || P <= 0 || nslots <= 0 || !x0 || !x1 || !q || !w_packed || !gram_partial || !sum0_partial || !sum1_partial) return CDFO_EINVAL;
+static int align_stats(const float* x0, int ld0, const float* x1, int ld1, const float* q, int ldq, const float* w_packed, const float* bias,
+                       int act, int ch_per_head, int B, long long P, int nslots, float* gram_partial, float* sum0_partial,
+                       float* sum1_partial, const pc_plane* pl, const float* stencil, void* stream) {
+  if (B <= 0 || P <= 0 || nslots <= 0 || !x0 || (!x1 && !pl) || !q || !w_packed || !gram_partial || !sum0_partial || !sum1_partial) return CDFO_EINVAL;
   if (act != CDFO_ACT_NONE && act != CDFO_ACT_LRELU && act != CDFO_ACT_RELU) return CDFO_EINVAL;
   if (ch_per_head != 8 && ch_per_head != 16) return CDFO_EINVAL;
-  const int lds_[3] = {ld0, ld1, ldq};
+  const int lds_[3] = {ld0, pl ? 64 : ld1, ldq};
   for (int i = 0; i < 3; ++i)
     if (lds_[i] < 64 || lds_[i] % 4 || (long long)lds_[i] * 4 * 32 >= (1ll << 31)) return CDFO_EINVAL;
   if (!aligned16(x0) || !aligned16(x1) || !aligned16(q) || !aligned16(w_packed) || !aligned16(gram_partial) || !aligned16(sum0_partial) ||
       !aligned16(sum1_partial))
     return CDFO_EALIGN;
   if ((P + 127) / 128 > 0x7fffffff / 2) return CDFO_EINVAL;
+  if (pl) {
+    if (!pl->base || !pl->w || !stencil || pl->Bi <= 0 || pl->s_b < 0 || pl->s_g < 0 || !pc_shape_ok(P, pl->W)) return CDFO_EINVAL;
+    if ((unsigned long long)pl->base % 4 || !aligned16(pl->w) || !aligned16(stencil)) return CDFO_EALIGN;
+  }
   hipStream_t st = static_cast<hipStream_t>(stream);
   sg_args s{};
-  s.src[0] = {x0, ld0, 0}; s.src[1] = {x1, ld1, 0}; s.src[2] = {q, ldq, 0};
+  s.src[0] = {x0, ld0, 0};
+  if (pl) { s.src[1] = {q, ldq, 0}; s.plane = *pl; s.stencil = stencil; }
+  else { s.src[1] = {x1, ld1, 0}; s.src[2] = {q, ldq, 0}; }
   s.w = w_packed; s.bias = bias; s.act_fn = act;
   s.P = P;
   s.gram = gram_partial; s.sum0 = sum0_partial; s.sum1 = sum1_partial; s.slots = nslots;
   int grid;
   if (!st_tiling(B, P, s.tiles_per_image, s.tiles, grid)) return CDFO_EINVAL;
   if (nslots < st_slots(B, s.tiles_per_image, grid)) return CDFO_EINVAL;
+  const double px = (double)B * P;
+  if (pl) {
+    const int lds = st_lds_bytes(1, 1, SG_NS) + pc_lds_bytes(1, SG_NS);
+    static_assert(st_lds_bytes(1, 1, SG_NS) + pc_lds_bytes(1, SG_NS) <= ST_MAX_LDS, "the PLANE form's LDS (128256 bytes)");
+    CdfoProfScope prof(st, KID_GRAM, px * (2.0 * 80 * 64 + 2.0 * 64 * 18), 4.0 * 129 * px);
+    static CdfoAttrOnce once8p, once16p;
+    return ch_per_head == 16 ? st_launch(align_gram_partial_kernel<16, true>, once16p, grid, lds, st, s)
+                             : st_launch(align_gram_partial_kernel<8, true>, once8p, grid, lds, st, s);
+  }
   const int lds = st_lds_bytes(2, 1, SG_NS);
-  const double px = (double)B * P;
   CdfoProfScope prof(st, KID_GRAM, px * (2.0 * 128 * 64 + 2.0 * 64 * 18), 4.0 * 192 * px);
   static CdfoAttrOnce once8, once16;
   return ch_per_head == 16 ? st_launch(align_gram_partial_kernel<16>, once16, grid, lds, st, s)
                            : st_launch(align_gram_partial_kernel<8>, once8, grid, lds, st, s);
+}
+
+extern "C" int cdfo_align_stats(const float* x0, int ld0, const float* x1, int ld1, const float* q, int ldq, const float* w_packed,
+                                const float* bias, int act, int ch_per_head, int B, long long P, int nslots, float* gram_partial,
+                                float* sum0_partial, float* sum1_partial, void* stream) {
+  if (!x1) return CDFO_EINVAL;
+  return align_stats(x0, ld0, x1, ld1, q, ldq, w_packed, bias, act, ch_per_head, B, P, nslots, gram_partial, sum0_partial, sum1_partial,
+                     nullptr, nullptr, stream);
+}
+
+extern "C" int cdfo_align_stats_plane(const float* x0, int ld0, const float* q, int ldq, const float* w_packed, const float* bias, int act,
+                                      int ch_per_head, int B, long long P, int nslots, float* gram_partial, float* sum0_partial,
+                                      float* sum1_partial, const float* plane, int plane_Bi, long long plane_sb, long long plane_sg,
+                                      int W, const float* plane_w, const float* stencil_w, void* stream) {
+  const pc_plane pl = {plane, plane_Bi, plane_sb, plane_sg, W, plane_w, 0};
+  return align_stats(x0, ld0, nullptr, 0, q, ldq, w_packed, bias, act, ch_per_head, B, P, nslots, gram_partial, sum0_partial, sum1_partial,
+                     &pl, stencil_w, stream);
 }
 
 int cdfo_conv1x1_stream_try(const cdfo_conv_args& a, hipStream_t st, const pc_plane* pl) {
diff --git a/cdfo_amd/csrc/plane_chunk.h b/cdfo_amd/csrc/plane_chunk.h
--- a/cdfo_amd/csrc/plane_chunk.h
+++ b/cdfo_amd/csrc/plane_chunk.h
@@ -48,8 +48,9 @@
   }
 }
 
+template <bool TAPS_OUT = false>
 __device__ __forceinline__ void pc_operand(const unsigned char* slot, int r, int h, int p, int P, int W, unsigned (&hi)[4],
-                                           unsigned (&lo)[4]) {
+                                           unsigned (&lo)[4], float* taps = nullptr) {
   const int x = p % W;
   const bool inside = p < P, lok = inside && x > 0, rok = inside && x + 1 < W;
   float t[9];
@@ -67,6 +68,10 @@
     v1[j] = h ? 0.f : t[4 + j];
   }
   split8_bf16(v0, v1, hi, lo);
+  if constexpr (TAPS_OUT) {
+#pragma unroll
+    for (int j = 0; j < 9; ++j) taps[j] = t[j];
+  }
 }
 
 template <int NCB>
diff --git a/cdfo_amd/csrc/stats.hip b/cdfo_amd/csrc/stats.hip
--- a/cdfo_amd/csrc/stats.hip
+++ b/cdfo_amd/csrc/stats.hip
@@ -112,6 +112,7 @@
   }
 }
 
+template <bool PLANE>
 __global__ __launch_bounds__(256) void align_fold_kernel(const float* __restrict__ gram_partial, int nchunk_g,
                                                          const float* __restrict__ sum_warp,
                                                          const float* __restrict__ sum_pred, int nchunk_s, float inv_P,
@@ -119,8 +120,10 @@
                                                          const float* __restrict__ du0_w, const float* __restrict__ du0_b,
                                                          const float* __restrict__ du2_w, const float* __restrict__ du2_b,
                                                          const float* __restrict__ proj, const float* __restrict__ wf,
-                                                         float* __restrict__ wout) {
+                                                         float* __restrict__ wout, const float* __restrict__ stencil,
+                                                         float* __restrict__ tables) {
   constexpr int CH = 16;
+  __shared__ float M2[PLANE ? 64 * 64 : 1];
   __shared__ float stats[64 * (CH + 2)];
   __shared__ float attn[64 * CH];
   __shared__ float Q[64 * 64];
@@ -158,15 +161,27 @@
     Q[idx] = s;
   }
   __syncthreads();
-  float* wo = wout + (long long)b * (192 * 64);
+  float* wo = wout + (long long)b * ((PLANE ? 128 : 192) * 64);
   for (int idx = threadIdx.x; idx < 4096; idx += blockDim.x) {
     const int o = idx >> 6, i = idx & 63, hb = (i / CH) * CH, j = i - hb;
     float r = 0.f;
 #pragma unroll
-    for (int cc = 0; cc < CH; ++cc) r += Q[o * 64 + hb + cc] * attn[(hb + cc) * CH + j];
+    for (int cc = 0; cc < CH; ++cc) r = fmaf(Q[o * 64 + hb + cc], attn[(hb + cc) * CH + j], r);
     wo[((i >> 2) * 64 + o) * 4 + (i & 3)] = r * gate[0][i];
-    wo[(((64 + i) >> 2) * 64 + o) * 4 + (i & 3)] = r * gate[1][i];
-    wo[(((128 + i) >> 2) * 64 + o) * 4 + (i & 3)] = wf[o * 128 + 64 + i];
+    if (PLANE) M2[idx] = r * gate[1][i];
+    else wo[(((64 + i) >> 2) * 64 + o) * 4 + (i & 3)] = r * gate[1][i];
+    wo[((((PLANE ? 64 : 128) + i) >> 2) * 64 + o) * 4 + (i & 3)] = wf[o * 128 + 64 + i];
+  }
+  if (PLANE) {
+    __syncthreads();
+    float* tb = tables + (long long)b * (64 * 16);
+    for (int idx = threadIdx.x; idx < 64 * 16; idx += blockDim.x) {
+      const int o = idx >> 4, j = idx & 15;
+      double s = 0.0;
+      if (j < 10)
+        for (int i = 0; i < 64; ++i) s = fma((double)M2[o * 64 + i], (double)stencil[i * 16 + j], s);
+      tb[idx] = (float)s;
+    }
   }
 }
 
@@ -244,9 +259,24 @@
                                const float* fusion_w, int B, float* wout, void* stream) {
   if (B <= 0 || nchunk_g <= 0 || nchunk_s <= 0 || P <= 0) return CDFO_EINVAL;
   CdfoProfScope prof(static_cast<hipStream_t>(stream), KID_FOLD, 0, 0);
-  hipLaunchKernelGGL(align_fold_kernel, dim3(B), dim3(256), 0, static_cast<hipStream_t>(stream), gram_partial, nchunk_g,
+  hipLaunchKernelGGL(align_fold_kernel<false>, dim3(B), dim3(256), 0, static_cast<hipStream_t>(stream), gram_partial, nchunk_g,
                      sum_warp, sum_pred, nchunk_s, 1.0f / (float)P, temperature, du0_w, du0_b, du2_w, du2_b, proj_w,
-                     fusion_w, wout);
+                     fusion_w, wout, nullptr, nullptr);
+  CDFO_LAUNCH_CHECK();
+  return 0;
+}
+
+extern "C" int cdfo_align_fold_plane(const float* gram_partial, int nchunk_g, const float* sum_warp, const float* sum_pred,
+                                     int nchunk_s, long long P, const float* temperature, const float* du0_w,
+                                     const float* du0_b, const float* du2_w, const float* du2_b, const float* proj_w,
+                                     const float* fusion_w, const float* stencil_w, int B, float* wout, float* tables,
+                                     void* stream) {
+  if (B <= 0 || nchunk_g <= 0 || nchunk_s <= 0 || P <= 0 || !stencil_w || !wout || !tables) return CDFO_EINVAL;
+  if (!aligned16(wout) || !aligned16(tables)) return CDFO_EALIGN;
+  CdfoProfScope prof(static_cast<hipStream_t>(stream), KID_FOLD, 0, 0);
+  hipLaunchKernelGGL(align_fold_kernel<true>, dim3(B), dim3(256), 0, static_cast<hipStream_t>(stream), gram_partial, nchunk_g,
+                     sum_warp, sum_pred, nchunk_s, 1.0f / (float)P, temperature, du0_w, du0_b, du2_w, du2_b, proj_w,
+                     fusion_w, wout, stencil_w, tables);
   CDFO_LAUNCH_CHECK();
   return 0;
 }
diff --git a/cdfo_amd/csrc/stream_ring.h b/cdfo_amd/csrc/stream_ring.h
--- a/cdfo_amd/csrc/stream_ring.h
+++ b/cdfo_amd/csrc/stream_ring.h
@@ -22,8 +22,8 @@
   grid = (int)(tiles < cus ? tiles : cus);
   return cus > 0;
 }
-inline int st_weight_bytes(int nkb, int ncb) { return 2 * (nkb * 4 * 2 * ncb * 64 * 16) + ncb * 64 * 4; }
-inline int st_lds_bytes(int nkb, int ncb, int ns) { return st_weight_bytes(nkb, ncb) + 4 * ns * ST_STAGE; }
+constexpr int st_weight_bytes(int nkb, int ncb) { return 2 * (nkb * 4 * 2 * ncb * 64 * 16) + ncb * 64 * 4; }
+constexpr int st_lds_bytes(int nkb, int ncb, int ns) { return st_weight_bytes(nkb, ncb) + 4 * ns * ST_STAGE; }
 
 template <class KernelPtr, class Args>
 int st_launch(KernelPtr kernel, CdfoAttrOnce& once, int grid, int lds, hipStream_t st, const Args& s) {
diff --git a/cdfo_amd/cvsr_v8.py b/cdfo_amd/cvsr_v8.py
--- a/cdfo_amd/cvsr_v8.py
+++ b/cdfo_amd/cvsr_v8.py
@@ -112,6 +112,7 @@
         self.rdab_fused = switches.get("CDFO_RDAB_FUSED")
         self.prior_stems = switches.get("CDFO_PRIOR_STEMS")
         self.inline_rms = switches.get("CDFO_INLINE_RMS")
+        self.inline_ufs = switches.get("CDFO_INLINE_UFS")
         self.neighbour_group = 0
         self.overlap_new_frame = switches.get("CDFO_OVERLAP_NEW")
         self.new_frame_alone = switches.get("CDFO_NEW_ALONE")
@@ -229,6 +230,10 @@
         w["rms_chunk_input_conv"] = K.pack_plane_chunk(*K.compose_stem_1x1(
             sd["conv_expand_rms.weight"], sd["conv_expand_rms.bias"], sd["RDAB.input_conv.weight"],
             torch.zeros_like(sd["RDAB.input_conv.bias"])))
+        w["ufs_chunk"] = K.pack_plane_chunk(sd["conv_expand_ufs.weight"], sd["conv_expand_ufs.bias"])
+        fo = sd["MV_deform_align.fusion_out.0.weight"]
+        w["ufs_chunk_fusion_out"] = K.pack_plane_chunk(*K.compose_stem_1x1(
+            sd["conv_expand_ufs.weight"], sd["conv_expand_ufs.bias"], fo[:, 64:], fo.new_zeros(fo.shape[0])))
         w[fe + "side_to_feaoneUDSA.body.0_n16"] = K.pack_conv_n16(sd[fe + "side_to_feaoneUDSA.body.0.weight"])
         w["udsa_head"] = K.pack_udsa_head(sd[fe + "side_to_feaoneUDSA.body.0.weight"], sd[fe + "side_to_feaoneUDSA.body.0.bias"],
                                           sd["conv_second.weight"], sd["conv_second.bias"])
@@ -360,7 +365,7 @@
             return self._conv(cat, w["RDAB.fuse"], res1=x, plane=(*rms_planes, w["rms_chunk"]))
         return self._conv(cat, w["RDAB.fuse"], res1=x)
 
-    def _align(self, w, xc, extra, pred, mvs, mv_bstride, out, frames=None):
+    def _align(self, w, xc, extra, pred, mvs, mv_bstride, out, frames=None, ufs_planes=None):
         raw = w["raw"]
         a = "MV_deform_align."
         GB, H, W, _ = xc.shape
@@ -372,20 +377,23 @@
         for g, mv in enumerate(mvs if frames is None else ()):
             K.flow_warp(extra[g * B:(g + 1) * B], mv, mv_bstride, out=warped[g * B:(g + 1) * B])
         fused = self.precision != "f32" and self.align_stats
-        if fused:
+        fold_args = (raw[a + "temperature"], raw[a + "conv_du.0.weight"], raw[a + "conv_du.0.bias"], raw[a + "conv_du.2.weight"],
+                     raw[a + "conv_du.2.bias"], raw[a + "project_out.weight"], raw[a + "fusion_out.0.weight"])
+        if ufs_planes is not None:
+            gp, sw, sp, ng = K.align_stats(warped, None, xc, w[a + "fusion_out.0"], K.ACT_RELU, 16,
+                                           plane=(*ufs_planes, w["ufs_chunk_fusion_out"], w["ufs_chunk"]))
+            fold128, tables = K.align_fold_plane(gp, ng, sw, sp, ng, H * W, *fold_args, w["ufs_chunk"])
+            o, part, n = self._conv([warped, xc], fold128, act=K.ACT_RELU, chan_sum_out=True, plane=(*ufs_planes, tables, 64 * 16))
+        elif fused:
             gp, sw, sp, ng = K.align_stats(warped, pred, xc, w[a + "fusion_out.0"], K.ACT_RELU, 16)
-            ns = ng
+            fold = K.align_fold(gp, ng, sw, sp, ng, H * W, *fold_args)
+            o, part, n = self._conv([warped, pred, xc], fold, act=K.ACT_RELU, chan_sum_out=True)
         else:
             kf = self._conv([warped, pred], w[a + "fusion_out.0"], act=K.ACT_RELU)
             gp, ng = K.gram_partial(xc, kf, 16)
             sw, ns = K.chan_sum_partial(warped)
             sp, _ = K.chan_sum_partial(pred)
-        fold = K.align_fold(gp, ng, sw, sp, ns, H * W, raw[a + "temperature"], raw[a + "conv_du.0.weight"],
-                            raw[a + "conv_du.0.bias"], raw[a + "conv_du.2.weight"], raw[a + "conv_du.2.bias"],
-                            raw[a + "project_out.weight"], raw[a + "fusion_out.0.weight"])
-        if fused:
-            o, part, n = self._conv([warped, pred, xc], fold, act=K.ACT_RELU, chan_sum_out=True)
-        else:
+            fold = K.align_fold(gp, ng, sw, sp, ns, H * W, *fold_args)
             o = self._conv([warped, pred, xc], fold, act=K.ACT_RELU)
             part, n = K.chan_sum_partial(o)
         gate = K.vec_mlp(part, n, H * W, raw[a + "CALayer.conv_du.0.weight"], raw[a + "CALayer.conv_du.0.bias"], 64,
@@ -925,18 +933,23 @@
         raw = w["raw"]
         B, N, _, H, W = mvs1.shape
         GB, P = len(idxs) * B, H * W
-        ufs_prior = K.empty_act(GB, H, W, NF, xcG.device)
-        for n, i in enumerate(idxs):
-            K.stem_conv(ufs[:, 0, i], N * P, B, H, W, raw["conv_expand_ufs.weight"], raw["conv_expand_ufs.bias"],
-                        out=ufs_prior[n * B:(n + 1) * B])
+        planes = ufs_prior = None
+        if (self.inline_ufs and "ufs_chunk" in w and self.precision != "f32" and not self.istraining and self.align_stats
+                and K.plane_ok(H, W) and ufs.dtype == torch.float32 and ufs.is_contiguous()):
+            planes = (ufs[:, 0, idxs[0]], B, N * P, P)
+        else:
+            ufs_prior = K.empty_act(GB, H, W, NF, xcG.device)
+            for n, i in enumerate(idxs):
+                K.stem_conv(ufs[:, 0, i], N * P, B, H, W, raw["conv_expand_ufs.weight"], raw["conv_expand_ufs.bias"],
+                            out=ufs_prior[n * B:(n + 1) * B])
         al = K.empty_act(GB, H, W, NF, xcG.device)
         xc = xcG if xcG.shape[0] == GB else xcG[:GB]
         self._align(w, xc, extra, ufs_prior, [mvs1[:, i] for i in idxs], N * 2 * P, al,
-                    frames=None if frames is None else (*frames, mvs1, idxs[0]))
+                    frames=None if frames is None else (*frames, mvs1, idxs[0]), ufs_planes=planes)
         if self.debug_taps is not None:
             for n, i in enumerate(idxs):
                 self.debug_taps[f"align_{i}"] = al[n * B:(n + 1) * B]
-        keep.extend([ufs_prior, xc])
+        keep.extend([xc] if ufs_prior is None else [ufs_prior, xc])
         return al
 
     @staticmethod
diff --git a/cdfo_amd/kernels.py b/cdfo_amd/kernels.py
--- a/cdfo_amd/kernels.py
+++ b/cdfo_amd/kernels.py
@@ -1383,9 +1383,11 @@
     return n
 
 
-def align_stats(x0: torch.Tensor, x1: torch.Tensor, q: torch.Tensor, pc: PackedConv, act: int, ch_per_head: int):
+def align_stats(x0: torch.Tensor, x1: Optional[torch.Tensor], q: torch.Tensor, pc: PackedConv, act: int, ch_per_head: int, plane=None):
+    if (x1 is None) != (plane is not None):
+        raise ValueError("align_stats: either x1 or the plane it is a stencil of")
     B, H, W, c0, ld0 = _chk_act(x0, "x0")
-    b1, h1, w1, c1, ld1 = _chk_act(x1, "x1")
+    b1, h1, w1, c1, ld1 = (B, H, W, 64, 0) if x1 is None else _chk_act(x1, "x1")
     bq, hq, wq, cq, ldq = _chk_act(q, "q")
     if (b1, h1, w1) != (B, H, W) or (bq, hq, wq) != (B, H, W) or (c0, c1, cq) != (64, 64, 64):
         raise ValueError("align_stats: three [B,H,W,64] operands expected")
@@ -1397,6 +1399,16 @@
     gram = buf[:B * n * gs].view(B, n, gs)
     s0 = buf[B * n * gs:B * n * (gs + 64)].view(B, n, 64)
     s1 = buf[B * n * (gs + 64):].view(B, n, 64)
+    if plane is not None:
+        view, Bi, s_b, s_g, table, _ = _plane_args(plane[:5], B, H, W, 64, "align_stats")
+        stencil = plane[5]
+        if (tuple(stencil.shape) != (64, 16) or stencil.dtype != torch.float32 or not stencil.is_contiguous()
+                or stencil.device != table.device or table.dim() != 2):
+            raise ValueError("align_stats: the stencil's table and the composed table must be fp32 [64,16] (pack_plane_chunk)")
+        check(_lib.lib().cdfo_align_stats_plane(_vp(x0), ld0, _vp(q), ldq, _vp(pc.w), _vp(pc.bias), act, ch_per_head, B,
+                                                C.c_longlong(H * W), n, _vp(gram), _vp(s0), _vp(s1), _vp(view), Bi, C.c_longlong(s_b),
+                                                C.c_longlong(s_g), W, _vp(table), _vp(stencil), _stream()), "cdfo_align_stats_plane")
+        return gram, s0, s1, n
     check(_lib.lib().cdfo_align_stats(_vp(x0), ld0, _vp(x1), ld1, _vp(q), ldq, _vp(pc.w), _vp(pc.bias), act, ch_per_head, B,
                                       C.c_longlong(H * W), n, _vp(gram), _vp(s0), _vp(s1), _stream()), "cdfo_align_stats")
     return gram, s0, s1, n
@@ -1432,6 +1444,18 @@
                                      _vp(du0_w), _vp(du0_b), _vp(du2_w), _vp(du2_b), _vp(proj_w), _vp(fusion_w), B,
                                      _vp(wout), _stream()), "cdfo_align_fold")
     return PackedConv(wout, None, 64, 192, 1, 64, False, 192 * 64)
+
+
+def align_fold_plane(gpart, ng, sw, sp, ns, P, temperature, du0_w, du0_b, du2_w, du2_b, proj_w, fusion_w, stencil):
+    B = gpart.shape[0]
+    if tuple(stencil.shape) != (64, 16) or stencil.dtype != torch.float32 or not stencil.is_contiguous():
+        raise ValueError("align_fold_plane: the stencil's table must be fp32 [64,16] (pack_plane_chunk)")
+    wout = torch.empty((B, 128 * 64), dtype=torch.float32, device=gpart.device)
+    tables = torch.empty((B, 64, 16), dtype=torch.float32, device=gpart.device)
+    check(_lib.lib().cdfo_align_fold_plane(_vp(gpart), ng, _vp(sw), _vp(sp), ns, C.c_longlong(P), _vp(temperature),
+                                           _vp(du0_w), _vp(du0_b), _vp(du2_w), _vp(du2_b), _vp(proj_w), _vp(fusion_w), _vp(stencil),
+                                           B, _vp(wout), _vp(tables), _stream()), "cdfo_align_fold_plane")
+    return PackedConv(wout, None, 64, 128, 1, 64, False, 128 * 64), tables
 
 
 def vec_mlp(part: torch.Tensor, n: int, P: int, w1, b1, c1: int, act1: int, w2=None, b2=None, c2: int = 0,
diff --git a/cdfo_amd/switches.py b/cdfo_amd/switches.py
--- a/cdfo_amd/switches.py
+++ b/cdfo_amd/switches.py
@@ -39,6 +39,7 @@
     Switch("CDFO_RDAB_FUSED", 1, ONOFF, "python", "0: LLongRangAttention's input_conv and mask kernel as two launches with the 128-channel product written, every V operand of its attentions fp32 (model.rdab_fused)"),
     Switch("CDFO_PRIOR_STEMS", 1, ONOFF, "python", "0: LLongRangAttention's mask statistics through memory: du0 written by the stem kernel, read back by conv_du_re.2, its result summed by a third launch (model.prior_stems)"),
     Switch("CDFO_INLINE_RMS", 1, ONOFF, "python", "0: fea_com = fea + conv_expand_rms(rms) written by the stem kernel and read by the mask kernel and RDAB.fuse, instead of built inside their products from the residual map; needs CDFO_PRIOR_STEMS (model.inline_rms)"),
+    Switch("CDFO_INLINE_UFS", 1, ONOFF, "python", "0: ufs_prior = conv_expand_ufs(ufs) written by one stem launch per neighbour and read by DualAttAlignment's statistics pass and its folded 192 -> 64 convolution, instead of built inside their products from the partition map; needs CDFO_ALIGN_STATS (model.inline_ufs)"),
     Switch("CDFO_WS_RING", 1, ONOFF, "hip", "0: Block_.body[0] on the private-halo kernel of rounds 1-2 instead of the ring-fed wave-specialised one"),
     Switch("CDFO_WS_WAVES", 12, INT, "hip", "8: two instead of three waves per SIMD in the private-halo weights-stationary kernel", (8, 12)),
     Switch("CDFO_RING_SPLIT", 1, ONOFF, "hip", "0: the four-tap ring convolution on the eight-identical-waves kernel"),
diff --git a/include/cdfo_hip.h b/include/cdfo_hip.h
--- a/include/cdfo_hip.h
+++ b/include/cdfo_hip.h
@@ -124,11 +124,19 @@
 int cdfo_align_stats(const float* x0, int ld0, const float* x1, int ld1, const float* q, int ldq, const float* w_packed,
                      const float* bias, int act, int ch_per_head, int B, long long P, int nslots, float* gram_partial,
                      float* sum0_partial, float* sum1_partial, void* stream);
+int cdfo_align_stats_plane(const float* x0, int ld0, const float* q, int ldq, const float* w_packed, const float* bias, int act,
+                           int ch_per_head, int B, long long P, int nslots, float* gram_partial, float* sum0_partial,
+                           float* sum1_partial, const float* plane, int plane_Bi, long long plane_sb, long long plane_sg, int W,
+                           const float* plane_w, const float* stencil_w, void* stream);
 int cdfo_mdta_fold(const float* partial, int nchunk, const float* temperature, const float* proj_w, int B, float* wout,
                    void* stream);
 int cdfo_align_fold(const float* gram_partial, int nchunk_g, const float* sum_warp, const float* sum_pred, int nchunk_s,
                     long long P, const float* temperature, const float* du0_w, const float* du0_b, const float* du2_w,
                     const float* du2_b, const float* proj_w, const float* fusion_w, int B, float* wout, void* stream);
+int cdfo_align_fold_plane(const float* gram_partial, int nchunk_g, const float* sum_warp, const float* sum_pred, int nchunk_s,
+                          long long P, const float* temperature, const float* du0_w, const float* du0_b, const float* du2_w,
+                          const float* du2_b, const float* proj_w, const float* fusion_w, const float* stencil_w, int B,
+                          float* wout, float* tables, void* stream);
 int cdfo_vec_mlp(const float* sum_partial, int nchunk, long long P, const float* w1, const float* b1, int c1, int act1,
                  const float* w2, const float* b2, int c2, int act2, int B, float* out, void* stream);
 
```

Measured after the change: 80.36 frames/s (median of 6 runs). 1.02x the previous value.
